# Cyan4973/FiniteStateEntropy

Measured on AMD Instinct MI355X. Metric: MB/s encode+decode per GPU on 32KB probagen blocks; bit-exact vs CPU ref, higher is better.
Workload: dtype u8; 1 GPU; probagen Proba14, 100000 x 32KB blocks per GPU, FSE encode+decode (one-shot calls at the reference's default limits: tableLog 11, decode maxLog 12), bit-exact check; blocks_per_gpu=100000, block_bytes=32768, codec=fse, parity=fse: roundtrip-all-blocks

## Files before the change

### finitestateentropy_amd/csrc/capi_batch.hip

```cpp
#include "internal.h"

extern "C" int FSEHIP_HIST_count_batch(unsigned* d_counts, unsigned* d_maxSymbolValues, size_t* d_results,
                                       const void* d_src, size_t srcStride, const size_t* d_sizes, size_t uniformSize,
                                       size_t nBlocks, void* stream)
{
    HistArgs a;
    a.counts = d_counts; a.maxSVs = d_maxSymbolValues; a.uniformMaxSV = 255; a.useUniformIn = 0;
    a.results = d_results; a.src = mkview(d_src, srcStride, d_sizes, uniformSize); a.nBlocks = nBlocks;
    return (int)launch_hist(a, (hipStream_t)stream);
}

extern "C" int FSEHIP_FSE_compress_usingCTable_batch(void* d_dst, size_t dstStride, size_t dstCapacity, size_t* d_results,
                                                     const void* d_src, size_t srcStride, const size_t* d_sizes, size_t uniformSize,
                                                     const FSEHIP_FSE_CTable* d_ctables, size_t ctableStrideU32, unsigned maxTableLog,
                                                     size_t nBlocks, void* stream)
{
    if (maxTableLog == 0 || maxTableLog > FSEHIP_FSE_MAX_TABLELOG) maxTableLog = FSEHIP_FSE_MAX_TABLELOG;
    FseEncArgs a;
    a.dst = (u8*)d_dst; a.dstStride = dstStride; a.dstCapacity = dstCapacity; a.results = d_results;
    a.src = mkview(d_src, srcStride, d_sizes, uniformSize);
    a.ctables = d_ctables; a.ctStrideU32 = ctableStrideU32; a.meta = nullptr;
    a.maxTableLog = maxTableLog; a.G = 0; a.slotU32 = 0; a.nBlocks = nBlocks; a.list = nullptr; a.count = nullptr;
    return (int)launch_fse_encode_auto(a, (hipStream_t)stream);
}

extern "C" int FSEHIP_FSE_decompress_usingDTable_batch(void* d_dst, size_t dstStride, size_t dstCapacity, size_t* d_results,
                                                       const void* d_cSrc, size_t cStride, const size_t* d_cSizes, size_t uniformCSize,
                                                       const FSEHIP_FSE_DTable* d_dtables, size_t dtableStrideU32, unsigned maxTableLog,
                                                       size_t nBlocks, void* stream)
{
    if (maxTableLog == 0 || maxTableLog > FSEHIP_FSE_MAX_TABLELOG) maxTableLog = FSEHIP_FSE_MAX_TABLELOG;
    FseDecArgs a;
    a.dst = (u8*)d_dst; a.dstStride = dstStride; a.dstCapacity = dstCapacity; a.results = d_results;
    a.csrc = mkview(d_cSrc, cStride, d_cSizes, uniformCSize);
    a.dtables = d_dtables; a.dtStrideU32 = dtableStrideU32; a.atab = nullptr; a.symtab = nullptr; a.meta = nullptr;
    a.maxTableLog = maxTableLog; a.G = 0; a.slotU32 = 0; a.nBlocks = nBlocks; a.tlMin = 0; a.declineNb0 = 0; a.onlyDeclined = 0;
    a.symScratch = nullptr; a.slotBitmap = nullptr; a.nSlots = 0; a.scratchSlotBytes = 0;
    return (int)launch_fse_decode(a, (hipStream_t)stream);
}

#define WS_SLACK 2048
#define WS_MAX_CHUNK 131072
static size_t ws_pass_blocks(size_t nBlocks) { const size_t c = nBlocks < WS_MAX_CHUNK ? nBlocks : WS_MAX_CHUNK; return c ? c : 1; }
static size_t ws_size(size_t nBlocks, size_t perBlock, size_t pad = 0) { return ws_pass_blocks(nBlocks) * perBlock + pad + WS_SLACK; }
static size_t round_chunk(size_t limit, size_t perRound)
{
    if (perRound == 0 || limit < perRound) return limit;
    return limit / perRound * perRound;
}
static size_t ws_chunk(size_t workspaceBytes, size_t nBlocks, size_t perBlock, size_t pad = 0, size_t perRound = 0)
{
    if (workspaceBytes < perBlock + pad + WS_SLACK) return 0;
    const size_t chunk = (workspaceBytes - WS_SLACK - pad) / perBlock;
    return chunk >= nBlocks ? nBlocks : round_chunk(chunk, perRound);
}
static inline size_t pass_blocks(size_t nBlocks, size_t b0, size_t chunk) { return nBlocks - b0 < chunk ? nBlocks - b0 : chunk; }

struct Carver {
    u8* const base; u8* p;
    explicit Carver(void* ws) : base((u8*)ws), p((u8*)ws) {}
    template <class T> T* take(size_t bytes) { T* const r = (T*)p; p += align_up(bytes, 256); return r; }
    template <class T> T* last(size_t bytes) { T* const r = (T*)p; p += bytes; return r; }
    size_t used() const { return (size_t)(p - base); }
};
template <class Meta> struct CounterWs {
    static constexpr size_t bytes_per_block = 1024 + 4 + 8 + sizeof(Meta);
    unsigned* counts; unsigned* maxSVs; size_t* hres; Meta* meta;
    CounterWs(Carver& c, size_t chunk)
        : counts(c.take<unsigned>(chunk * 1024)), maxSVs(c.take<unsigned>(chunk * 4)), hres(c.take<size_t>(chunk * 8)), meta(c.take<Meta>(chunk * sizeof(Meta))) {}
    HistArgs hist_args(unsigned msv, const BlockView& src, size_t nb) const
    {
        HistArgs h;
        h.counts = counts; h.maxSVs = maxSVs; h.uniformMaxSV = msv; h.useUniformIn = 1; h.results = hres; h.src = src; h.nBlocks = nb;
        return h;
    }
};
template <class Meta> struct BuildCTableWs {
    static constexpr size_t bytes_per_block = CounterWs<Meta>::bytes_per_block;
    Carver c; CounterWs<Meta> cb;
    BuildCTableWs(void* ws, size_t chunk) : c(ws), cb(c, chunk) {}
    size_t end() const { return c.used(); }
};

struct FseCWs { size_t perBlock; size_t ctU32; size_t ts; unsigned maxTl; };
static FseCWs fse_cws(unsigned tableLog)
{
    FseCWs w;
    unsigned tl = tableLog ? tableLog : FSEHIP_FSE_DEFAULT_TABLELOG;
    if (tl < 9) tl = 9;
    if (tl > FSEHIP_FSE_MAX_TABLELOG) tl = FSEHIP_FSE_MAX_TABLELOG;
    w.maxTl = tl;
    w.ctU32 = FSEHIP_FSE_CTABLE_SIZE_U32(tl, 255);
    w.ts = (size_t)1 << tl;
    w.perBlock = 1024 + 4 + 8 + sizeof(FseMeta) + 4 * w.ctU32 + FSE_EBINS * sizeof(u32);
    return w;
}
struct FseCompWs {
    Carver c; CounterWs<FseMeta> cb; u32* ctables; u32* encLists; u32* encCounts;
    FseCompWs(void* ws, size_t chunk, const FseCWs& w)
        : c(ws), cb(c, chunk), ctables(c.take<u32>(chunk * 4 * w.ctU32)), encLists(c.take<u32>(chunk * FSE_EBINS * sizeof(u32))),
          encCounts(c.last<u32>(FSE_EBINS * sizeof(u32))) {}
    size_t end() const { return c.used(); }
};

extern "C" size_t FSEHIP_FSE_compress_batch_workspaceSize(size_t nBlocks, unsigned tableLog) { return ws_size(nBlocks, fse_cws(tableLog).perBlock); }

extern "C" int FSEHIP_FSE_compress_batch(void* d_dst, size_t dstStride, size_t dstCapacity, size_t* d_results,
                                         const void* d_src, size_t srcStride, const size_t* d_sizes, size_t uniformSize,
                                         unsigned maxSymbolValue, unsigned tableLog, size_t nBlocks,
                                         void* d_workspace, size_t workspaceBytes, void* stream)
{
    hipStream_t s = (hipStream_t)stream;
    if ((uintptr_t)d_workspace & 255u) return (int)hipErrorInvalidValue;
    if (nBlocks == 0) return 0;
    if (tableLog > FSEHIP_FSE_MAX_TABLELOG)
        return batch_arg_error(d_results, nullptr, 0, dstCapacity, nBlocks, FSEHIP_ERROR(tableLog_tooLarge), 0, s);
    if (maxSymbolValue > 255 && tableLog != 0) {
        const size_t wksp = 4 * (size_t)FSEHIP_FSE_CTABLE_SIZE_U32(FSEHIP_FSE_MAX_TABLELOG, 255) + ((size_t)1 << FSEHIP_FSE_MAX_TABLELOG);
        const size_t ctBytes = 4 * (1 + ((size_t)1 << (tableLog - 1)) + 2 * ((size_t)maxSymbolValue + 1));
        if (ctBytes <= wksp && wksp - ctBytes < 4096)
            return batch_arg_error(d_results, d_sizes, uniformSize, dstCapacity, nBlocks, FSEHIP_ERROR(workSpace_tooSmall), 2, s);
    }
    return fse_compress_view(d_dst, dstStride, dstCapacity, d_results, mkview(d_src, srcStride, d_sizes, uniformSize), maxSymbolValue, tableLog, nBlocks,
                             d_workspace, workspaceBytes, s);
}
int fse_compress_view(void* d_dst, size_t dstStride, size_t dstCapacity, size_t* d_results, const BlockView& srcAll, unsigned maxSymbolValue, unsigned tableLog,
                      size_t nBlocks, void* d_workspace, size_t workspaceBytes, hipStream_t s)
{
    const FseCWs w = fse_cws(tableLog);
    const size_t chunk = ws_chunk(workspaceBytes, nBlocks, w.perBlock, 0, fse_encode_blocks_per_round(w.maxTl));
    if (chunk == 0) return (int)hipErrorInvalidValue;
    const FseCompWs ws(d_workspace, chunk, w);
    if (ws.end() > workspaceBytes) return (int)hipErrorInvalidValue;
    unsigned msv = maxSymbolValue ? maxSymbolValue : 255;
    if (msv > 255) msv = 255;
    for (size_t b0 = 0; b0 < nBlocks; b0 += chunk) {
        const size_t nb = pass_blocks(nBlocks, b0, chunk);
        const BlockView src = subview(srcAll, b0);
        CK(launch_hist(ws.cb.hist_args(msv, src, nb), s));
        FseCPrepArgs c;
        c.counts = ws.cb.counts; c.maxSVs = ws.cb.maxSVs; c.histResults = ws.cb.hres; c.src = src;
        c.dst = (u8*)d_dst + b0 * dstStride; c.dstStride = dstStride; c.dstCapacity = dstCapacity;
        c.maxSVReq = msv; c.tableLogReq = tableLog;
        c.ctables = ws.ctables; c.ctStrideU32 = w.ctU32; c.maxTl = w.maxTl;
        c.meta = ws.cb.meta; c.results = d_results + b0; c.nBlocks = nb;
        CK(launch_fse_cprep(c, s));
        FseEncArgs e;
        e.dst = (u8*)d_dst + b0 * dstStride; e.dstStride = dstStride; e.dstCapacity = dstCapacity; e.results = d_results + b0;
        e.src = src; e.ctables = ws.ctables; e.ctStrideU32 = w.ctU32; e.meta = ws.cb.meta;
        e.maxTableLog = w.maxTl; e.G = 0; e.slotU32 = 0; e.nBlocks = nb; e.list = ws.encLists; e.count = ws.encCounts;
        CK(launch_fse_encode_auto(e, s));
    }
    return 0;
}

struct FseDecWs {
    static size_t bytes_per_block(unsigned maxLog) { return sizeof(FseMeta) + 512 + 3 * ((size_t)1 << maxLog) + FSE_DCLS_COUNT * sizeof(u32); }
    Carver c; FseMeta* meta; s16* norms; u16* atab; u8* symtab; u32* lists; u32* counts;
    FseDecWs(void* ws, size_t chunk, unsigned maxLog)
        : c(ws), meta(c.take<FseMeta>(chunk * sizeof(FseMeta))), norms(c.take<s16>(chunk * 512)), atab(c.take<u16>((chunk * 2) << maxLog)),
          symtab(c.take<u8>(chunk << maxLog)), lists(c.take<u32>(chunk * FSE_DCLS_COUNT * sizeof(u32))), counts(c.last<u32>(FSE_DCLS_COUNT * sizeof(u32))) {}
    size_t end() const { return c.used(); }
    FseDPrepArgs dprep_args(const BlockView& cs, unsigned maxLog, size_t* results, size_t nb) const
    {
        FseDPrepArgs d;
        d.csrc = cs; d.maxLog = maxLog; d.atab = atab; d.symtab = symtab; d.norms = norms; d.meta = meta; d.lists = lists; d.counts = counts;
        d.results = results; d.nBlocks = nb; d.rawRle = 0; d.origSizes = nullptr; d.uniformOrig = 0;
        return d;
    }
};
static_assert(5 * 255 + FSE_DCLS_COUNT * sizeof(u32) <= WS_SLACK && 6 * 255 + FSE_EBINS * sizeof(u32) <= WS_SLACK, "WS_SLACK covers the padding of the FSE workspaces");
static unsigned clamp_maxlog(unsigned maxLog) { return (maxLog == 0 || maxLog > FSEHIP_FSE_MAX_TABLELOG) ? FSEHIP_FSE_MAX_TABLELOG : maxLog; }

extern "C" size_t FSEHIP_FSE_decompress_batch_workspaceSize(size_t nBlocks, unsigned maxLog) { return ws_size(nBlocks, FseDecWs::bytes_per_block(clamp_maxlog(maxLog))); }

static int fse_decompress_impl(void* d_dst, size_t dstStride, size_t dstCapacity, size_t* d_results, const BlockView& csAll, unsigned maxLog, size_t nBlocks,
                               void* d_workspace, size_t workspaceBytes, hipStream_t s, const size_t* d_origSizes, size_t uniformOrig, int rawRle,
                               const u64* d_dstOffsets = nullptr, const size_t* d_dstCaps = nullptr)
{
    if ((uintptr_t)d_workspace & 255u) return (int)hipErrorInvalidValue;
    if (nBlocks == 0) return 0;
    maxLog = clamp_maxlog(maxLog);
    const size_t chunk = ws_chunk(workspaceBytes, nBlocks, FseDecWs::bytes_per_block(maxLog), 0, fse_decode_blocks_per_round(maxLog));
    if (chunk == 0) return (int)hipErrorInvalidValue;
    const FseDecWs ws(d_workspace, chunk, maxLog);
    if (ws.end() > workspaceBytes) return (int)hipErrorInvalidValue;
    for (size_t b0 = 0; b0 < nBlocks; b0 += chunk) {
        const size_t nb = pass_blocks(nBlocks, b0, chunk);
        const BlockView cs = subview(csAll, b0);
        if (rawRle) CK(launch_rawrle_expand((u8*)d_dst + b0 * dstStride, dstStride, dstCapacity, d_results + b0, cs, d_origSizes ? d_origSizes + b0 : nullptr, uniformOrig, nb, s));
        FseDPrepArgs d = ws.dprep_args(cs, maxLog, d_results + b0, nb);
        d.rawRle = rawRle; d.origSizes = d_origSizes ? d_origSizes + b0 : nullptr; d.uniformOrig = uniformOrig;
        CK(launch_fse_dprep(d, s));
        FseDecArgs e;
        e.dst = (u8*)d_dst + b0 * dstStride; e.dstStride = dstStride; e.dstCapacity = dstCapacity; e.results = d_results + b0;
        e.csrc = cs; e.dtables = nullptr; e.dtStrideU32 = 0; e.atab = ws.atab; e.symtab = ws.symtab; e.meta = ws.meta;
        e.maxTableLog = maxLog; e.G = 0; e.slotU32 = 0; e.nBlocks = nb; e.tlMin = 0; e.declineNb0 = 0; e.onlyDeclined = 0;
        e.symScratch = nullptr; e.slotBitmap = nullptr; e.nSlots = 0; e.scratchSlotBytes = 0;
        if (d_dstOffsets) { e.dst = (u8*)d_dst; e.dstOffsets = d_dstOffsets + b0; e.dstCaps = d_dstCaps + b0; }
        CK(launch_fse_decode_classes(e, ws.lists, ws.counts, s));
    }
    return 0;
}
extern "C" int FSEHIP_FSE_decompress_batch(void* d_dst, size_t dstStride, size_t dstCapacity, size_t* d_results,
                                           const void* d_cSrc, size_t cStride, const size_t* d_cSizes, size_t uniformCSize,
                                           unsigned maxLog, size_t nBlocks,
                                           void* d_workspace, size_t workspaceBytes, void* stream)
{
    return fse_decompress_impl(d_dst, dstStride, dstCapacity, d_results, mkview(d_cSrc, cStride, d_cSizes, uniformCSize), maxLog, nBlocks,
                               d_workspace, workspaceBytes, (hipStream_t)stream, nullptr, 0, 0);
}
int fse_decompress_view(void* d_dst, const u64* d_dstOffsets, const size_t* d_dstCaps, size_t* d_results, const BlockView& csrc, unsigned maxLog, size_t nBlocks,
                        void* d_workspace, size_t workspaceBytes, hipStream_t s)
{
    return fse_decompress_impl(d_dst, 0, 0, d_results, csrc, maxLog, nBlocks, d_workspace, workspaceBytes, s, nullptr, 0, 0, d_dstOffsets, d_dstCaps);
}
extern "C" int FSEHIP_FSE_decompress_packed_batch(void* d_dst, size_t dstStride, size_t dstCapacity, size_t* d_results,
                                                  const void* d_packed, const uint64_t* d_offsets, const size_t* d_origSizes, size_t uniformOrigSize,
                                                  unsigned maxLog, size_t nBlocks, void* d_workspace, size_t workspaceBytes, void* stream)
{
    BlockView v = mkview(d_packed, 0, nullptr, 0);
    v.offsets = (const u64*)d_offsets;
    return fse_decompress_impl(d_dst, dstStride, dstCapacity, d_results, v, maxLog, nBlocks, d_workspace, workspaceBytes, (hipStream_t)stream,
                               d_origSizes, uniformOrigSize, 1);
}

extern "C" size_t FSEHIP_FSE_buildCTable_batch_workspaceSize(size_t nBlocks) { return ws_size(nBlocks, BuildCTableWs<FseMeta>::bytes_per_block); }
extern "C" int FSEHIP_FSE_buildCTable_batch(FSEHIP_FSE_CTable* d_ctables, size_t ctableStrideU32, void* d_headers, size_t headerStride, size_t headerCapacity,
                                            size_t* d_results, const void* d_src, size_t srcStride, const size_t* d_sizes, size_t uniformSize,
                                            unsigned maxSymbolValue, unsigned tableLog, size_t nBlocks, void* d_workspace, size_t workspaceBytes, void* stream)
{
    hipStream_t s = (hipStream_t)stream;
    if ((uintptr_t)d_workspace & 255u) return (int)hipErrorInvalidValue;
    if (nBlocks == 0) return 0;
    if (tableLog > FSEHIP_FSE_MAX_TABLELOG) return batch_arg_error(d_results, nullptr, 0, headerCapacity, nBlocks, FSEHIP_ERROR(tableLog_tooLarge), 0, s);
    const FseCWs w = fse_cws(tableLog);
    if (ctableStrideU32 < w.ctU32) return (int)hipErrorInvalidValue;
    const size_t chunk = ws_chunk(workspaceBytes, nBlocks, BuildCTableWs<FseMeta>::bytes_per_block);
    if (chunk == 0) return (int)hipErrorInvalidValue;
    const BuildCTableWs<FseMeta> ws(d_workspace, chunk);
    if (ws.end() > workspaceBytes) return (int)hipErrorInvalidValue;
    unsigned msv = maxSymbolValue ? maxSymbolValue : 255;
    if (msv > 255) msv = 255;
    for (size_t b0 = 0; b0 < nBlocks; b0 += chunk) {
        const size_t nb = pass_blocks(nBlocks, b0, chunk);
        const BlockView src = mkview((const u8*)d_src + b0 * srcStride, srcStride, d_sizes ? d_sizes + b0 : nullptr, uniformSize);
        CK(launch_hist(ws.cb.hist_args(msv, src, nb), s));
        FseCPrepArgs c;
        c.counts = ws.cb.counts; c.maxSVs = ws.cb.maxSVs; c.histResults = ws.cb.hres; c.src = src;
        c.dst = (u8*)d_headers + b0 * headerStride; c.dstStride = headerStride; c.dstCapacity = headerCapacity;
        c.maxSVReq = msv; c.tableLogReq = tableLog;
        c.ctables = d_ctables + b0 * ctableStrideU32; c.ctStrideU32 = ctableStrideU32; c.maxTl = w.maxTl;
        c.meta = ws.cb.meta; c.results = d_results + b0; c.nBlocks = nb;
        CK(launch_fse_cprep(c, s));
        CK(launch_hdr_results(ws.cb.meta, sizeof(FseMeta), d_results + b0, nb, s));
    }
    return 0;
}

extern "C" int FSEHIP_FSE_normalizeCount_batch(short* d_norms, size_t normStride, unsigned tableLog, const unsigned* d_counts, size_t countStride,
                                               const size_t* d_totals, const unsigned* d_maxSymbolValues, size_t nBlocks, size_t* d_results, void* stream)
{
    if (nBlocks == 0) return 0;
    if (!d_norms || !d_counts || !d_totals || !d_maxSymbolValues || !d_results || normStride < 256 || countStride < 256) return (int)hipErrorInvalidValue;
    return (int)launch_fse_glue_normalize((s16*)d_norms, normStride, tableLog, d_counts, countStride, d_totals, d_maxSymbolValues, d_results, nBlocks, (hipStream_t)stream);
}
extern "C" int FSEHIP_FSE_writeNCount_batch(void* d_headers, size_t headerStride, size_t headerCapacity, const short* d_norms, size_t normStride,
                                            const unsigned* d_maxSymbolValues, unsigned tableLog, size_t nBlocks, size_t* d_results, void* stream)
{
    if (nBlocks == 0) return 0;
    if (!d_headers || !d_norms || !d_maxSymbolValues || !d_results || normStride < 256 || headerCapacity > headerStride) return (int)hipErrorInvalidValue;
    return (int)launch_fse_glue_write_ncount((u8*)d_headers, headerStride, headerCapacity, (const s16*)d_norms, normStride, d_maxSymbolValues, tableLog, d_results, nBlocks,
                                             (hipStream_t)stream);
}
extern "C" int FSEHIP_FSE_readNCount_batch(short* d_norms, size_t normStride, unsigned* d_maxSymbolValues, unsigned* d_tableLogs,
                                           const void* d_headers, size_t headerStride, const size_t* d_headerSizes, size_t uniformHeaderSize,
                                           size_t nBlocks, size_t* d_results, void* stream)
{
    if (nBlocks == 0) return 0;
    if (!d_norms || !d_maxSymbolValues || !d_tableLogs || !d_headers || !d_results) return (int)hipErrorInvalidValue;
    return (int)launch_fse_glue_read_ncount((s16*)d_norms, normStride, d_maxSymbolValues, d_tableLogs, mkview(d_headers, headerStride, d_headerSizes, uniformHeaderSize),
                                            d_results, nBlocks, (hipStream_t)stream);
}

extern "C" size_t FSEHIP_FSE_buildDTable_batch_workspaceSize(size_t nBlocks, unsigned maxLog) { return FSEHIP_FSE_decompress_batch_workspaceSize(nBlocks, maxLog); }
extern "C" int FSEHIP_FSE_buildDTable_batch(FSEHIP_FSE_DTable* d_dtables, size_t dtableStrideU32, size_t* d_results,
                                            const void* d_headers, size_t headerStride, const size_t* d_headerSizes, size_t uniformHeaderSize,
                                            unsigned maxLog, size_t nBlocks, void* d_workspace, size_t workspaceBytes, void* stream)
{
    hipStream_t s = (hipStream_t)stream;
    if ((uintptr_t)d_workspace & 255u) return (int)hipErrorInvalidValue;
    if (nBlocks == 0) return 0;
    maxLog = clamp_maxlog(maxLog);
    if (dtableStrideU32 < FSEHIP_FSE_DTABLE_SIZE_U32(maxLog)) return (int)hipErrorInvalidValue;
    const size_t chunk = ws_chunk(workspaceBytes, nBlocks, FseDecWs::bytes_per_block(maxLog));
    if (chunk == 0) return (int)hipErrorInvalidValue;
    const FseDecWs ws(d_workspace, chunk, maxLog);
    if (ws.end() > workspaceBytes) return (int)hipErrorInvalidValue;
    for (size_t b0 = 0; b0 < nBlocks; b0 += chunk) {
        const size_t nb = pass_blocks(nBlocks, b0, chunk);
        const FseDPrepArgs d = ws.dprep_args(mkview((const u8*)d_headers + b0 * headerStride, headerStride, d_headerSizes ? d_headerSizes + b0 : nullptr, uniformHeaderSize),
                                             maxLog, d_results + b0, nb);
        CK(launch_fse_dprep(d, s));
        CK(launch_fse_export_dtables(d, d_dtables + b0 * dtableStrideU32, dtableStrideU32, s));
        CK(launch_hdr_results(ws.meta, sizeof(FseMeta), d_results + b0, nb, s));
    }
    return 0;
}

extern "C" int FSEHIP_FSE_buildCTable_fromNorm_batch(FSEHIP_FSE_CTable* d_ctables, size_t ctableStrideU32, const short* d_norms, size_t normStride,
                                                     const unsigned* d_maxSymbolValues, unsigned tableLog, size_t nBlocks, size_t* d_results, void* stream)
{
    if (nBlocks == 0) return 0;
    if (!d_ctables || !d_norms || !d_maxSymbolValues || !d_results || normStride < 256) return (int)hipErrorInvalidValue;
    if (tableLog >= 1 && tableLog <= FSEHIP_FSE_MAX_TABLELOG && ctableStrideU32 < FSEHIP_FSE_CTABLE_SIZE_U32(tableLog, 255)) return (int)hipErrorInvalidValue;
    return (int)launch_fse_ctable_from_norm((const s16*)d_norms, normStride, d_maxSymbolValues, tableLog, d_ctables, ctableStrideU32, d_results, nBlocks, (hipStream_t)stream);
}
extern "C" size_t FSEHIP_FSE_buildDTable_fromNorm_batch_workspaceSize(size_t nBlocks, unsigned tableLog) { return FSEHIP_FSE_decompress_batch_workspaceSize(nBlocks, tableLog); }
extern "C" int FSEHIP_FSE_buildDTable_fromNorm_batch(FSEHIP_FSE_DTable* d_dtables, size_t dtableStrideU32, const short* d_norms, size_t normStride,
                                                     const unsigned* d_maxSymbolValues, unsigned tableLog, size_t nBlocks, size_t* d_results,
                                                     void* d_workspace, size_t workspaceBytes, void* stream)
{
    hipStream_t s = (hipStream_t)stream;
    if ((uintptr_t)d_workspace & 255u) return (int)hipErrorInvalidValue;
    if (nBlocks == 0) return 0;
    if (!d_dtables || !d_norms || !d_maxSymbolValues || !d_results || normStride < 256) return (int)hipErrorInvalidValue;
    if (tableLog > FSEHIP_FSE_MAX_TABLELOG) return batch_arg_error(d_results, nullptr, 0, 0, nBlocks, FSEHIP_ERROR(tableLog_tooLarge), 0, s);
    const unsigned maxLog = tableLog ? tableLog : 1;
    if (dtableStrideU32 < FSEHIP_FSE_DTABLE_SIZE_U32(maxLog)) return (int)hipErrorInvalidValue;
    const size_t chunk = ws_chunk(workspaceBytes, nBlocks, FseDecWs::bytes_per_block(maxLog));
    if (chunk == 0) return (int)hipErrorInvalidValue;
    const FseDecWs ws(d_workspace, chunk, maxLog);
    if (ws.end() > workspaceBytes) return (int)hipErrorInvalidValue;
    for (size_t b0 = 0; b0 < nBlocks; b0 += chunk) {
        const size_t nb = pass_blocks(nBlocks, b0, chunk);
        const FseDPrepArgs d = ws.dprep_args(mkview(nullptr, 0, nullptr, 0), maxLog, d_results + b0, nb);
        CK(launch_fse_dprep_from_norm(d, (const s16*)d_norms + b0 * normStride, normStride, d_maxSymbolValues + b0, tableLog, s));
        CK(launch_fse_export_dtables(d, d_dtables + b0 * dtableStrideU32, dtableStrideU32, s));
        CK(launch_hdr_results(ws.meta, sizeof(FseMeta), d_results + b0, nb, s));
    }
    return 0;
}

extern "C" size_t FSEHIP_HUF_buildCTable_batch_workspaceSize(size_t nBlocks) { return ws_size(nBlocks, BuildCTableWs<HufMeta>::bytes_per_block); }
extern "C" int FSEHIP_HUF_buildCTable_batch(FSEHIP_HUF_CElt* d_ctables, size_t ctableStrideU32, void* d_headers, size_t headerStride, size_t headerCapacity,
                                            size_t* d_results, const void* d_src, size_t srcStride, const size_t* d_sizes, size_t uniformSize,
                                            unsigned maxSymbolValue, unsigned tableLog, size_t nBlocks, void* d_workspace, size_t workspaceBytes, void* stream)
{
    hipStream_t s = (hipStream_t)stream;
    if ((uintptr_t)d_workspace & 255u) return (int)hipErrorInvalidValue;
    if (nBlocks == 0) return 0;
    if (tableLog > FSEHIP_HUF_TABLELOG_MAX || maxSymbolValue > 255)
        return batch_arg_error(d_results, d_sizes, uniformSize, headerCapacity, nBlocks,
                               tableLog > FSEHIP_HUF_TABLELOG_MAX ? FSEHIP_ERROR(tableLog_tooLarge) : FSEHIP_ERROR(maxSymbolValue_tooLarge), 1, s);
    if (ctableStrideU32 < 256) return (int)hipErrorInvalidValue;
    const size_t chunk = ws_chunk(workspaceBytes, nBlocks, BuildCTableWs<HufMeta>::bytes_per_block);
    if (chunk == 0) return (int)hipErrorInvalidValue;
    const BuildCTableWs<HufMeta> ws(d_workspace, chunk);
    if (ws.end() > workspaceBytes) return (int)hipErrorInvalidValue;
    const unsigned msv = maxSymbolValue ? maxSymbolValue : 255;
    for (size_t b0 = 0; b0 < nBlocks; b0 += chunk) {
        const size_t nb = pass_blocks(nBlocks, b0, chunk);
        const BlockView src = mkview((const u8*)d_src + b0 * srcStride, srcStride, d_sizes ? d_sizes + b0 : nullptr, uniformSize);
        CK(launch_hist(ws.cb.hist_args(msv, src, nb), s));
        HufCPrepArgs c;
        c.counts = ws.cb.counts; c.maxSVs = ws.cb.maxSVs; c.histResults = ws.cb.hres; c.src = src;
        c.dst = (u8*)d_headers + b0 * headerStride; c.dstStride = headerStride; c.dstCapacity = headerCapacity;
        c.maxSVReq = msv; c.huffLogReq = tableLog; c.ctables = d_ctables + b0 * ctableStrideU32; c.ctStrideU32 = ctableStrideU32;
        c.meta = ws.cb.meta; c.results = d_results + b0; c.nBlocks = nb;
        CK(launch_huf_cprep(c, s, nullptr));
        CK(launch_hdr_results(ws.cb.meta, sizeof(HufMeta), d_results + b0, nb, s));
    }
    return 0;
}

extern "C" int FSEHIP_HUF_buildCTable_fromCount_batch(FSEHIP_HUF_CElt* d_ctables, size_t ctableStrideU32, const unsigned* d_counts, size_t countStride,
                                                      const unsigned* d_maxSymbolValues, unsigned maxNbBits, size_t nBlocks, size_t* d_results, void* stream)
{
    if (nBlocks == 0) return 0;
    if (!d_ctables || !d_counts || !d_maxSymbolValues || !d_results || ctableStrideU32 < 256 || (ctableStrideU32 & 3) || countStride != 256) return (int)hipErrorInvalidValue;
    HufCPrepArgs c;
    c.counts = d_counts; c.maxSVs = d_maxSymbolValues; c.histResults = nullptr; c.src = mkview(nullptr, 0, nullptr, 0);
    c.dst = nullptr; c.dstStride = 0; c.dstCapacity = 0; c.maxSVReq = 255; c.huffLogReq = maxNbBits;
    c.ctables = d_ctables; c.ctStrideU32 = ctableStrideU32; c.meta = nullptr; c.results = d_results; c.nBlocks = nBlocks;
    return (int)launch_huf_cprep_glue(c, 1, (hipStream_t)stream);
}
extern "C" int FSEHIP_HUF_writeCTable_batch(void* d_headers, size_t headerStride, size_t headerCapacity, const FSEHIP_HUF_CElt* d_ctables, size_t ctableStrideU32,
                                            const unsigned* d_maxSymbolValues, unsigned huffLog, size_t nBlocks, size_t* d_results, void* stream)
{
    if (nBlocks == 0) return 0;
    if (!d_headers || !d_ctables || !d_maxSymbolValues || !d_results || ctableStrideU32 < 256 || (ctableStrideU32 & 3) || headerCapacity > headerStride) return (int)hipErrorInvalidValue;
    HufCPrepArgs c;
    c.counts = nullptr; c.maxSVs = d_maxSymbolValues; c.histResults = nullptr; c.src = mkview(nullptr, 0, nullptr, 0);
    c.dst = (u8*)d_headers; c.dstStride = headerStride; c.dstCapacity = headerCapacity; c.maxSVReq = 255; c.huffLogReq = huffLog;
    c.ctables = (u32*)d_ctables; c.ctStrideU32 = ctableStrideU32; c.meta = nullptr; c.results = d_results; c.nBlocks = nBlocks;
    return (int)launch_huf_cprep_glue(c, 2, (hipStream_t)stream);
}

struct HufReadDTableWs {
    static constexpr size_t bytes_per_block = sizeof(HufMeta) + HUF_DCLS_COUNT * sizeof(u32);
    Carver c; HufMeta* meta; u32* lists; u32* counts;
    HufReadDTableWs(void* ws, size_t chunk)
        : c(ws), meta(c.take<HufMeta>(chunk * sizeof(HufMeta))), lists(c.take<u32>(chunk * HUF_DCLS_COUNT * sizeof(u32))), counts(c.last<u32>(HUF_DCLS_COUNT * sizeof(u32))) {}
    size_t end() const { return c.used(); }
};
static int huf_read_dtable_batch(hipError_t (*launch)(const HufDPrepArgs&, hipStream_t), FSEHIP_HUF_DTable* d_dtables, size_t dtableStrideU32, unsigned maxTableLog,
                                 size_t* d_results, const void* d_src, size_t srcStride, const size_t* d_srcSizes, size_t uniformSrcSize,
                                 size_t nBlocks, void* d_workspace, size_t workspaceBytes, hipStream_t s)
{
    const size_t chunk = ws_chunk(workspaceBytes, nBlocks, HufReadDTableWs::bytes_per_block);
    if (chunk == 0) return (int)hipErrorInvalidValue;
    const HufReadDTableWs ws(d_workspace, chunk);
    if (ws.end() > workspaceBytes) return (int)hipErrorInvalidValue;
    for (size_t b0 = 0; b0 < nBlocks; b0 += chunk) {
        const size_t nb = pass_blocks(nBlocks, b0, chunk);
        HufDPrepArgs d;
        d.csrc = mkview((const u8*)d_src + b0 * srcStride, srcStride, d_srcSizes ? d_srcSizes + b0 : nullptr, uniformSrcSize);
        d.dstSizes = mkview(nullptr, 0, nullptr, 0); d.dst = nullptr; d.dstStride = 0;
        d.dtables = d_dtables + b0 * dtableStrideU32; d.dtStrideU32 = dtableStrideU32; d.meta = ws.meta; d.lists = ws.lists; d.counts = ws.counts;
        d.results = d_results + b0; d.nBlocks = nb; d.tableOnly = 1; d.dtMaxLog = maxTableLog;
        CK(launch(d, s));
    }
    return 0;
}
extern "C" size_t FSEHIP_HUF_readDTableX1_batch_workspaceSize(size_t nBlocks) { return ws_size(nBlocks, HufReadDTableWs::bytes_per_block); }
extern "C" int FSEHIP_HUF_readDTableX1_batch(FSEHIP_HUF_DTable* d_dtables, size_t dtableStrideU32, unsigned maxTableLog, size_t* d_results,
                                             const void* d_src, size_t srcStride, const size_t* d_srcSizes, size_t uniformSrcSize,
                                             size_t nBlocks, void* d_workspace, size_t workspaceBytes, void* stream)
{
    if ((uintptr_t)d_workspace & 255u) return (int)hipErrorInvalidValue;
    if (nBlocks == 0) return 0;
    if (maxTableLog == 0 || maxTableLog > FSEHIP_HUF_TABLELOG_MAX) maxTableLog = FSEHIP_HUF_TABLELOG_MAX;
    if (dtableStrideU32 < 1 + ((size_t)1 << maxTableLog)) return (int)hipErrorInvalidValue;
    return huf_read_dtable_batch(launch_huf_dprep, d_dtables, dtableStrideU32, maxTableLog, d_results, d_src, srcStride, d_srcSizes, uniformSrcSize,
                                 nBlocks, d_workspace, workspaceBytes, (hipStream_t)stream);
}

extern "C" size_t FSEHIP_HUF_readDTableX2_batch_workspaceSize(size_t nBlocks) { return FSEHIP_HUF_readDTableX1_batch_workspaceSize(nBlocks); }
extern "C" int FSEHIP_HUF_readDTableX2_batch(FSEHIP_HUF_DTable* d_dtables, size_t dtableStrideU32, unsigned maxTableLog, size_t* d_results,
                                             const void* d_src, size_t srcStride, const size_t* d_srcSizes, size_t uniformSrcSize,
                                             size_t nBlocks, void* d_workspace, size_t workspaceBytes, void* stream)
{
    if ((uintptr_t)d_workspace & 255u) return (int)hipErrorInvalidValue;
    if (nBlocks == 0) return 0;
    if (maxTableLog <= FSEHIP_HUF_TABLELOG_MAX && dtableStrideU32 < 1 + ((size_t)1 << maxTableLog)) return (int)hipErrorInvalidValue;
    return huf_read_dtable_batch(launch_huf_dprep_x2, d_dtables, dtableStrideU32, maxTableLog, d_results, d_src, srcStride, d_srcSizes, uniformSrcSize,
                                 nBlocks, d_workspace, workspaceBytes, (hipStream_t)stream);
}

extern "C" int FSEHIP_HUF_compress4X_usingCTable_batch(void* d_dst, size_t dstStride, size_t dstCapacity, size_t* d_results,
                                                       const void* d_src, size_t srcStride, const size_t* d_sizes, size_t uniformSize,
                                                       const FSEHIP_HUF_CElt* d_ctables, size_t ctableStrideU32,
                                                       size_t nBlocks, void* stream)
{
    HufEncArgs a;
    a.dst = (u8*)d_dst; a.dstStride = dstStride; a.dstCapacity = dstCapacity; a.results = d_results;
    a.src = mkview(d_src, srcStride, d_sizes, uniformSize);
    a.ctables = d_ctables; a.ctStrideU32 = ctableStrideU32; a.meta = nullptr; a.streams = 4; a.split1X = 0; a.nBlocks = nBlocks;
    return (int)launch_huf_encode(a, (hipStream_t)stream);
}

extern "C" int FSEHIP_HUF_compress1X_usingCTable_batch(void* d_dst, size_t dstStride, size_t dstCapacity, size_t* d_results,
                                                       const void* d_src, size_t srcStride, const size_t* d_sizes, size_t uniformSize,
                                                       const FSEHIP_HUF_CElt* d_ctables, size_t ctableStrideU32,
                                                       size_t nBlocks, void* stream)
{
    HufEncArgs a;
    a.dst = (u8*)d_dst; a.dstStride = dstStride; a.dstCapacity = dstCapacity; a.results = d_results;
    a.src = mkview(d_src, srcStride, d_sizes, uniformSize);
    a.ctables = d_ctables; a.ctStrideU32 = ctableStrideU32; a.meta = nullptr; a.streams = 1; a.split1X = 1; a.nBlocks = nBlocks;
    return (int)launch_huf_encode(a, (hipStream_t)stream);
}

static int huf_dtable_batch(int streams, int acceptX2, void* d_dst, size_t dstStride, const size_t* d_dstSizes, size_t uniformDstSize,
// ... 262 lines not shown
```

### finitestateentropy_amd/csrc/fse_decode.hip

```cpp
#include "internal.h"
#include <atomic>

#include "bitreader.h"

#ifndef FSE_SYM_L1
#define FSE_SYM_L1 1
#endif
#ifndef FSE_DEC_RING
#define FSE_DEC_RING 64
#endif
#define FSE_IN_RING 256
#define FSE_IN_RING_LOG 8
#define FSE_IN_CHUNK 64
#define FSE_IN_LANES (FSE_IN_CHUNK / 4)
#define FSE_IN_MIRROR 16
#ifndef FSE_CHECK_EVERY
#define FSE_CHECK_EVERY 16
#endif
#ifndef FSE_PHASE_UNROLL
#define FSE_PHASE_UNROLL 16
#endif
#define FSE_FINISH_EVERY 2
#ifndef FSE_DEC_LDS_KB
#define FSE_DEC_LDS_KB 160
#endif
#ifndef FSE_DEC_WAVES
#define FSE_DEC_WAVES 2
#endif
#ifndef FSE_SRV_WAVES
#define FSE_SRV_WAVES 9
#endif
#define FSE_MAXG (4 * FSE_SRV_WAVES)
#define FSE_WGS_PER_CU (160 / FSE_DEC_LDS_KB)

__device__ unsigned long long g_decTiming[16];
static std::atomic<bool> g_decTimingOn{false};
#define TIMING(...) do { if constexpr (TIMED) { __VA_ARGS__ } } while (0)
struct BulkState { u32 s, q, bq; };

typedef const __attribute__((address_space(1))) u8* gbl_u8_ptr;
typedef __attribute__((address_space(1))) u8* gbl_u8_w_ptr;
typedef u32 __attribute__((aligned(1))) u32_unaligned;
DEV u32 gbl_load_u32(gbl_u8_ptr p) { return *(const __attribute__((address_space(1))) u32_unaligned*)p; }
DEV void gbl_store_u32(gbl_u8_w_ptr p, u32 w) { *(__attribute__((address_space(1))) u32_unaligned*)p = w; }
typedef const __attribute__((address_space(3))) u16* lds_u16_ptr;
typedef const __attribute__((address_space(3))) u32* lds_u32_ptr;
DEV u32 lds_cell(u32 addr) { return *(lds_u16_ptr)(uintptr_t)addr; }

DEV bool wave_all(bool p) { return __builtin_amdgcn_ballot_w64(p) == __builtin_amdgcn_ballot_w64(true); }
DEV u32 dpp_swap(u32 v) { return (u32)__builtin_amdgcn_mov_dpp((int)v, 0xB1, 0xF, 0xF, true); }

template <bool NB0>
DEV void fse_bulk_phase(u32& sMine, u32& qRef, u32& bqRef, u32 tabOff, u32 myIn, u32 half, u32 maskB, uint2* ringMine)
{
    u32 s = sMine, q = qRef, bq = bqRef;
    u32 prev = 0;
    (void)half;
    u32 w0, w1, w2;
    {   const lds_u32_ptr wp = (lds_u32_ptr)(uintptr_t)(myIn + (q & (FSE_IN_RING - 4)));
        w0 = wp[0]; w1 = wp[1]; w2 = wp[2]; }
#pragma unroll 8
    for (int it = 0; it < FSE_CHECK_EVERY; ++it) {
        const u32 c = lds_cell(s);
        const lds_u32_ptr np = (lds_u32_ptr)(uintptr_t)(myIn + ((q - 8u) & (FSE_IN_RING - 4)));
        const u32 n0 = np[0], n1 = np[1];
        const u32 thi = __builtin_amdgcn_alignbit(w2, w1, bq), tlo = __builtin_amdgcn_alignbit(w1, w0, bq);
        const u32 cO = dpp_swap(c);
        const u32 nbM = c >> 12, nbO = cO >> 12;
        const u32 sStart = s;
        {   const u32 t = thi << (nbO & maskB);
            const u32 bits = __builtin_amdgcn_ubfe(t, 32u - nbM, nbM);
            s = (((c & 0xFFFu) | bits) << 1) + tabOff; }
        const u32 c2 = lds_cell(s);
        const u32 s12 = nbM + nbO;
        u32 t3 = __builtin_amdgcn_alignbit(thi, tlo, 32u - s12);
        if (NB0) t3 = s12 ? t3 : thi;
        const u32 rec = __builtin_amdgcn_perm(s, sStart, 0x05040100u);
        const u32 cO2 = dpp_swap(c2);
        const u32 nbM2 = c2 >> 12, nbO2 = cO2 >> 12;
        {   const u32 t = t3 << (nbO2 & maskB);
            const u32 bits = __builtin_amdgcn_ubfe(t, 32u - nbM2, nbM2);
            s = (((c2 & 0xFFFu) | bits) << 1) + tabOff; }
        const int left = (int)bq - (int)(s12 + nbM2 + nbO2);
        const bool k1 = left < 0, k2 = left < -32;
        w2 = k2 ? w0 : (k1 ? w1 : w2);
        w1 = k2 ? n1 : (k1 ? w0 : w1);
        w0 = k2 ? n0 : (k1 ? n1 : w0);
        q += (u32)((left >> 5) << 2);
        bq = (u32)left & 31u;
        if (it & 1) ringMine[it & ~1] = make_uint2(prev, rec); else prev = rec;
    }
    sMine = s; qRef = q; bqRef = bq;
}

DEV u32 dpp_swap_and(u32 v, u32 m) { return dpp_swap(v) & m; }
DEV u32 dpp_swap_add(u32 v, u32 w) { return dpp_swap(v) + w; }
DEV u32 lshl_or(u32 v, u32 sh, u32 o) { u32 r; __asm__("v_lshl_or_b32 %0, %1, %2, %3" : "=v"(r) : "v"(v), "v"(sh), "v"(o)); return r; }
DEV u32 ring_dword(u32 P) { u32 r; __asm__("v_bfe_u32 %0, %1, 5, %2" : "=v"(r) : "v"(P), "n"(FSE_IN_RING_LOG - 2)); return r; }
#define SB __builtin_amdgcn_sched_barrier(0)
template <int NITER>
DEV void fse_bulk_phase_rev(u32& sMine, u32& Pref, u32& PheadRef, u32 K, u32 cellShift, u32 tabOff, u32 myIn, u32 maskB, uint2* ringMine)
{
    u32 s = sMine, P = Pref;
    u32 prev = 0;
    __asm__ volatile("" : "+v"(myIn));
    u32 c = lds_cell(s);
    u32 Pw = P;
    lds_u32_ptr wp = (lds_u32_ptr)(uintptr_t)(myIn + (ring_dword(P) << 2));
    u32 w0 = wp[0], w1 = wp[1], w2 = wp[2], w3 = wp[3];
#pragma unroll FSE_PHASE_UNROLL
    for (int it = 0; it < NITER; ++it) {
        if (it == NITER - 1) PheadRef = P;
        const bool k = ((P ^ Pw) & 32u) != 0;
        const u32 e0 = k ? w1 : w0, e1 = k ? w2 : w1, e2 = k ? w3 : w2;
        u32 lo = __builtin_amdgcn_alignbit(e1, e0, P);
        u32 hi = __builtin_amdgcn_alignbit(e2, e1, P);
        __asm__ volatile("" : "+v"(lo), "+v"(hi));
        SB;
        const u32 sStart = s;
        s = lshl_or(__builtin_amdgcn_ubfe(lo, dpp_swap_and(c, maskB), c), K - c, (c >> cellShift) | tabOff);
        const u32 c2 = lds_cell(s);
        SB;
        const u32 n1 = dpp_swap_add(c, c);
        const u32 P1 = P + (n1 & 31u);
        if (it + 1 < NITER) {
            Pw = P1;
            wp = (lds_u32_ptr)(uintptr_t)(myIn + (ring_dword(P1) << 2));
            w0 = wp[0]; w1 = wp[1]; w2 = wp[2]; w3 = wp[3];
        }
        u32 lo2 = __builtin_amdgcn_alignbit(hi, lo, n1);
        u32 rec = __builtin_amdgcn_perm(s, sStart, 0x05040100u);
        __asm__ volatile("" : "+v"(lo2), "+v"(rec));
        if (it & 1) ringMine[it & ~1] = make_uint2(prev, rec); else prev = rec;
        SB;
        s = lshl_or(__builtin_amdgcn_ubfe(lo2, dpp_swap_and(c2, maskB), c2), K - c2, (c2 >> cellShift) | tabOff);
        if (it + 1 < NITER) c = lds_cell(s);
        SB;
        const u32 n2 = dpp_swap_add(c2, c2);
        P = P1 + (n2 & 31u);
    }
    sMine = s; Pref = P;
}
#undef SB

struct DecCtl {
    u32 pubIters;
    u32 pubPofs;
    u32 srvFlushed;
    int srvValidLo;
    int initValidLo;
    int S32;
    u32 inLo, inHi, outLo, outHi, symLo, symHi;
};
#define FSE_DEC_THREADS (64 * (FSE_DEC_WAVES + FSE_SRV_WAVES))

DEV u32 ctl_load(const u32* p) { return __hip_atomic_load(p, __ATOMIC_ACQUIRE, __HIP_MEMORY_SCOPE_WORKGROUP); }
DEV int ctl_load(const int* p) { return __hip_atomic_load(p, __ATOMIC_ACQUIRE, __HIP_MEMORY_SCOPE_WORKGROUP); }
DEV u32 ctl_peek(const u32* p) { const u32 v = __hip_atomic_load(p, __ATOMIC_RELAXED, __HIP_MEMORY_SCOPE_WORKGROUP); __asm__ volatile("" ::: "memory"); return v; }
DEV int ctl_peek(const int* p) { const int v = __hip_atomic_load(p, __ATOMIC_RELAXED, __HIP_MEMORY_SCOPE_WORKGROUP); __asm__ volatile("" ::: "memory"); return v; }
DEV void ctl_store(u32* p, u32 v) { __hip_atomic_store(p, v, __ATOMIC_RELEASE, __HIP_MEMORY_SCOPE_WORKGROUP); }
DEV u64 ctl_load2(const u32* p) { return __hip_atomic_load((const u64*)p, __ATOMIC_ACQUIRE, __HIP_MEMORY_SCOPE_WORKGROUP); }
DEV u64 ctl_peek2(const u32* p) { const u64 v = __hip_atomic_load((const u64*)p, __ATOMIC_RELAXED, __HIP_MEMORY_SCOPE_WORKGROUP); __asm__ volatile("" ::: "memory"); return v; }
DEV void ctl_store2(u32* p, u32 lo, u32 hi) { __hip_atomic_store((u64*)p, (u64)lo | ((u64)hi << 32), __ATOMIC_RELEASE, __HIP_MEMORY_SCOPE_WORKGROUP); }
DEV void ctl_store(int* p, int v) { __hip_atomic_store(p, v, __ATOMIC_RELEASE, __HIP_MEMORY_SCOPE_WORKGROUP); }

#define FSE_SRV_G 4
#ifndef FSE_FLUSH_MIN
#define FSE_FLUSH_MIN 32u
#endif
static_assert(FSE_SRV_WAVES * FSE_SRV_G == FSE_MAXG, "every block of a workgroup has a service wave");
static_assert((FSE_DEC_RING & (FSE_DEC_RING - 1)) == 0 && FSE_DEC_RING % FSE_CHECK_EVERY == 0, "ring positions wrap by masking; a phase never wraps");
DEV void fse_ring_put(u32* rg, int off, u32 w)
{
    const u32 j = (u32)off & (FSE_IN_RING - 1);
    rg[j >> 2] = w;
    if (j < FSE_IN_MIRROR) rg[(FSE_IN_RING + j) >> 2] = w;
}
DEV void fse_ring_put_rev(u32* rg, int Sg, int off, u32 w) { fse_ring_put(rg, ((Sg + 3) & ~3) - 4 - off, __brev(w)); }
DEV u32 fse_scratch_slot_claim(const FseDecArgs& a, u32* flagsSh)
{
    u32 slot = (u32)blockIdx.x % a.nSlots;
    for (;;) {
        const u32 bit = 1u << (slot & 31u);
        const u32 old = __hip_atomic_fetch_or(a.slotBitmap + (slot >> 5), bit, __ATOMIC_ACQUIRE, __HIP_MEMORY_SCOPE_AGENT);
        if (!(old & bit)) break;
        slot = slot + 1 == a.nSlots ? 0 : slot + 1;
    }
    flagsSh[6] = slot;
#if FSE_SYM_L1
    __builtin_amdgcn_fence(__ATOMIC_ACQUIRE, "agent");
#endif
    return slot;
}
DEV void fse_scratch_slot_done(const FseDecArgs& a, u32* flagsSh, int lane)
{
    if (lane == 0 && atomicAdd(&flagsSh[7], 1u) == FSE_SRV_WAVES + FSE_DEC_WAVES - 1) {
        const u32 slot = flagsSh[6];
        __hip_atomic_fetch_and(a.slotBitmap + (slot >> 5), ~(1u << (slot & 31u)), __ATOMIC_RELEASE, __HIP_MEMORY_SCOPE_AGENT);
    }
}
DEV u32 srv_rl(u32 v, int l) { return (u32)__builtin_amdgcn_readlane((int)v, l); }
DEV unsigned long long srv_rl64(unsigned long long v, int l) { return (unsigned long long)srv_rl((u32)v, l) | ((unsigned long long)srv_rl((u32)(v >> 32), l) << 32); }
template <bool TIMED, bool CALLER>
DEV void fse_decode_service(const FseDecArgs& a, u8* ldsb, DecCtl* ctlAll, u32 slotBytes, u32 ringOff, u32 inOff, int lane, int g0, bool rev, u32* flagsSh)
{
    const int myG = g0 + (lane < FSE_SRV_G ? lane : 0);
    DecCtl* const ctl = ctlAll + (myG < a.G ? myG : 0);
    const unsigned long long inBits = ((unsigned long long)ctl->inHi << 32) | ctl->inLo;
    const unsigned long long outBits = ((unsigned long long)ctl->outHi << 32) | ctl->outLo;
    const unsigned long long tabBits = ((unsigned long long)ctl->symHi << 32) | ctl->symLo;
    const int S32 = ctl->S32;
    int validLo = ctl->initValidLo;
    u32 flushed = 0, fpos = 0;
    bool live = lane < FSE_SRV_G && myG < a.G && !(ctl->pubPofs >> 31);

    static_assert(64 / FSE_IN_LANES == FSE_SRV_G, "one 16-lane group per block of a service wave");
    const int grp = lane / FSE_IN_LANES, sub = lane % FSE_IN_LANES;
    const int SgK = __shfl(S32, grp, WAVE);
    const gbl_u8_ptr igK = (gbl_u8_ptr)(uintptr_t)__shfl(inBits, grp, WAVE);
    u32* const rgK = (u32*)(ldsb + (size_t)(g0 + grp) * slotBytes + inOff);
    {   const bool liveK = (__ballot(live) >> grp) & 1ull;
        const int vlo = __shfl(validLo, grp, WAVE);
#pragma unroll
        for (int c = 0; c < FSE_IN_RING / FSE_IN_CHUNK; ++c) {
            const int off = liveK ? vlo + FSE_IN_CHUNK * c + 4 * sub : -1;
            if (off >= 0 && off + 4 <= SgK) { const u32 w = gbl_load_u32(igK + off); if (rev) fse_ring_put_rev(rgK, SgK, off, w); else fse_ring_put(rgK, off, w); }
            else if (off >= 0 && off < SgK) {
                u32 w = 0;
                for (int i = 0; i < 3; ++i) if (off + i < SgK) w |= (u32)igK[off + i] << (8 * i);
                if (rev) fse_ring_put_rev(rgK, SgK, off, w); else fse_ring_put(rgK, off, w);
            }
        }
        if (live) ctl_store(&ctl->srvValidLo, validLo);
    }

    int nextOff = __shfl(validLo, grp, WAVE) - FSE_IN_CHUNK + 4 * sub;
    u32 pend = 0;
    if (((__ballot(live) >> grp) & 1ull) && nextOff >= 0 && nextOff + 4 <= SgK) pend = gbl_load_u32(igK + nextOff);
    u32 yq[FSE_SRV_G][4];
#pragma unroll
    for (int l = 0; l < FSE_SRV_G; ++l) { yq[l][0] = yq[l][1] = yq[l][2] = yq[l][3] = 0; }
    unsigned long long sBusy = 0, sIdle = 0, nBusy = 0, sA = 0;
    (void)sBusy; (void)sIdle; (void)nBusy; (void)sA;
    TIMING(sA = __builtin_readcyclecounter(););
    for (;;) {
        u32 pp = 0x80000000u, it = flushed;
        if (live) { const u64 pub = ctl_load2(&ctl->pubIters); it = (u32)pub; pp = (u32)(pub >> 32); }
        const bool fin = (pp >> 31) != 0;
        const int P = (int)(pp & 0x7FFFFFFFu);
        const u32 avail = it - flushed;
        const bool wantFlush = live && (avail >= FSE_FLUSH_MIN || (fin && avail > 0));
        const bool wantFill = live && !fin && validLo > 0 && P + 4 <= validLo + (FSE_IN_RING - FSE_IN_CHUNK);
        const unsigned long long fm = __ballot(wantFlush), rm = __ballot(wantFill);
        if (live && fin && avail == 0) live = false;
        if (!(fm | rm)) {
            if (!__any(live)) break;
            __builtin_amdgcn_s_sleep(4);
            TIMING(const unsigned long long sB = __builtin_readcyclecounter(); sIdle += sB - sA; sA = sB;);
            continue;
        }
        const bool fillK = (rm >> grp) & 1ull;
        if (rm) {
            if (fillK) { if (rev) fse_ring_put_rev(rgK, SgK, nextOff, pend); else fse_ring_put(rgK, nextOff, pend); }
            if (wantFill) { validLo -= FSE_IN_CHUNK; ctl_store(&ctl->srvValidLo, validLo); }
            if (fillK) {
                nextOff -= FSE_IN_CHUNK;
                pend = 0;
                if (nextOff >= 0 && nextOff + 4 <= SgK) pend = gbl_load_u32(igK + nextOff);
            }
        }
#pragma unroll
        for (int l = 0; l < FSE_SRV_G; ++l) {
            if (!((fm >> l) & 1ull)) continue;
            const u32 cnt = srv_rl(avail, l), fp_g = srv_rl(fpos, l);
            const gbl_u8_ptr tg = (gbl_u8_ptr)(uintptr_t)srv_rl64(tabBits, l);
            if ((u32)lane < cnt) {
                u32 ri = fp_g + (u32)lane;
                ri = ri >= FSE_DEC_RING ? ri - FSE_DEC_RING : ri;
                const u32* const rw = (const u32*)(ldsb + (size_t)(g0 + l) * slotBytes + ringOff) + 4u * (ri >> 1) + (ri & 1u);
                uint2 rec; rec.x = rw[0]; rec.y = rw[2];
                const u32 x0 = __builtin_amdgcn_ubfe(rec.x, 1u, a.ldsLog), x1 = __builtin_amdgcn_ubfe(rec.x, 17u, a.ldsLog);
                const u32 x2 = __builtin_amdgcn_ubfe(rec.y, 1u, a.ldsLog), x3 = __builtin_amdgcn_ubfe(rec.y, 17u, a.ldsLog);
#if FSE_SYM_L1
                yq[l][0] = tg[x0]; yq[l][2] = tg[x1]; yq[l][1] = tg[x2]; yq[l][3] = tg[x3];
#else
                if (CALLER) {
                    yq[l][0] = __hip_atomic_load(tg + x0, __ATOMIC_RELAXED, __HIP_MEMORY_SCOPE_AGENT); yq[l][2] = __hip_atomic_load(tg + x1, __ATOMIC_RELAXED, __HIP_MEMORY_SCOPE_AGENT);
                    yq[l][1] = __hip_atomic_load(tg + x2, __ATOMIC_RELAXED, __HIP_MEMORY_SCOPE_AGENT); yq[l][3] = __hip_atomic_load(tg + x3, __ATOMIC_RELAXED, __HIP_MEMORY_SCOPE_AGENT);
                } else { yq[l][0] = tg[x0]; yq[l][2] = tg[x1]; yq[l][1] = tg[x2]; yq[l][3] = tg[x3]; }
#endif
            }
        }
        if (wantFlush) { ctl_store(&ctl->srvFlushed, it); }
#pragma unroll
        for (int l = 0; l < FSE_SRV_G; ++l) {
            if (!((fm >> l) & 1ull)) continue;
            const u32 cnt = srv_rl(avail, l), fl_g = srv_rl(flushed, l);
            gbl_u8_w_ptr const og = (gbl_u8_w_ptr)(uintptr_t)(srv_rl64(outBits, l) + 4ull * fl_g);
            if ((u32)lane < cnt) {
                const u32 w = yq[l][0] | (yq[l][1] << 8) | (yq[l][2] << 16) | (yq[l][3] << 24);
                gbl_store_u32(og + 4u * lane, w);
            }
        }
        if (wantFlush) { fpos += it - flushed; fpos = fpos >= FSE_DEC_RING ? fpos - FSE_DEC_RING : fpos; flushed = it; }
        TIMING(const unsigned long long sB = __builtin_readcyclecounter(); sBusy += sB - sA; sA = sB; ++nBusy;);
    }
    TIMING(if (lane == 0 && g0 == 0) { atomicAdd(&g_decTiming[5], sBusy); atomicAdd(&g_decTiming[6], sIdle); });
    if (CALLER) fse_scratch_slot_done(a, flagsSh, lane);
}

struct FseCellsRef { const u32* cells;
    DEV void get(u32 st, u32& ns, u32& nb, u32& sym) const { const u32 c = cells[st]; ns = c & 0xFFFFu; sym = (c >> 16) & 0xFFu; nb = c >> 24; } };
struct FseCellsCompact { const u16* A; const u8* syms;
    DEV void get(u32 st, u32& ns, u32& nb, u32& sym) const { const u32 c = A[st]; ns = c & 0xFFFu; nb = c >> 12; sym = syms[st]; } };
struct FseCellsRev { const u16* A; const u8* syms; u32 tl, cellShift;
    DEV void get(u32 st, u32& ns, u32& nb, u32& sym) const { const u32 i = __brev(st) >> (32u - tl); const u32 c = A[i]; nb = c & 31u; ns = __brev(c >> cellShift) >> (32u - tl); sym = syms[i]; } };
template <class Cells>
DEV u32 fse_tail_step(const Cells& t, u32& state, BitReader& r, bool fast)
{
    u32 ns, nb, sym;
    t.get(state, ns, nb, sym);
    const u32 low = fast ? r.read_fast(nb) : r.read(nb);
    state = ns + low;
    return sym;
}
template <class Cells>
DEV size_t fse_tail(const Cells& t, u32 s1, u32 s2, BitReader& r, u8* out, long op, long omax, bool fast)
{
    for (;;) {
        const int st = r.reload();
        if (!((st == BR_UNFINISHED) & (op < omax - 3))) break;
        u32 w = fse_tail_step(t, s1, r, fast);
        w |= fse_tail_step(t, s2, r, fast) << 8;
        w |= fse_tail_step(t, s1, r, fast) << 16;
        w |= fse_tail_step(t, s2, r, fast) << 24;
        __builtin_memcpy(out + op, &w, 4);
        op += 4;
    }
    for (;;) {
        if (op > omax - 2) return FERR(dstSize_tooSmall);
        out[op++] = (u8)fse_tail_step(t, s1, r, fast);
        if (r.reload() == BR_OVERFLOW) { out[op++] = (u8)fse_tail_step(t, s2, r, fast); return (size_t)op; }
        if (op > omax - 2) return FERR(dstSize_tooSmall);
        out[op++] = (u8)fse_tail_step(t, s2, r, fast);
        if (r.reload() == BR_OVERFLOW) { out[op++] = (u8)fse_tail_step(t, s1, r, fast); return (size_t)op; }
    }
}

template <bool FAST, bool TIMED, bool CALLER, bool VIEW = false>
__global__ __launch_bounds__(FSE_DEC_THREADS) void k_fse_decode(FseDecArgs a)
{
    extern __shared__ __attribute__((aligned(16))) u32 lds[];
    const int tid = threadIdx.x, lane = tid & 63, wave = tid >> 6;
    unsigned long long tBorn = 0, wBorn = 0;
    (void)tBorn; (void)wBorn;
    TIMING(tBorn = __builtin_readcyclecounter(); wBorn = wall_clock64(););
    const size_t first = (size_t)blockIdx.x * a.G;
    static_assert(FSE_DBINS % 4 == 0, "the bin lengths are read as 16-byte vectors");
    size_t nTot = a.nBlocks, q0 = first;
    u32 bin0 = 0, cnt0 = 0xFFFFFFFFu;
    if (a.count) {
        uint4 cv[FSE_DBINS / 4];
#pragma unroll
        for (u32 i = 0; i < FSE_DBINS / 4; ++i) cv[i] = ((const uint4*)a.count)[i];
        u64 before = 0;
        bool found = false;
#pragma unroll
        for (u32 i = 0; i < FSE_DBINS; ++i) {
            const uint4 v = cv[i >> 2];
            const u32 c = (i & 3u) == 0 ? v.x : (i & 3u) == 1 ? v.y : (i & 3u) == 2 ? v.z : v.w;
            const bool here = !found & (((u64)first < before + c) | (i == FSE_DBINS - 1));
            bin0 = here ? i : bin0; q0 = here ? (size_t)((u64)first - before) : q0; cnt0 = here ? c : cnt0;
            found |= here;
            before += c;
        }
        nTot = (size_t)before;
    }
    if (first >= nTot) return;
    auto slotBlock = [&](size_t g) -> size_t {
        if (!a.list) return first + g;
        size_t q = q0 + g; u32 i = bin0;
        if (q >= cnt0) {
            while (i < FSE_DBINS - 1) { const u32 c = a.count[i]; if (q < c) break; q -= c; ++i; }
        }
        return a.list[(size_t)i * a.nBlocks + q];
    };
    u8* const lds8 = (u8*)lds;
    const u32 tabStride = 2u << a.ldsLog;
    DecCtl* const ctlAll = (DecCtl*)(lds8 + (size_t)a.G * tabStride);
    u8* const ldsb = (u8*)ctlAll + (size_t)a.G * sizeof(DecCtl);
    const u32 slotBytes = a.slotU32 * 4u;
    const u32 ringOff = 0;
    const u32 inOff = FSE_DEC_RING * 8;

    u32* const flagsSh = (u32*)(ldsb + (size_t)a.G * slotBytes);
    if (tid < 6 || tid == 7) flagsSh[tid] = 0;
    const bool decWave = wave < FSE_DEC_WAVES;
    u8* const tlSh = (u8*)(flagsSh + 8);
    if (CALLER) {
        __syncthreads();
        bool mine = false;
        if (tid >= 64 && tid < 64 + a.G) {
            const size_t g = (size_t)tid - 64;
            u32 tl = 0xFFu;
            if (first + g < nTot) {
                const size_t bi = slotBlock(g);
                if (!(a.onlyDeclined && a.results[bi] != FSE_DECLINED)) {
                    const u32 t0 = a.dtables[bi * a.dtStrideU32] & 0xFFFFu;
                    if (t0 <= a.ldsLog && t0 >= a.tlMin) tl = t0;
                    else if (t0 > a.maxTableLog && a.tlMin == 0 && !a.onlyDeclined) a.results[bi] = FERR(tableLog_tooLarge);
                }
            }
            tlSh[g] = (u8)tl;
            mine = tl != 0xFFu;
        }
        if (mine) flagsSh[1] = 1u;
        u32 slot = 0;
        if (tid == 0) slot = fse_scratch_slot_claim(a, flagsSh);
        __syncthreads();
        if (!flagsSh[1]) {
            if (tid == 0) __hip_atomic_fetch_and(a.slotBitmap + (slot >> 5), ~(1u << (slot & 31u)), __ATOMIC_RELEASE, __HIP_MEMORY_SCOPE_AGENT);
            return;
        }
    }
    else __syncthreads();
    u8* const symSlot = CALLER ? a.symScratch + (size_t)flagsSh[6] * a.scratchSlotBytes : nullptr;
    {   u64 badBits = 0, declBits = 0; bool anyNb0 = false;
        if (!CALLER) {
            const size_t nTab = nTot - first < (size_t)a.G ? nTot - first : (size_t)a.G;
            if (tabStride >= 1024u) {
                const u32 ppt = tabStride >> 10;
                const u32 nPieces = (u32)nTab * ppt;
                for (u32 p = (u32)wave; p < nPieces; p += FSE_DEC_THREADS / 64) {
                    const u32 g = p / ppt, k = p - g * ppt;
                    const size_t bi = slotBlock(g);
                    const u8* const src = (const u8*)(a.atab + (bi << a.maxTableLog)) + 1024u * k + 16u * (u32)lane;
                    __builtin_amdgcn_global_load_lds((const __attribute__((address_space(1))) void*)src,
                                                     (__attribute__((address_space(3))) void*)(lds8 + 1024u * p), 16, 0, 0);
                }
            }
            else {
            uint4* const dstv = (uint4*)lds8;
            const u32 vptLog = a.ldsLog - 3u;
            const u32 nvec = (u32)nTab << vptLog;
            constexpr u32 MAXV = (FSE_MAXG * 512u / 16u + FSE_DEC_THREADS - 1) / FSE_DEC_THREADS;
            uint4 buf[MAXV];
#pragma unroll
            for (u32 k = 0; k < MAXV; ++k) {
                const u32 idx = tid + k * FSE_DEC_THREADS;
                if (idx < nvec) {
                    const size_t sl = first + (idx >> vptLog);
                    const size_t bi = slotBlock(sl - first);
                    buf[k] = ((const uint4*)(a.atab + (bi << a.maxTableLog)))[idx & ((1u << vptLog) - 1u)];
                }
            }
#pragma unroll
            for (u32 k = 0; k < MAXV; ++k) { const u32 idx = tid + k * FSE_DEC_THREADS; if (idx < nvec) dstv[idx] = buf[k]; }
            }
            if (!FAST) for (size_t g = 0; g < nTab; ++g) {
                const u32 st = a.meta[slotBlock(g)].state; anyNb0 |= st != 0 && !(st & 2u); }
        }
        else {
            const size_t nTab = nTot - first < (size_t)a.G ? nTot - first : (size_t)a.G;
            constexpr u32 QL = 2048u / 4u / 64u;
            if (!decWave) for (u32 g = (u32)wave - FSE_DEC_WAVES; g < (u32)nTab; g += FSE_SRV_WAVES) {
                const u32 tl = tlSh[g];
                if (tl == 0xFFu) continue;
                const u32 ts = 1u << tl;
                const u32* const t = a.dtables + slotBlock(g) * a.dtStrideU32;
                u8* const slotB = lds8 + (size_t)g * tabStride;
                u16* const A = (u16*)slotB;
                u8* const symOut = symSlot + ((size_t)g << a.ldsLog);
                bool bad = false, nbz = false;
                if (FAST && tl >= 4u) {
                    const u32 sR = 32u - tl;
                    const u32 qo[4] = { 0u, 1u << (tl - 1u), 1u << (tl - 2u), 3u << (tl - 2u) };
                    const u32 passes = ts > 2048u ? ts / 2048u : 1u;
                    u32 acc = 0, minNb = 15u;
                    uint4 cv[QL];
                    for (u32 h = 0; h < passes; ++h) {
#pragma unroll
                        for (u32 j = 0; j < QL; ++j) {
                            const u32 i0 = 2048u * h + 4u * ((u32)lane + 64u * j);
                            cv[j] = make_uint4(0, 0, 0, 0);
                            if (i0 < ts) __builtin_memcpy(&cv[j], t + 1 + i0, 16);
                        }
#pragma unroll
                        for (u32 j = 0; j < QL; ++j) {
                            const u32 i0 = 2048u * h + 4u * ((u32)lane + 64u * j);
                            if (i0 >= ts) continue;
                            const u32 r0 = __brev(i0) >> sR;
                            const u32 cw[4] = { cv[j].x, cv[j].y, cv[j].z, cv[j].w };
#pragma unroll
                            for (u32 q = 0; q < 4; ++q) {
                                const u32 c = cw[q], ns = c & 0xFFFFu, nb = c >> 24;
                                acc |= (ns >> tl) | ((tl - nb) >> 5) | (ns & ((1u << (nb & 31u)) - 1u));
                                minNb = nb < minNb ? nb : minNb;
                                slotB[r0 | qo[q]] = (u8)(c >> 16);
                            }
                        }
                    }
                    { for (u32 off = 16u * (u32)lane; off < ts; off += 1024u) { const uint4 v = *(const uint4*)(slotB + off); *(uint4*)(symOut + off) = v; } }
                    for (u32 h = 0; h < passes; ++h) {
                        if (passes > 1u) {
#pragma unroll
                            for (u32 j = 0; j < QL; ++j) { const u32 i0 = 2048u * h + 4u * ((u32)lane + 64u * j); __builtin_memcpy(&cv[j], t + 1 + i0, 16); }
                        }
#pragma unroll
                        for (u32 j = 0; j < QL; ++j) {
                            const u32 i0 = 2048u * h + 4u * ((u32)lane + 64u * j);
                            if (i0 >= ts) continue;
                            const u32 r0 = __brev(i0) >> sR;
                            const u32 cw[4] = { cv[j].x, cv[j].y, cv[j].z, cv[j].w };
#pragma unroll
                            for (u32 q = 0; q < 4; ++q) {
                                const u32 c = cw[q];
                                A[r0 | qo[q]] = (u16)(((__brev(c << 16) >> (16u - tl)) << 5) | ((c >> 24) & 31u));
                            }
                        }
                    }
                    bad = acc != 0; nbz = minNb == 0;
                } else {
#pragma unroll 2
                    for (u32 i = (u32)lane; i < ts; i += 64u) {
                        const u32 c = t[1 + i];
                        const u32 ns = c & 0xFFFFu, nb = c >> 24;
                        bad |= (ns >> tl) != 0 || nb > tl || nb > 15u || (ns & ((1u << (nb & 15u)) - 1u)) != 0;
                        nbz |= nb == 0;
                        const u32 pos = FAST ? __brev(i) >> (32u - tl) : i;
                        symOut[pos] = (u8)(c >> 16);
                        if (FAST) A[pos] = (u16)((nb & 31u) | ((__brev(ns & ((1u << tl) - 1u)) >> (32u - tl)) << 5));
                        else A[pos] = (u16)((ns & 0xFFFu) | (nb << 12));
                    }
                }
                if (__any(bad)) badBits |= 1ull << g;
                if (FAST && tl == 12u && __any(nbz)) declBits |= 1ull << g;
                anyNb0 |= __any(nbz) != 0;
            }
        }
        if (badBits) { atomicOr(&flagsSh[2], (u32)badBits); atomicOr(&flagsSh[3], (u32)(badBits >> 32)); }
        if (declBits) { atomicOr(&flagsSh[4], (u32)declBits); atomicOr(&flagsSh[5], (u32)(declBits >> 32)); }
        if (anyNb0) atomicOr(&flagsSh[0], 1u);
    }
    const int ppw = (a.G + FSE_DEC_WAVES - 1) / FSE_DEC_WAVES;
    const int gsl = (decWave ? wave * ppw : 0) + (lane >> 1);
    const u32 half = (u32)lane & 1u, maskB = half ? ~0u : 0u;
    const bool inRange = (lane >> 1) < ppw && gsl < a.G && first + (size_t)gsl < nTot;
    const size_t b = inRange ? slotBlock((size_t)gsl) : 0;
    bool owner = decWave && inRange;
    u32 hdr = 0;
    if (owner && a.meta) { if (a.meta[b].state == 0) owner = false; else hdr = a.meta[b].hdrSize; }
    u32 tl = 0; bool fast = false;
    constexpr bool compact = !CALLER;
    const u32* const gtab = compact ? nullptr : a.dtables + (owner ? b : 0) * a.dtStrideU32;
    if (owner) {
        if (compact) { tl = a.meta[b].tableLog; fast = (a.meta[b].state & 2u) != 0; if (tl > a.ldsLog) { a.results[b] = FERR(tableLog_tooLarge); owner = false; } }
        else {
            const u32 h0 = gtab[0]; tl = h0 & 0xFFFFu; fast = (h0 >> 16) != 0;
            if (tlSh[gsl] == 0xFFu) owner = false;
        }
    }
    const u32* const cells = compact ? nullptr : gtab + 1;
    const u8* const syms = compact ? a.symtab + ((owner ? b : 0) << a.maxTableLog) : symSlot + ((size_t)(gsl < a.G ? gsl : 0) << a.ldsLog);
    const u32 ldsBase = (u32)(uintptr_t)(__attribute__((address_space(3))) u8*)lds8;
    if (ldsBase & (tabStride - 1)) __builtin_trap();
    const u32 tabOff = ldsBase + (u32)(gsl < a.G ? gsl : 0) * tabStride;
    const u16* const A = (const u16*)(lds8 + (tabOff - ldsBase));
    const u8* in = nullptr; size_t S = 0; u8* out = nullptr;
    const long omax = VIEW ? (long)a.dstCaps[owner ? b : 0] : (long)a.dstCapacity;
    long op = 0;
    BitReader r; r.base = nullptr; r.size = 0; r.at = 0; r.win = 0; r.used = 0;
    u32 s1 = 0, s2 = 0;
    if (owner) {
        in = view_ptr(a.csrc, b) + hdr;
        S = view_size(a.csrc, b) - hdr;
        out = VIEW ? a.dst + a.dstOffsets[b] : a.dst + b * a.dstStride;
        const size_t e = r.init(in, S);
        if (is_err(e)) { a.results[b] = e; owner = false; }
        else {
            s1 = r.read(tl); r.reload();
            s2 = r.read(tl); r.reload();
        }
    }

    __builtin_amdgcn_s_waitcnt(0x0f70);
    __syncthreads();
    const u64 badMask = (u64)flagsSh[2] | ((u64)flagsSh[3] << 32);
    const u64 declMask = (u64)flagsSh[4] | ((u64)flagsSh[5] << 32);
    const bool nb0 = flagsSh[0] != 0;
    if (CALLER && owner && a.declineNb0 && ((declMask >> gsl) & 1ull)) { if (half == 0) a.results[b] = FSE_DECLINED; owner = false; }

    const bool bulkOk = owner && S < (1ull << 28) && !((badMask >> gsl) & 1ull) && !(FAST && !compact && ((declMask >> gsl) & 1ull));
    const int Bstart = bulkOk ? (int)(8u * ((u32)r.at + 8u)) - (int)r.used : 0;
    const long groups0 = (omax - 3 - op + 3) / 4;
    bool can = bulkOk && (FAST ? Bstart >= 65 + 48 * (FSE_CHECK_EVERY - 1) : r.at >= 24 + 6 * FSE_CHECK_EVERY + 8) && groups0 >= FSE_CHECK_EVERY;
    bool can2 = FAST && bulkOk && Bstart >= 65 + 48 * (FSE_FINISH_EVERY - 1) && groups0 >= FSE_FINISH_EVERY;
    const bool everBulk = can || can2;
    BulkState bs; bs.q = 0; bs.bq = 0;
    {   const u32 st = half ? s2 : s1;
        bs.s = tabOff + 2u * (FAST ? __brev(st) >> (32u - (tl ? tl : 1u)) : st); }
    const u32 inA = (u32)((uintptr_t)in & 3u);
    const u32 R8 = 8u * (((u32)S + inA + 3u) & ~3u);
    u32 P = 0;
    long groups = 0;
    u32 iters = 0;
    int validLo = 0;
    if (everBulk) {
        const u32 B = 8u * ((u32)r.at + 8u + inA) - r.used;
        bs.q = 4u * (B >> 5) - 8u; bs.bq = B & 31u; P = R8 - B;
        groups = (omax - 3 - op + 3) >> 2;
        const int c0 = (int)((0 - ((uintptr_t)in - inA)) & (FSE_IN_CHUNK - 1));
        validLo = (((int)bs.q + 8 - 112 - c0) & ~(FSE_IN_CHUNK - 1)) + c0;
    }
    DecCtl* const ctl = ctlAll + (gsl < a.G ? gsl : 0);
    if (decWave && (lane >> 1) < ppw && gsl < a.G && half == 0) {
        ctl->pubIters = 0; ctl->pubPofs = everBulk ? bs.q + 8u : 0x80000000u;
        ctl->srvFlushed = 0; ctl->srvValidLo = 0x7FFFFFFF;
        ctl->initValidLo = validLo; ctl->S32 = (int)(S < (1ull << 31) ? S + inA : 0);
        const unsigned long long ib = (unsigned long long)(uintptr_t)(in - inA), ob = (unsigned long long)(uintptr_t)out, tb = (unsigned long long)(uintptr_t)syms;
        ctl->inLo = (u32)ib; ctl->inHi = (u32)(ib >> 32); ctl->outLo = (u32)ob; ctl->outHi = (u32)(ob >> 32); ctl->symLo = (u32)tb; ctl->symHi = (u32)(tb >> 32);
    }
    __syncthreads();
    if (!decWave) { fse_decode_service<TIMED, CALLER>(a, ldsb, ctlAll, slotBytes, ringOff, inOff, lane, (wave - FSE_DEC_WAVES) * FSE_SRV_G, FAST, flagsSh); return; }

    __builtin_amdgcn_s_setprio(3);
    uint2* const myRing = (uint2*)(ldsb + (size_t)(gsl < a.G ? gsl : 0) * slotBytes + ringOff) + half;
    const u32 myIn = (u32)(uintptr_t)(__attribute__((address_space(3))) u8*)(ldsb + (size_t)(gsl < a.G ? gsl : 0) * slotBytes + inOff);
    unsigned long long tRun = 0, tWait = 0, nRun = 0, nWait = 0, tA = 0, tFin = 0, nFin = 0, tInner = 0;
    (void)tRun; (void)tWait; (void)nRun; (void)nWait; (void)tA; (void)tFin; (void)nFin; (void)tInner;
    TIMING(tA = __builtin_readcyclecounter(););
    const unsigned long long tBulk0 = tA;
    (void)tBulk0;
    u32 rpos = 0;
    u64 srvNext = ctl_peek2(&ctl->srvFlushed);
    const u32 inA8 = 8u * inA;
    u32 Phead = P;
    int grp = groups > (1 << 30) ? (1 << 30) : (int)groups;
    if constexpr (FAST) {
        uint2* const dummyRing = (uint2*)(flagsSh + 32) + half;
        if ((lane >> 1) < ppw && everBulk) {
        for (;;) {
            const int lowest = (int)bs.q - 4 * ((48 * (FSE_CHECK_EVERY - 1) + 31) / 32);
            const int need = lowest > 0 ? lowest : 0;
            bool rdy;
            do {
                const u32 fl = (u32)srvNext;
                const int vlo = (int)(u32)(srvNext >> 32);
                srvNext = ctl_peek2(&ctl->srvFlushed);
                rdy = !can | ((iters + FSE_CHECK_EVERY - fl <= FSE_DEC_RING) & (need >= vlo));
                TIMING(if (!__all(rdy)) { const unsigned long long tB = __builtin_readcyclecounter(); tWait += tB - tA; ++nWait; tA = tB; });
            } while (!__all(rdy));
            if (!__any(can)) break;
            if (__all(can)) {
                u32 qp;
                for (;;) {
                    unsigned long long tI = 0; (void)tI;
                    TIMING(tI = __builtin_readcyclecounter(););
                    fse_bulk_phase_rev<FSE_CHECK_EVERY>(bs.s, P, Phead, tl + 1u, 4u, tabOff, myIn, maskB & 31u, myRing + (iters & (FSE_DEC_RING - 1)));
                    TIMING(tInner += __builtin_readcyclecounter() - tI;);
                    iters += FSE_CHECK_EVERY; grp -= FSE_CHECK_EVERY;
                    const u32 B = R8 - P;
                    qp = 4u * (B >> 5);
                    const u32 Bp = B - inA8;
                    const u32 shortBy = max(Bp - (65u + 48u * (FSE_CHECK_EVERY - 1)), (u32)grp - (u32)FSE_CHECK_EVERY);
                    can = shortBy < 0xC0000000u;
                    const bool more = can | ((Bp >= 65u + 48u * (FSE_FINISH_EVERY - 1)) & (grp >= FSE_FINISH_EVERY));
                    ctl_store2(&ctl->pubIters, iters, more ? qp : (qp | 0x80000000u));
                    TIMING(const unsigned long long tB = __builtin_readcyclecounter(); tRun += tB - tA; ++nRun; tA = tB;);
                    if (!wave_all(can)) break;
                    const int needF = max((int)qp - 8 - 4 * ((48 * (FSE_CHECK_EVERY - 1) + 31) / 32), 0);
                    const int roomF = FSE_DEC_RING - FSE_CHECK_EVERY - (int)iters;
                    bool rdyF;
                    do {
                        const int fl = (int)(u32)srvNext;
                        const int vlo = (int)(u32)(srvNext >> 32);
                        srvNext = ctl_peek2(&ctl->srvFlushed);
                        rdyF = min(roomF + fl, needF - vlo) >= 0;
                        TIMING(if (!wave_all(rdyF)) { const unsigned long long tB = __builtin_readcyclecounter(); tWait += tB - tA; ++nWait; tA = tB; });
                    } while (!wave_all(rdyF));
                }
                bs.q = qp - 8u; rpos = iters & (FSE_DEC_RING - 1);
                continue;
            }
            uint2* const ring = can ? myRing + rpos : dummyRing;
            u32 sN = bs.s, Pn = P, PhN = Phead;
            unsigned long long tI = 0; (void)tI;
            TIMING(tI = __builtin_readcyclecounter(););
            fse_bulk_phase_rev<FSE_CHECK_EVERY>(sN, Pn, PhN, tl + 1u, 4u, tabOff, myIn, maskB & 31u, ring);
            TIMING(tInner += __builtin_readcyclecounter() - tI;);
            bs.s = can ? sN : bs.s; P = can ? Pn : P; Phead = can ? PhN : Phead;
            const u32 adv = can ? (u32)FSE_CHECK_EVERY : 0u;
            rpos = (rpos + adv) & (FSE_DEC_RING - 1);
            iters += adv; grp -= (int)adv;
            const u32 B = R8 - P;
            bs.q = 4u * (B >> 5) - 8u;
            const u32 Bp = B - inA8;
            const bool canN = can & (Bp >= 65u + 48u * (FSE_CHECK_EVERY - 1)) & (grp >= FSE_CHECK_EVERY);
            const bool more = canN | ((Bp >= 65u + 48u * (FSE_FINISH_EVERY - 1)) & (grp >= FSE_FINISH_EVERY));
            if (can & (half == 0)) ctl_store2(&ctl->pubIters, iters, more ? bs.q + 8u : ((bs.q + 8u) | 0x80000000u));
            can = canN;
            TIMING(const unsigned long long tB = __builtin_readcyclecounter(); tRun += tB - tA; ++nRun; tA = tB;);
        }
        {   const u32 B = R8 - P; bs.bq = B & 31u;
            can2 = bulkOk & (B - inA8 >= 65u + 48u * (FSE_FINISH_EVERY - 1)) & (grp >= FSE_FINISH_EVERY); }
        can2 = can2 & bulkOk;
        for (;;) {
            const u32 fl = (u32)srvNext;
            const int vlo = (int)(u32)(srvNext >> 32);
            srvNext = ctl_peek2(&ctl->srvFlushed);
            const int lowest = (int)bs.q - 8;
            const bool rdy = !can2 | ((iters + FSE_FINISH_EVERY - fl <= FSE_DEC_RING) & ((lowest > 0 ? lowest : 0) >= vlo));
            if (!__all(rdy)) {
                TIMING(const unsigned long long tB = __builtin_readcyclecounter(); tWait += tB - tA; ++nWait; tA = tB;);
                continue;
            }
            if (!__any(can2)) break;
            uint2* const ring = can2 ? myRing + rpos : dummyRing;
            u32 sN = bs.s, Pn = P, PhN = Phead;
            fse_bulk_phase_rev<FSE_FINISH_EVERY>(sN, Pn, PhN, tl + 1u, 4u, tabOff, myIn, maskB & 31u, ring);
            bs.s = can2 ? sN : bs.s; P = can2 ? Pn : P; Phead = can2 ? PhN : Phead;
            rpos = can2 ? (rpos + FSE_FINISH_EVERY) & (FSE_DEC_RING - 1) : rpos;
            iters += can2 ? FSE_FINISH_EVERY : 0u; grp -= can2 ? FSE_FINISH_EVERY : 0;
            const u32 B = R8 - P;
            bs.q = 4u * (B >> 5) - 8u; bs.bq = B & 31u;
            const bool can2N = can2 & (B - inA8 >= 65u + 48u * (FSE_FINISH_EVERY - 1)) & (grp >= FSE_FINISH_EVERY);
            if (can2 & (half == 0)) ctl_store2(&ctl->pubIters, iters, can2N ? bs.q + 8u : ((bs.q + 8u) | 0x80000000u));
            can2 = can2N;
            TIMING(const unsigned long long tB = __builtin_readcyclecounter(); tFin += tB - tA; ++nFin; tA = tB;);
        }
        }
    } else {
    while (__any(can)) {
        const u32 fl = (u32)srvNext;
        const int vlo = (int)(u32)(srvNext >> 32);
        srvNext = ctl_peek2(&ctl->srvFlushed);
        const int lowest = (int)bs.q - (6 * FSE_CHECK_EVERY + 8);
        const bool ready = can & (iters + FSE_CHECK_EVERY - fl <= FSE_DEC_RING) & ((lowest > 0 ? lowest : 0) >= vlo);
        if (ready) {
            uint2* const ring = myRing + rpos;
            rpos = (rpos + FSE_CHECK_EVERY) & (FSE_DEC_RING - 1);
            if (nb0) fse_bulk_phase<true>(bs.s, bs.q, bs.bq, tabOff, myIn, half, maskB, ring);
            else     fse_bulk_phase<false>(bs.s, bs.q, bs.bq, tabOff, myIn, half, maskB, ring);
            iters += FSE_CHECK_EVERY; grp -= FSE_CHECK_EVERY;
            can = (bs.q >= 24u + 6u * FSE_CHECK_EVERY + 4u) & (grp >= FSE_CHECK_EVERY);
            if (half == 0) ctl_store2(&ctl->pubIters, iters, can ? bs.q + 8u : ((bs.q + 8u) | 0x80000000u));
        }
        TIMING(const unsigned long long tB = __builtin_readcyclecounter(); if (__any(ready)) { tRun += tB - tA; ++nRun; } else { tWait += tB - tA; ++nWait; } tA = tB;);
    }
    }
    TIMING(if (lane == 0) { atomicAdd(&g_decTiming[0], tRun); atomicAdd(&g_decTiming[1], tWait); atomicAdd(&g_decTiming[2], nRun); atomicAdd(&g_decTiming[3], nWait); atomicAdd(&g_decTiming[4], 1ull);
                            atomicAdd(&g_decTiming[13], tBulk0 - tBorn); atomicAdd(&g_decTiming[15], tFin); atomicAdd(&g_decTiming[10], nFin); atomicAdd(&g_decTiming[7], tInner); });
    const u32 sOther = dpp_swap(bs.s);
    const unsigned long long tBulk1 = tA;
    (void)tBulk1;
    if (owner && !half) {
    op = 4 * (long)iters;
    if (iters) {
        const u32 B = 8u * (bs.q + 8u) + bs.bq - 8u * inA;
        const u32 Bh = FAST ? R8 - Phead - 8u * inA : B;
        r.at = (size_t)((Bh + 7u) >> 3) - 8; r.used = 8u * ((u32)r.at + 8u) - B; r.win = ldg64u(in + r.at); s1 = (bs.s - tabOff) >> 1; s2 = (sOther - tabOff) >> 1;
        if (FAST) { s1 = __brev(s1) >> (32u - tl); s2 = __brev(s2) >> (32u - tl); }
    }

    size_t result;
    if (!compact) {
        if ((badMask >> gsl) & 1ull) result = fse_tail(FseCellsRef{cells}, s1, s2, r, out, op, omax, fast);
        else if (FAST)               result = fse_tail(FseCellsRev{A, syms, tl, 5u}, s1, s2, r, out, op, omax, fast);
        else                         result = fse_tail(FseCellsCompact{A, syms}, s1, s2, r, out, op, omax, fast);
    }
    else if (FAST)    result = fse_tail(FseCellsRev{A, syms, tl, 5u}, s1, s2, r, out, op, omax, fast);
    else              result = fse_tail(FseCellsCompact{A, syms}, s1, s2, r, out, op, omax, fast);
    a.results[b] = result;
    TIMING(if (lane == 0) { const unsigned long long tE = __builtin_readcyclecounter(); atomicAdd(&g_decTiming[11], tE - tBorn); atomicAdd(&g_decTiming[12], wall_clock64() - wBorn);
                            atomicAdd(&g_decTiming[14], tE - tBulk1); });
    }
    if (CALLER) fse_scratch_slot_done(a, flagsSh, lane);
}

static void fse_decode_geometry(unsigned ldsLog, size_t ldsBytes, unsigned* slotU32, int* G)
{
    *slotU32 = (FSE_DEC_RING * 8 + FSE_IN_RING + FSE_IN_MIRROR + 16) / 4;
    int g = (int)((ldsBytes - 256) / ((2u << ldsLog) + *slotU32 * 4 + sizeof(DecCtl)));
    if (g > FSE_MAXG) g = FSE_MAXG;
    *G = g;
}
#define FSE_DEC_LDS (FSE_DEC_LDS_KB * 1024)
size_t fse_decode_blocks_per_round(unsigned maxTableLog)
{
    unsigned slot; int G;
    fse_decode_geometry(maxTableLog < FSE_DEC_FAST_MAXLOG ? maxTableLog : FSE_DEC_FAST_MAXLOG, FSE_DEC_LDS, &slot, &G);
    const int cus = dev_props().ok ? dev_props().cus : 256;
    return (size_t)G * FSE_WGS_PER_CU * cus;
}

#define FSE_SYM_SLOT_BYTES (FSE_MAXG * 2048u)
#include <mutex>
namespace {
std::mutex g_symMutex;
struct SymScratch { u8* base = nullptr; u32* bitmap = nullptr; u32 nSlots = 0; };
SymScratch g_symScratch[64];
}
static hipError_t fse_sym_scratch(FseDecArgs& a, hipStream_t s)
{
    int dev = 0;
    hipError_t e = hipGetDevice(&dev);
    if (e != hipSuccess) return e;
    if (dev < 0 || dev >= 64) return hipErrorInvalidDevice;
    std::lock_guard<std::mutex> lock(g_symMutex);
    SymScratch& sc = g_symScratch[dev];
    if (!sc.base && s) {
        hipStreamCaptureStatus st = hipStreamCaptureStatusNone;
        if (hipStreamIsCapturing(s, &st) == hipSuccess && st != hipStreamCaptureStatusNone) return hipErrorStreamCaptureUnsupported;
        (void)hipGetLastError();
    }
    if (!sc.base) {
        const u32 nSlots = 2u * (u32)(dev_props().ok ? dev_props().cus : 256);
        const size_t bitmapBytes = ((nSlots + 31u) / 32u * 4u + 255u) & ~(size_t)255;
        u8* p = nullptr;
        e = hipMalloc((void**)&p, bitmapBytes + (size_t)nSlots * FSE_SYM_SLOT_BYTES);
        if (e != hipSuccess) return e;
        e = hipMemset(p, 0, bitmapBytes);
        if (e != hipSuccess) { (void)hipFree(p); return e; }
        sc.bitmap = (u32*)p; sc.base = p + bitmapBytes; sc.nSlots = nSlots;
    }
    a.symScratch = sc.base; a.slotBitmap = sc.bitmap; a.nSlots = sc.nSlots; a.scratchSlotBytes = FSE_SYM_SLOT_BYTES;
    return hipSuccess;
}

static hipError_t fse_decode_launch(FseDecArgs a, bool rev, hipStream_t s)
{
    const size_t ldsBytes = FSE_DEC_LDS;
    const bool caller = a.atab == nullptr;
    {   hipError_t e = ensure_dyn_lds((const void*)k_fse_decode<true, false, false>, FSE_DEC_LDS);
        if (e == hipSuccess) e = ensure_dyn_lds((const void*)k_fse_decode<false, false, false>, FSE_DEC_LDS);
        if (e == hipSuccess) e = ensure_dyn_lds((const void*)k_fse_decode<true, true, false>, FSE_DEC_LDS);
        if (e == hipSuccess && caller) e = ensure_dyn_lds((const void*)k_fse_decode<true, false, true>, FSE_DEC_LDS);
        if (e == hipSuccess && caller) e = ensure_dyn_lds((const void*)k_fse_decode<false, false, true>, FSE_DEC_LDS);
        if (e == hipSuccess && caller) e = fse_sym_scratch(a, s);
        if (e != hipSuccess) return e;
    }
    fse_decode_geometry(a.ldsLog, ldsBytes, &a.slotU32, &a.G);
    if (a.G < 1) return hipErrorInvalidValue;
    if (caller && ((size_t)a.G << a.ldsLog) > FSE_SYM_SLOT_BYTES) return hipErrorInvalidValue;
    const size_t groups = (a.nBlocks + a.G - 1) / a.G;
    if (a.dstOffsets) {
        if (caller || !a.dstCaps) return hipErrorInvalidValue;
        hipError_t e = ensure_dyn_lds((const void*)k_fse_decode<true, false, false, true>, FSE_DEC_LDS);
        if (e == hipSuccess) e = ensure_dyn_lds((const void*)k_fse_decode<false, false, false, true>, FSE_DEC_LDS);
        if (e != hipSuccess) return e;
        if (rev) hipLaunchKernelGGL((k_fse_decode<true, false, false, true>), dim3((unsigned)groups), dim3(FSE_DEC_THREADS), ldsBytes, s, a);
        else     hipLaunchKernelGGL((k_fse_decode<false, false, false, true>), dim3((unsigned)groups), dim3(FSE_DEC_THREADS), ldsBytes, s, a);
        return hipGetLastError();
    }
    if (caller) {
        if (rev && g_decTimingOn.load(std::memory_order_relaxed)) {
            hipError_t e = ensure_dyn_lds((const void*)k_fse_decode<true, true, true>, FSE_DEC_LDS);
            if (e != hipSuccess) return e;
            hipLaunchKernelGGL((k_fse_decode<true, true, true>), dim3((unsigned)groups), dim3(FSE_DEC_THREADS), ldsBytes, s, a);
        }
        else if (rev) hipLaunchKernelGGL((k_fse_decode<true, false, true>), dim3((unsigned)groups), dim3(FSE_DEC_THREADS), ldsBytes, s, a);
        else     hipLaunchKernelGGL((k_fse_decode<false, false, true>), dim3((unsigned)groups), dim3(FSE_DEC_THREADS), ldsBytes, s, a);
    }
    else if (rev && g_decTimingOn.load(std::memory_order_relaxed)) hipLaunchKernelGGL((k_fse_decode<true, true, false>), dim3((unsigned)groups), dim3(FSE_DEC_THREADS), ldsBytes, s, a);
    else if (rev) hipLaunchKernelGGL((k_fse_decode<true, false, false>), dim3((unsigned)groups), dim3(FSE_DEC_THREADS), ldsBytes, s, a);
    else          hipLaunchKernelGGL((k_fse_decode<false, false, false>), dim3((unsigned)groups), dim3(FSE_DEC_THREADS), ldsBytes, s, a);
    return hipGetLastError();
}

extern "C" __attribute__((visibility("default"))) int FSEHIP_prepareDevice(void)
{
    FseDecArgs a = FseDecArgs();
    return (int)fse_sym_scratch(a, nullptr);
}

extern "C" __attribute__((visibility("default"))) int FSEHIP_debug_decodeTiming(int enable, unsigned long long* out16)
{
    hipError_t e = hipDeviceSynchronize();
    if (e != hipSuccess) return (int)e;
    if (enable) {
        unsigned long long zero[16] = { 0 };
        e = hipMemcpyToSymbol(HIP_SYMBOL(g_decTiming), zero, sizeof(zero));
        g_decTimingOn.store(e == hipSuccess);
        return (int)e;
    }
    g_decTimingOn.store(false);
    if (!out16) return 0;
    e = hipMemcpyFromSymbol(out16, HIP_SYMBOL(g_decTiming), sizeof(g_decTiming));
    if (e != hipSuccess) return (int)e;
    int dev = 0, khz = 0;
    (void)hipGetDevice(&dev);
    (void)hipDeviceGetAttribute(&khz, hipDeviceAttributeClockRate, dev);
    unsigned slot; int G;
    fse_decode_geometry(FSE_DEC_FAST_MAXLOG, FSE_DEC_LDS, &slot, &G);
    out16[8] = (unsigned long long)khz; out16[9] = (unsigned long long)G | ((unsigned long long)FSE_WGS_PER_CU << 32) | ((unsigned long long)FSE_DEC_WAVES << 40) | ((unsigned long long)FSE_CHECK_EVERY << 48);
    return 0;
}

hipError_t launch_fse_decode(FseDecArgs a, hipStream_t s)
{
    if (a.nBlocks == 0) return hipSuccess;
    a.list = nullptr; a.count = nullptr;
    probe_before(PK_FSE_DECODE, s);
    a.ldsLog = a.maxTableLog < FSE_DEC_FAST_MAXLOG ? a.maxTableLog : FSE_DEC_FAST_MAXLOG;
    a.tlMin = 0; a.declineNb0 = 0; a.onlyDeclined = 0;
    hipError_t e = fse_decode_launch(a, true, s);
    if (e == hipSuccess && a.maxTableLog > FSE_DEC_FAST_MAXLOG) {
        a.ldsLog = a.maxTableLog; a.tlMin = FSE_DEC_FAST_MAXLOG + 1; a.declineNb0 = 1;
        e = fse_decode_launch(a, true, s);
        if (e == hipSuccess) { a.tlMin = 0; a.declineNb0 = 0; a.onlyDeclined = 1; e = fse_decode_launch(a, false, s); }
    }
    probe_after(PK_FSE_DECODE, s);
    return e;
}

hipError_t launch_fse_decode_classes(FseDecArgs a, const u32* lists, const u32* counts, hipStream_t s)
{
    if (a.nBlocks == 0) return hipSuccess;
    probe_before(PK_FSE_DECODE, s);
    hipError_t e = hipSuccess;
    for (int c = 0; c < FSE_DCLS_KINDS && e == hipSuccess; ++c) {
        if (c != FSE_DCLS_REV11 && a.maxTableLog <= FSE_DEC_FAST_MAXLOG) break;
        a.list = lists + (size_t)c * FSE_DBINS * a.nBlocks; a.count = counts + c * FSE_DBINS;
        a.ldsLog = c == FSE_DCLS_REV11 ? (a.maxTableLog < FSE_DEC_FAST_MAXLOG ? a.maxTableLog : FSE_DEC_FAST_MAXLOG) : a.maxTableLog;
        e = fse_decode_launch(a, c != FSE_DCLS_PLAIN, s);
    }
    probe_after(PK_FSE_DECODE, s);
    return e;
}
```

### finitestateentropy_amd/csrc/fse_encode.hip

```cpp
#include "internal.h"

#define FSE_ENC_STEP(x, sym, bits, nb)                                                              \
    {   const u32 f2 = tt[2 * (sym)], dn = tt[2 * (sym) + 1];                                        \
        nb = ((x) + dn) >> 16;                                                                       \
        bits = __builtin_amdgcn_ubfe((x), 0u, nb);                                                   \
        (x) = *(const u16*)(ldsb + ((((x) >> nb) << 1) + f2));                                       \
    }

__global__ __launch_bounds__(64) void k_fse_encode(FseEncArgs a)
{
    extern __shared__ __attribute__((aligned(16))) u32 lds[];
    const u8* const ldsb = (const u8*)lds;
    const u32 lane = threadIdx.x;
    const size_t first = (size_t)blockIdx.x * a.G;

    if (a.meta) {
        const size_t bb = first + lane;
        const bool mine = lane < (u32)a.G && bb < a.nBlocks && !fse_enc_skip(a.meta[bb].state, a.onlyState);
        if (!__any(mine)) return;
    }

    for (int g = 0; g < a.G; ++g) {
        const size_t b = first + g;
        if (b >= a.nBlocks) break;
        if (a.meta && fse_enc_skip(a.meta[b].state, a.onlyState)) continue;
        if (a.sizeSplit && view_size(a.src, b) >= FSE_ENC_WAVE_MIN) continue;
        const u32* t = a.ctables + b * a.ctStrideU32;
        const u32 h = t[0];
        const u32 tl = h & 0xFFFFu, msv = (h >> 16) > 255u ? 255u : (h >> 16);
        if (tl > a.maxTableLog) continue;
        const u32 ttStart = 1 + (tl ? (1u << (tl - 1)) : 1u);
        const u32 words = ttStart + 2 * (msv + 1);
        u32* s = lds + (size_t)g * a.slotU32;
        const u32 stOff = (u32)(g * a.slotU32 + 1) * 4u;
        for (u32 i = lane; i < words; i += 64) {
            u32 v = t[i];
            if (i >= ttStart && (((i - ttStart) & 1u) == 0)) v = 2u * v + stOff;
            s[i] = v;
        }
    }
    __syncthreads();
    if (lane >= (u32)a.G) return;
    const size_t b = first + lane;
    if (b >= a.nBlocks) return;
    u32 hdr = 0;
    if (a.meta) { if (fse_enc_skip(a.meta[b].state, a.onlyState)) return; hdr = a.meta[b].hdrSize; }
    if (a.sizeSplit && view_size(a.src, b) >= FSE_ENC_WAVE_MIN) return;

    const u32 h0 = a.ctables[b * a.ctStrideU32];
    const u32 tl = h0 & 0xFFFFu;
    if (tl > a.maxTableLog) {
        a.results[b] = FERR(tableLog_tooLarge);
        return;
    }
    const u32* const tt = lds + (size_t)lane * a.slotU32 + 1 + (tl ? (1u << (tl - 1)) : 1u);

    const u8* const sbase = a.src.offsets ? a.src.base + a.src.offsets[b] : a.src.base + first * a.src.stride;
    const u32 soff = a.src.offsets ? 0u : lane * (u32)a.src.stride;
    u8* const dbase = a.dst + first * a.dstStride;
    const u32 doff = lane * (u32)a.dstStride + hdr;
    const size_t n64 = view_size(a.src, b);
    const size_t cap64 = a.dstCapacity - hdr;

    size_t csize = 0;
    if (n64 >= ((size_t)1 << 31)) { a.results[b] = FERR(srcSize_wrong); return; }
    const u32 n = (u32)n64;
    if (n > 2 && cap64 > 8) {
        const u32 lim = (u32)(cap64 - 8);
        u64 acc = 0; u32 nacc = 0, pos = 0;
#define FSE_FLUSH()                                                                                  \
        {   __builtin_memcpy(dbase + (doff + pos), &acc, 8);                                          \
            const u32 nby = nacc >> 3;                                                                \
            pos += nby; pos = pos > lim ? lim : pos;                                                  \
            acc >>= (nby << 3); nacc &= 7u; }
        u32 xa, xb;
        {   const u32 s0 = sbase[soff + n - 1], s1 = sbase[soff + n - 2];
            const u32 f0 = tt[2 * s0], d0 = tt[2 * s0 + 1], f1 = tt[2 * s1], d1 = tt[2 * s1 + 1];
            const u32 n0 = (d0 + (1u << 15)) >> 16, n1 = (d1 + (1u << 15)) >> 16;
            xa = *(const u16*)(ldsb + (((((n0 << 16) - d0) >> n0) << 1) + f0));
            xb = *(const u16*)(ldsb + (((((n1 << 16) - d1) >> n1) << 1) + f1));
        }
        u32 idx = n - 2;
        bool swapped = false;
        while (idx > 0 && (((uintptr_t)(sbase + soff) + idx) & 15u)) {
            const u32 sym = sbase[soff + idx - 1];
            u32 bits, nb;
            FSE_ENC_STEP(xa, sym, bits, nb)
            acc |= (u64)bits << nacc; nacc += nb;
            FSE_FLUSH()
            const u32 tsw = xa; xa = xb; xb = tsw; swapped = !swapped;
            --idx;
        }
        if (idx >= 16) {
            uint4 cur = *(const uint4*)(sbase + (soff + idx - 16));
            while (idx >= 16) {
                const u32 nidx = idx - 16;
                const uint4 nxt = *(const uint4*)(sbase + (soff + (nidx >= 16 ? nidx - 16 : nidx)));
                u32 ba, na, bb, nbb;
#define FSE_PAIR(w, hiA, hiB)                                                                        \
                {   const u32 sa = __builtin_amdgcn_ubfe(w, hiA, 8u), sb = __builtin_amdgcn_ubfe(w, hiB, 8u); \
                    FSE_ENC_STEP(xa, sa, ba, na)                                                      \
                    FSE_ENC_STEP(xb, sb, bb, nbb)                                                     \
                    acc |= (u64)(ba | (bb << na)) << nacc; nacc += na + nbb; }
                FSE_PAIR(cur.w, 24u, 16u) FSE_PAIR(cur.w, 8u, 0u) FSE_FLUSH()
                FSE_PAIR(cur.z, 24u, 16u) FSE_PAIR(cur.z, 8u, 0u) FSE_FLUSH()
                FSE_PAIR(cur.y, 24u, 16u) FSE_PAIR(cur.y, 8u, 0u) FSE_FLUSH()
                FSE_PAIR(cur.x, 24u, 16u) FSE_PAIR(cur.x, 8u, 0u) FSE_FLUSH()
                cur = nxt;
                idx = nidx;
            }
        }
        while (idx > 0) {
            const u32 sym = sbase[soff + idx - 1];
            u32 bits, nb;
            FSE_ENC_STEP(xa, sym, bits, nb)
            acc |= (u64)bits << nacc; nacc += nb;
            FSE_FLUSH()
            const u32 tsw = xa; xa = xb; xb = tsw; swapped = !swapped;
            --idx;
        }
        if (swapped) { const u32 tsw = xa; xa = xb; xb = tsw; }
        const u32 c2 = (n & 1) ? xb : xa, c1 = (n & 1) ? xa : xb;
        acc |= (u64)(c2 & ((1u << tl) - 1u)) << nacc; nacc += tl; FSE_FLUSH()
        acc |= (u64)(c1 & ((1u << tl) - 1u)) << nacc; nacc += tl; FSE_FLUSH()
        acc |= (u64)1 << nacc; nacc += 1; FSE_FLUSH()
        csize = (pos >= lim) ? 0 : (size_t)pos + (nacc > 0);
#undef FSE_FLUSH
#undef FSE_PAIR
    }
    if (a.meta) {
        size_t r = 0;
        if (csize != 0 && (size_t)hdr + csize < n64 - 1) r = (size_t)hdr + csize;
        a.results[b] = r;
    } else a.results[b] = csize;
}

#define FSE_ENC_LDS (80 * 1024)
static void fse_encode_geometry(unsigned maxTableLog, unsigned* slotU32, int* G)
{
    *slotU32 = (1 + (1u << (maxTableLog - 1)) + 512) | 1u;
    int g = (int)(FSE_ENC_LDS / (*slotU32 * 4));
    if (g > 64) g = 64;
    *G = g;
}
size_t fse_encode_blocks_per_round(unsigned maxTableLog)
{
    unsigned slot; int G;
    fse_encode_geometry(maxTableLog, &slot, &G);
    const int cus = dev_props().ok ? dev_props().cus : 256;
    return (size_t)G * 2 * cus;
}

hipError_t launch_fse_encode(FseEncArgs a, hipStream_t s)
{
    if (a.nBlocks == 0) return hipSuccess;
    const size_t ldsBytes = FSE_ENC_LDS;
    {   const hipError_t e = ensure_dyn_lds((const void*)k_fse_encode, (int)ldsBytes); if (e != hipSuccess) return e; }
    fse_encode_geometry(a.maxTableLog, &a.slotU32, &a.G);
    if (a.nBlocks > 1 && ((a.src.stride > 0x3FFFFFFu) || (a.dstStride > 0x3FFFFFFu))) a.G = 1;
    if (a.dstCapacity > 0x7FFFFFF0u) a.dstCapacity = 0x7FFFFFF0u;
    const size_t groups = (a.nBlocks + a.G - 1) / a.G;
    probe_before(PK_FSE_ENCODE, s);
    hipLaunchKernelGGL(k_fse_encode, dim3((unsigned)groups), dim3(64), ldsBytes, s, a);
    probe_after(PK_FSE_ENCODE, s);
    return hipGetLastError();
}
```

### finitestateentropy_amd/csrc/fse_encode_wave.hip

```cpp
#include "internal.h"

#ifndef FSE_WV_WARM_FACTOR
#define FSE_WV_WARM_FACTOR 2u
#endif
#define FSE_WV_WARM_MIN 64u
#define FSE_WV_WARM_MAX 4096u

typedef const __attribute__((address_space(3))) u16* wv_lds_u16;
typedef const __attribute__((address_space(3))) u32* wv_lds_u32;
typedef u32 wv_u32x2 __attribute__((ext_vector_type(2)));
typedef const __attribute__((address_space(3))) wv_u32x2* wv_lds_u64;
DEV u32 wv_lds_addr(const void* p) { return (u32)(uintptr_t)(const __attribute__((address_space(3))) u8*)p; }
template <bool TT4>
DEV void wv_step(u32& st, u32 ttb, u32 sym, u32& nb)
{
    if (TT4) {
        const u32 e = *(wv_lds_u32)(uintptr_t)(ttb + 4u * sym);
        nb = (st + (e & 0xFFFFu)) >> 12;
        st = *(wv_lds_u16)(uintptr_t)(((st >> nb) + (u32)((int)e >> 16)) << 1);
    } else {
        const wv_u32x2 e = *(wv_lds_u64)(uintptr_t)(ttb + 8u * sym);
        nb = (st + e.y) >> 16;
        st = *(wv_lds_u16)(uintptr_t)(((st >> nb) << 1) + e.x);
    }
// ... 75 lines not shown
        while (j + 64 <= jb) {
            const u32 nj = j + 64;
            const u8* const q = src + (n - 64 - (nj + 64 <= jb ? nj : j));
            const uint4 n0 = wv_load16(q), n1 = wv_load16(q + 16), n2 = wv_load16(q + 32), n3 = wv_load16(q + 48);
            __asm__ volatile("" ::: "memory");
            WV_QUAD(c3) WV_QUAD(c2) WV_QUAD(c1) WV_QUAD(c0)
            c0 = n0; c1 = n1; c2 = n2; c3 = n3; j = nj;
        }
    }
    while (j + 16 <= jb) {
        const uint4 c = wv_load16(src + (n - 16 - j));
        WV_QUAD(c)
        j += 16;
    }
#undef WV_QUAD
#undef WV_PAIR
    for (; j < jb; ++j) {
        const u32 sym = src[n - 1 - j];
        u32 nb, b1;
        if (j & 1u) { WV_STEP_BITS(xb, sym, nb, b1) } else { WV_STEP_BITS(xa, sym, nb, b1) }
        k.push(b1, nb);
    }
}

enum { WV_CK_NONE = 0, WV_CK_RECORD = 1, WV_CK_MERGE = 2 };
#define WV_CK_MAX 8u
struct WvCk { uint2* slot; u32 every, left, idx, total; u32 d; bool merged; };
template <bool TT4, int CK>
DEV void wv_chain(u32 ttb, const u8* src, u32 n, u32 ja, u32 jb, u32 c, u32& x, u32& bits, WvCk* ck = nullptr)
{
    u32 j = ja;
    const u32 shHi = 24u - 8u * c, shLo = 8u - 8u * c;
#define WV_CSTEP(w, sh) { const u32 sy = __builtin_amdgcn_ubfe(w, sh, 8u); u32 nb; WV_STEP(x, sy, nb) bits += nb; }
#define WV_CQUAD(v) WV_CSTEP(v.w, shHi) WV_CSTEP(v.w, shLo) WV_CSTEP(v.z, shHi) WV_CSTEP(v.z, shLo) WV_CSTEP(v.y, shHi) WV_CSTEP(v.y, shLo) WV_CSTEP(v.x, shHi) WV_CSTEP(v.x, shLo)
    if (j + 64 <= jb) {
        const u8* p = src + (n - 64 - j);
        uint4 c0 = wv_load16(p), c1 = wv_load16(p + 16), c2 = wv_load16(p + 32), c3 = wv_load16(p + 48);
        while (j + 64 <= jb) {
            const u32 nj = j + 64;
            const u8* const q = src + (n - 64 - (nj + 64 <= jb ? nj : j));
            const uint4 n0 = wv_load16(q), n1 = wv_load16(q + 16), n2 = wv_load16(q + 32), n3 = wv_load16(q + 48);
            __asm__ volatile("" ::: "memory");
            WV_CQUAD(c3) WV_CQUAD(c2) WV_CQUAD(c1) WV_CQUAD(c0)
            c0 = n0; c1 = n1; c2 = n2; c3 = n3; j = nj;
            if (CK != WV_CK_NONE && --ck->left == 0) {
                ck->left = ck->every;
                if (CK == WV_CK_MERGE && ck->idx < WV_CK_MAX) {
                    const uint2 o = ck->slot[ck->idx];
                    if (o.x == x) {
                        const u32 d = bits - o.y;
                        for (u32 i = ck->idx; i < ck->total && i < WV_CK_MAX; ++i) ck->slot[i].y += d;
                        ck->d = d; ck->merged = true;
                        return;
                    }
                }
                if (ck->idx < WV_CK_MAX) ck->slot[ck->idx] = make_uint2(x, bits);
                ++ck->idx;
            }
        }
    }
    while (j + 16 <= jb) {
        const uint4 v = wv_load16(src + (n - 16 - j));
        WV_CQUAD(v)
        j += 16;
    }
#undef WV_CQUAD
#undef WV_CSTEP
    for (j += c; j < jb; j += 2) { u32 nb; WV_STEP(x, (u32)src[n - 1 - j], nb) bits += nb; }
}

template <bool TT4>
DEV u32 wv_init_state(u32 ttb, u32 sym)
{
    if (TT4) {
        const u32 e = *(wv_lds_u32)(uintptr_t)(ttb + 4u * sym);
        const u32 d = e & 0xFFFFu, nb = (d >> 12) + 1u, msp = (nb << 12) - d;
        return *(wv_lds_u16)(uintptr_t)(((msp >> nb) + (u32)((int)e >> 16)) << 1);
    }
    const wv_u32x2 e = *(wv_lds_u64)(uintptr_t)(ttb + 8u * sym);
    const u32 nb = (e.y + (1u << 15)) >> 16;
    return *(wv_lds_u16)(uintptr_t)(((((nb << 16) - e.y) >> nb) << 1) + e.x);
}

template <bool TT4>
DEV size_t wv_serial(u32 ttb, const u8* src, u32 n, u8* dst, size_t cap, u32 tl)
{
    const u32 lim = (u32)(cap - 8);
    u64 acc = 0; u32 nacc = 0, pos = 0;
    u32 xa = wv_init_state<TT4>(ttb, src[n - 1]), xb = wv_init_state<TT4>(ttb, src[n - 2]);
    for (u32 j = 2; j < n; ++j) {
        const u32 sym = src[n - 1 - j];
        u32 nb, bits;
        if (j & 1u) { WV_STEP_BITS(xb, sym, nb, bits) } else { WV_STEP_BITS(xa, sym, nb, bits) }
        acc |= (u64)bits << nacc; nacc += nb;
        if (nacc >= 32u || j + 1 == n) {
            __builtin_memcpy(dst + pos, &acc, 8);
            const u32 nby = nacc >> 3; pos += nby; pos = pos > lim ? lim : pos; acc >>= (nby << 3); nacc &= 7u;
        }
    }
    const u32 c2 = (n & 1u) ? xb : xa, c1 = (n & 1u) ? xa : xb, mask = (1u << tl) - 1u;
#define WV_FLUSH() { __builtin_memcpy(dst + pos, &acc, 8); const u32 nby = nacc >> 3; pos += nby; pos = pos > lim ? lim : pos; acc >>= (nby << 3); nacc &= 7u; }
    acc |= (u64)(c2 & mask) << nacc; nacc += tl; WV_FLUSH()
    acc |= (u64)(c1 & mask) << nacc; nacc += tl; WV_FLUSH()
    acc |= (u64)1 << nacc; nacc += 1; WV_FLUSH()
#undef WV_FLUSH
    return (pos >= lim) ? 0 : (size_t)pos + (nacc > 0);
}

#ifdef FSE_ENC_TIMING
__device__ unsigned long long g_encTiming[4096 * 8];
extern "C" __attribute__((visibility("default"))) int FSEHIP_debug_encTiming(unsigned long long* host) { return (int)hipMemcpyFromSymbol(host, HIP_SYMBOL(g_encTiming), sizeof(g_encTiming)); }
#define ETIMING(x) x
#else
#define ETIMING(x)
#endif

#define FSE_WV_WAVES 1
#ifndef WV_LANES
#define WV_LANES 32u
#endif
#define WV_BPW (64u / WV_LANES)
template <bool TT4>
__global__ __launch_bounds__(64 * FSE_WV_WAVES) void k_fse_encode_wave(FseEncArgs a, u32 slotWords, u32 tableWords)
{
    ETIMING(unsigned long long T0 = __builtin_readcyclecounter(); unsigned long long T1 = 0; unsigned long long T2 = 0; unsigned long long T3 = 0; unsigned long long T4 = 0; u32 rounds = 0; u32 nBad0 = 0; u32 firstBad = 99;)
    extern __shared__ __attribute__((aligned(16))) u32 ldsAll[];
    const u32 lane = threadIdx.x & 63u, wv = threadIdx.x >> 6;
    const u32 part = lane / WV_LANES, hl = lane % WV_LANES;
    const u32 partBase = lane - hl;
    const u32 slot = wv * WV_BPW + part;
    u32* const lds = ldsAll + slot * slotWords;
    const u32 ldsOff = wv_lds_addr(ldsAll) + slot * slotWords * 4u;
    const size_t pos = ((size_t)blockIdx.x * FSE_WV_WAVES + wv) * WV_BPW + part;

    size_t b = pos;
    bool on = pos < a.nBlocks;
    if (a.list) {
        size_t q = pos; int i = 0;
        for (; i < FSE_EBINS; ++i) { const u32 c = a.count[i]; if (q < c) break; q -= c; }
        on = i < FSE_EBINS;
        b = on ? (size_t)a.list[(size_t)i * a.nBlocks + q] : 0;
    }
    u32 hdr = 0;
    if (on && a.meta) { if (fse_enc_skip(a.meta[b].state, a.onlyState)) on = false; else hdr = a.meta[b].hdrSize; }
    const u32* const gct = a.ctables + (on ? b : 0) * a.ctStrideU32;
    u32 tl = 0, msv = 0;
    if (on) {
        const u32 h0 = gct[0];
        tl = h0 & 0xFFFFu; msv = (h0 >> 16) > 255u ? 255u : (h0 >> 16);
        if (tl > a.maxTableLog) { if (hl == 0) a.results[b] = FERR(tableLog_tooLarge); on = false; }
    }
    const u8* const src = on ? view_ptr(a.src, b) : nullptr;
    const size_t n64 = on ? view_size(a.src, b) : 0;
    u8* const dst = a.dst + (on ? b : 0) * a.dstStride + hdr;
    const size_t cap = a.dstCapacity - hdr;
    if (on && a.sizeSplit && n64 < FSE_ENC_WAVE_MIN) on = false;
    if (on && n64 >= ((size_t)1 << 31)) { if (hl == 0) a.results[b] = FERR(srcSize_wrong); on = false; }
    const u32 n = (u32)n64;
    if (on && (n <= 2 || cap <= 8)) { if (hl == 0) a.results[b] = 0; on = false; }
    if (on && tl == 0) {
        if (hl == 0) { dst[0] = 1; a.results[b] = a.meta ? (((size_t)hdr + 1 < n64 - 1) ? (size_t)hdr + 1 : 0) : 1; }
        on = false;
    }

    const u32 ttStart = 1 + (tl ? (1u << (tl - 1)) : 1u);
    const u32 ttAl = (ttStart + 1u) & ~1u;
    u32 presentLane = 0;
    if (on) {
        for (u32 i = hl; i < ttStart; i += WV_LANES) lds[i] = gct[i];
        for (u32 sy = hl; sy <= msv; sy += WV_LANES) {
            const u32 dfs = gct[ttStart + 2 * sy], dnb = gct[ttStart + 2 * sy + 1];
            presentLane += dnb != ((tl + 1) << 16) - (1u << tl);
            if (TT4) {
                const u32 mbo = (dnb >> 16) + 1u, msp = (mbo << 16) - dnb;
                lds[ttAl + sy] = (((mbo << 12) - msp) & 0xFFFFu) | ((dfs + 2u + (ldsOff >> 1)) << 16);
            } else {
                lds[ttAl + 2 * sy] = 2u * dfs + 4u + ldsOff;
                lds[ttAl + 2 * sy + 1] = dnb;
            }
        }
    }
    u32 present = presentLane;
#pragma unroll
    for (int off = (int)WV_LANES / 2; off > 0; off >>= 1) present += (u32)__shfl_xor((int)present, off, WAVE);
    u32 warm = (FSE_WV_WARM_FACTOR << tl) / (present ? present : 1u);
    warm = (warm + 63u) & ~63u;
    warm = warm < FSE_WV_WARM_MIN ? FSE_WV_WARM_MIN : (warm > FSE_WV_WARM_MAX ? FSE_WV_WARM_MAX : warm);
    __builtin_amdgcn_fence(__ATOMIC_ACQ_REL, "wavefront");
    u32 ttb = ldsOff + 4u * ttAl;
    __asm__("" : "+v"(ttb));
    u32* const ringBase = lds + tableWords;
    ETIMING(T1 = __builtin_readcyclecounter();)

    const u32 m = on ? n - 2 : 0u;
    u32 C = (m + WV_LANES - 1u) / WV_LANES;
    C = m >= 4096u ? (C + 63u) & ~63u : (C + 1u) & ~1u;
    C = C ? C : 2u;
    const u32 delta = m >= 4096u ? (u32)((0 - ((uintptr_t)src + n - 2u)) & 62u) : 0u;
    const u32 lo0 = hl ? 2 + hl * C - delta : 2u, hi0 = 2 + (hl + 1) * C - delta;
    const u32 j0 = lo0 < n ? lo0 : n;
    const u32 j1 = (hl == WV_LANES - 1u || hi0 > n) ? n : hi0;
    const bool mine = on && j0 < n;
    const u32 lastLane = m ? ((m + delta - 1) / C < WV_LANES - 1u ? (m + delta - 1) / C : WV_LANES - 1u) : 0u;

    const u32 cc = hl & 1u, kk = hl >> 1;
    const u32 sLo0 = kk ? 2 + 2u * kk * C - delta : 2u, sMid0 = 2 + (2u * kk + 1u) * C - delta, sHi0 = 2 + (2u * kk + 2u) * C - delta;
    const u32 sLo = sLo0 < n ? sLo0 : n, sMid = sMid0 < n ? sMid0 : n;
    const u32 sHi = (2u * kk + 2u >= WV_LANES || sHi0 > n) ? n : sHi0;
    const bool mineC = on && sLo < n;
    WvCk ck; ck.slot = (uint2*)(ringBase + hl * (WV_RING / 4)); ck.merged = false; ck.d = 0; ck.idx = 0;
    ck.every = (2u * C / 64u + WV_CK_MAX - 1u) / WV_CK_MAX; ck.every = ck.every ? ck.every : 1u;
    if (C & 63u) ck.every = 0x7FFFFFFFu;
    ck.left = ck.every; ck.total = (2u * C / 64u) / ck.every;
    u32 cstart = 0, cmid = 0, cend = 0, bitsLo = 0, bitsTot = 0;
    if (mineC) {
        u32 x, scratch = 0;
        if (sLo <= 2 + warm) {
            x = wv_init_state<TT4>(ttb, src[n - 1 - cc]);
            wv_chain<TT4, WV_CK_NONE>(ttb, src, n, 2, sLo, cc, x, scratch);
        } else {
            x = 1u << tl;
            wv_chain<TT4, WV_CK_NONE>(ttb, src, n, sLo - warm, sLo, cc, x, scratch);
        }
        cstart = x;
        u32 lo = sLo, hi = sMid, nbits = 0;
#pragma nounroll
        for (int piece = 0; piece < 2; ++piece) {
            wv_chain<TT4, WV_CK_RECORD>(ttb, src, n, lo, hi, cc, x, nbits, &ck);
            if (piece == 0) { cmid = x; bitsLo = nbits; }
            lo = sMid; hi = sHi;
        }
        cend = x; bitsTot = nbits;
    }
    ETIMING(T2 = __builtin_readcyclecounter();)
#ifndef WV_SAMPLE_CACHE
#define WV_SAMPLE_CACHE 1
#endif
    u32 oStart = 0xFFFFFFFFu, oEnd = 0, oMid = 0, oLo = 0, oTot = 0;
    u32 rEnd = cend, rMid = cmid, rLo = bitsLo, rTot = bitsTot;
    for (;;) {
        u32 prevEnd; bool bad;
        for (;;) {
            prevEnd = (u32)__shfl_up((int)cend, 2, WAVE);
            bad = mineC && kk > 0 && cstart != prevEnd;
            const bool hit = WV_SAMPLE_CACHE && bad && oStart == prevEnd;
            if (!__any(hit)) break;
            if (hit) {
                u32 t;
                t = cstart; cstart = oStart; oStart = t;  t = cend; cend = oEnd; oEnd = t;  t = cmid; cmid = oMid; oMid = t;
                t = bitsLo; bitsLo = oLo; oLo = t;  t = bitsTot; bitsTot = oTot; oTot = t;
            }
        }
        if (!__any(bad)) break;
        ETIMING(if (rounds == 0) { const unsigned long long bm = __ballot(bad); nBad0 = (u32)__builtin_popcountll(bm); firstBad = (u32)__builtin_ctzll(bm); })
        if (bad) {
            oStart = cstart; oEnd = cend; oMid = cmid; oLo = bitsLo; oTot = bitsTot;
            cstart = prevEnd; cend = rEnd; cmid = rMid; bitsLo = rLo; bitsTot = rTot;
            u32 x = cstart, lo = sLo, hi = sMid, nbits = 0;
            ck.merged = false; ck.idx = 0; ck.left = ck.every;
            bool midDone = false;
#pragma nounroll
            for (int piece = 0; piece < 2 && !ck.merged; ++piece) {
                wv_chain<TT4, WV_CK_MERGE>(ttb, src, n, lo, hi, cc, x, nbits, &ck);
                if (piece == 0 && !ck.merged) { cmid = x; bitsLo = nbits; midDone = true; }
                lo = sMid; hi = sHi;
            }
            if (ck.merged) {
                if (!midDone) bitsLo += ck.d;
                bitsTot += ck.d;
            } else { cend = x; bitsTot = nbits; }
            rEnd = cend; rMid = cmid; rLo = bitsLo; rTot = bitsTot;
        }
        ETIMING(++rounds;)
    }
    ETIMING(T3 = __builtin_readcyclecounter();)
    u32 start, bits;
    {   const int la = (int)(partBase + (hl & ~1u)), lb = la + 1;
        const u32 sA = (u32)__shfl((int)cstart, la, WAVE), sB = (u32)__shfl((int)cstart, lb, WAVE);
        const u32 mA = (u32)__shfl((int)cmid, la, WAVE), mB = (u32)__shfl((int)cmid, lb, WAVE);
        const u32 lA = (u32)__shfl((int)bitsLo, la, WAVE), lB = (u32)__shfl((int)bitsLo, lb, WAVE);
        const u32 tA = (u32)__shfl((int)bitsTot, la, WAVE), tB = (u32)__shfl((int)bitsTot, lb, WAVE);
        start = cc ? (mA | (mB << 16)) : (sA | (sB << 16));
        bits = cc ? (tA - lA) + (tB - lB) : lA + lB;
    }
    u32 xa = 0, xb = 0;

    u32 incl = bits;
#pragma unroll
    for (int off = 1; off < (int)WV_LANES; off <<= 1) { const u32 o = (u32)__shfl_up((int)incl, off, WAVE); if ((int)hl >= off) incl += o; }
    const u32 excl = incl - bits;
    const u64 bodyBits = (u32)__shfl((int)incl, (int)(partBase + WV_LANES - 1u), WAVE);

    const u64 totalBits = bodyBits + 2u * tl + 1u;
    const size_t whole = (size_t)(totalBits >> 3);
    size_t csize = (whole >= cap - 8) ? 0 : (size_t)((totalBits + 7) >> 3);
    size_t result = csize;
    if (a.meta) result = (csize != 0 && (size_t)hdr + csize < n64 - 1) ? (size_t)hdr + csize : 0;
    if (on && result == 0) { if (hl == 0) a.results[b] = 0; on = false; }

    {   const unsigned long long thin = __ballot(on && mine && hl < lastLane && bits < 8u);
        const unsigned long long partMask = (WV_LANES == 64u ? ~0ull : ((1ull << (WV_LANES & 63u)) - 1ull)) << partBase;
        if (on && (thin & partMask)) {
            if (a.meta && a.onlyState == FSE_ENC_PAR) {
                if (hl == 0) const_cast<FseMeta*>(a.meta)[b].state = FSE_ENC_LANE;
            } else if (hl == 0) {
                const size_t cs = wv_serial<TT4>(ttb, src, n, dst, cap, tl);
                a.results[b] = a.meta ? ((cs != 0 && (size_t)hdr + cs < n64 - 1) ? (size_t)hdr + cs : 0) : cs;
            }
            on = false;
        }
    }
    u32 tail = 0;
    if (on && mine) {
        WvSink k;
        const u32 lead = (u32)((uintptr_t)dst & (WV_RING - 1));
        const u32 off0 = lead + (excl >> 3);
        k.dstAl = dst - lead; k.ring = ringBase + hl * (WV_RING / 4); k.ringA = wv_lds_addr(k.ring);
        k.woff = off0 & ~3u; k.done = off0; k.acc = 0; k.nacc = 8u * (off0 & 3u) + (excl & 7u);
        xa = start & 0xFFFFu; xb = start >> 16;
        wv_emit<TT4>(ttb, src, n, j0, j1, xa, xb, k);
        if (hl == lastLane) {
            const u32 c2 = (n & 1u) ? xb : xa, c1 = (n & 1u) ? xa : xb;
            const u32 mask = (1u << tl) - 1u;
            k.push(c2 & mask, tl);
            k.push(c1 & mask, tl);
            k.push(1u, 1u);
            k.nacc = (k.nacc + 7u) & ~7u;
        }
        k.ring[(k.woff & (WV_RING - 1)) >> 2] = k.acc;
        k.copy_out(k.woff + (k.nacc >> 3));
        tail = k.acc >> (k.nacc & ~7u);
    }
    const u32 prevTail = (u32)__shfl_up((int)tail, 1, WAVE);
    if (on && mine && hl > 0 && (excl & 7u)) {
        u8* const p = dst + (excl >> 3);
        const uintptr_t ad = (uintptr_t)p;
        atomicOr((u32*)(ad & ~(uintptr_t)3), prevTail << (8u * (u32)(ad & 3u)));
    }
    ETIMING(T4 = __builtin_readcyclecounter(); if (hl == 0 && b < 4096) { unsigned long long* t = g_encTiming + 8 * b; t[0] = T1 - T0; t[1] = T2 - T1; t[2] = T3 - T2; t[3] = T4 - T3; t[4] = rounds; t[5] = nBad0; t[6] = firstBad; })
    if (on && hl == 0) a.results[b] = result;
}

__global__ __launch_bounds__(64) void k_fse_enc_lists(FseEncArgs a)
{
    const size_t b = (size_t)blockIdx.x * 64 + threadIdx.x;
    const u32 lane = threadIdx.x;
    int bin = -1;
    if (b < a.nBlocks && a.meta[b].state == FSE_ENC_PAR) { const u32 p = a.meta[b].pace; bin = (int)(p < FSE_EBINS ? p : FSE_EBINS - 1); }
    const unsigned long long below = (1ull << lane) - 1ull;
    for (int c = 0; c < FSE_EBINS; ++c) {
        const unsigned long long mask = __ballot(bin == c);
        if (!mask) continue;
        const int leader = __builtin_ctzll(mask);
        u32 base = 0;
        if ((int)lane == leader) base = atomicAdd(&a.count[c], (u32)__builtin_popcountll(mask));
        base = (u32)__shfl((int)base, leader, WAVE);
        if (bin == c) a.list[(size_t)c * a.nBlocks + base + (u32)__builtin_popcountll(mask & below)] = (u32)b;
    }
}
hipError_t launch_fse_enc_lists(const FseEncArgs& a, hipStream_t s)
{
    if (a.nBlocks == 0) return hipSuccess;
    const hipError_t e = launch_zero_u32(a.count, FSE_EBINS, s);
    if (e != hipSuccess) return e;
    hipLaunchKernelGGL(k_fse_enc_lists, dim3((unsigned)((a.nBlocks + 63) / 64)), dim3(64), 0, s, a);
    return hipGetLastError();
}

hipError_t launch_fse_encode_wave(FseEncArgs a, hipStream_t s)
{
    if (a.nBlocks == 0) return hipSuccess;
    const bool tt4 = a.maxTableLog <= 11;
    const u32 tableWords = (2 + (1u << (a.maxTableLog - 1)) + (tt4 ? 256 : 512) + 2 + 31) & ~31u;
#ifndef WV_EXTRA_LDS_WORDS
#define WV_EXTRA_LDS_WORDS 0u
#endif
    const u32 slotWords = tableWords + WV_LANES * (WV_RING / 4) + WV_EXTRA_LDS_WORDS;
    const size_t ldsBytes = 4 * (size_t)slotWords * WV_BPW * FSE_WV_WAVES;
    const size_t perGroup = (size_t)WV_BPW * FSE_WV_WAVES;
    probe_before(PK_FSE_ENCODE_WAVE, s);
    const dim3 grid((unsigned)((a.nBlocks + perGroup - 1) / perGroup));
    if (tt4) hipLaunchKernelGGL(k_fse_encode_wave<true>, grid, dim3(64 * FSE_WV_WAVES), ldsBytes, s, a, slotWords, tableWords);
    else     hipLaunchKernelGGL(k_fse_encode_wave<false>, grid, dim3(64 * FSE_WV_WAVES), ldsBytes, s, a, slotWords, tableWords);
    probe_after(PK_FSE_ENCODE_WAVE, s);
    return hipGetLastError();
}
```

### finitestateentropy_amd/csrc/fse_tables.hip

```cpp
#include "internal.h"

#include "wave_glue.h"
#include "ncount_reader.h"
#include "fse_wave_build.h"

template <u32 MAXC>
DEV void fse_wave_build_ctable(const WaveBuildLds& w, const int nn[4], u32 maxSV, u32 tl, u32* img, u32 lane)
{
    u16* const cumAll = w.cumP;
    *(uint2*)(w.nrm + 4 * lane) = make_uint2(((u32)nn[0] & 0xFFFFu) | ((u32)nn[1] << 16), ((u32)nn[2] & 0xFFFFu) | ((u32)nn[3] << 16));
    __syncthreads();
    const u32 ts = 1u << tl;
    u16* const stateTable = (u16*)(img + 1);
    u32* const tt = img + 1 + (ts >> 1);
    {
        u32 eff[4], laneSum = 0;
#pragma unroll
        for (int i = 0; i < 4; ++i) { eff[i] = nn[i] == -1 ? 1u : (u32)nn[i]; laneSum += eff[i]; }
        u32 total;
        u32 run = wb_scan_excl(laneSum, lane, &total);
#pragma unroll
        for (int i = 0; i < 4; ++i) {
            const u32 s = 4 * lane + i;
            cumAll[s] = (u16)run;
            if (s <= maxSV) {
                if (nn[i] == 0) { tt[2 * s] = 0; tt[2 * s + 1] = ((tl + 1) << 16) - ts; }
                else if (nn[i] == -1 || nn[i] == 1) { tt[2 * s] = run - 1u; tt[2 * s + 1] = (tl << 16) - ts; }
                else {
                    const u32 maxBitsOut = tl - hibit32((u32)nn[i] - 1);
                    tt[2 * s] = run - (u32)nn[i];
                    tt[2 * s + 1] = (maxBitsOut << 16) - ((u32)nn[i] << maxBitsOut);
                }
            }
            run += eff[i];
        }
        if (lane == 0) img[0] = tl | (maxSV << 16);
    }
    __syncthreads();
    wave_spread_rank<MAXC>(w, maxSV, tl, lane, [&](u32 s) { return (u32)cumAll[s]; },
                     [&](u32 u, u32 s, u32 r, u32 first) { (void)s; stateTable[first + r] = (u16)(ts + u); });
}

template <u32 MAXC>
__global__ __launch_bounds__(64) void k_fse_cprep(FseCPrepArgs a, u32 capTs)
{
    extern __shared__ __attribute__((aligned(16))) u8 wbLds[];
    const size_t b = blockIdx.x;
    const u32 lane = threadIdx.x;
    const size_t n = view_size(a.src, b);
    FseMeta m; m.state = 0; m.hdrSize = 0; m.tableLog = 0; m.maxSV = 0; m.pace = 0;
    const size_t top = a.histResults[b];
    size_t result = 0; bool go = false;
    if (n <= 1) result = 0;
    else if (is_err(top)) result = top;
    else if (top == n) result = 1;
    else if (top == 1 || top < (n >> 7)) result = 0;
    else go = true;
    const WaveBuildLds w = wave_build_carve(wbLds, capTs, true);
    u32* const hdrImg = w.cnt;
    u32 maxSV = 0, tl = 0;
    int nn[4] = { 0, 0, 0, 0 };
    if (go) {
        maxSV = a.maxSVs[b];
        tl = wg_optimal_tablelog(a.tableLogReq, n, maxSV, 2);
        if ((1u << tl) > 64u * MAXC || (1u << tl) > capTs) { result = FERR(tableLog_tooLarge); go = false; }
    }
    if (go) {
        const uint4 cv = ((const uint4*)(a.counts + b * 256))[lane];
        const u32 c[4] = { cv.x, cv.y, cv.z, cv.w };
        for (u32 i = lane; i < 136; i += 64) hdrImg[i] = 0;
        const size_t e = wg_normalize<64>(nn, c, (u64)n, maxSV, tl, lane);
        if (is_err(e)) { result = e; go = false; }
    }
    __syncthreads();
    if (go) {
        const size_t h = wg_write_ncount<64>(hdrImg, a.dstCapacity, nn, maxSV, tl, lane);
        if (is_err(h)) { result = h; go = false; }
        else m.hdrSize = (u32)h;
    }
    __syncthreads();
    if (!go) { if (lane == 0) { a.meta[b] = m; a.results[b] = result; } return; }
    {   u8* const dst = a.dst + b * a.dstStride;
        const u8* const hb = (const u8*)hdrImg;
        for (u32 i = lane; i < m.hdrSize; i += 64) dst[i] = hb[i];
    }
    int top1 = nn[0] > nn[1] ? nn[0] : nn[1]; top1 = nn[2] > top1 ? nn[2] : top1; top1 = nn[3] > top1 ? nn[3] : top1;
    top1 = wave_max_i32(top1);
    m.state = ((u32)top1 * 64u > (63u << tl) || n < FSE_ENC_WAVE_MIN) ? FSE_ENC_LANE : FSE_ENC_PAR;
    {
        u32 present = (nn[0] != 0) + (nn[1] != 0) + (nn[2] != 0) + (nn[3] != 0);
        present = wg_sum<64>(present);
        const u32 mix = (1u << tl) / (present ? present : 1u);
        m.pace = mix < 64u ? 0u : mix < 128u ? 1u : mix < 256u ? 2u : 3u;
    }
    m.tableLog = tl; m.maxSV = maxSV;
    if (lane == 0) a.meta[b] = m;
    fse_wave_build_ctable<MAXC>(w, nn, maxSV, tl, a.ctables + b * a.ctStrideU32, lane);
}

__global__ __launch_bounds__(64) void k_fse_dparse(FseDPrepArgs a)
{
    __shared__ __attribute__((aligned(16))) u32 stage[NCS_WORDS];
    const size_t b0 = (size_t)blockIdx.x * 64, b = b0 + threadIdx.x;
    const u32 lane = threadIdx.x;
    const bool have = b < a.nBlocks;
    const u8* const in = have ? view_ptr(a.csrc, b) : nullptr;
    const size_t cSize = have ? view_size(a.csrc, b) : 0;
    bool done = false;
    if (have && a.rawRle) { const size_t orig = a.origSizes ? a.origSizes[b] : a.uniformOrig; done = cSize == orig || cSize == 1; }
    const u32 staged = ncount_stage(stage, in, cSize, lane, have && !done);
    {   uint4* const rows = (uint4*)(a.norms + b0 * 256);
        const u32 nRows = a.nBlocks - b0 < 64 ? (u32)(a.nBlocks - b0) : 64u;
        for (u32 i = lane; i < nRows * 32u; i += 64) rows[i] = make_uint4(0, 0, 0, 0);
    }
    __syncthreads();
    int cls = -1;
    if (have) {
        FseMeta m; m.state = 0; m.hdrSize = 0; m.tableLog = 0; m.maxSV = 0; m.pace = 0; m.pace = 0;
        size_t result = 0;
        if (!done) do {
            u32 tl = 0, maxSV = 255;
            s16* const norm = a.norms + b * 256;
            const size_t h = ncount_read_staged(norm, &maxSV, &tl, stage + lane, staged, in, cSize);
            if (is_err(h)) { result = h; break; }
            if (tl > a.maxLog) { result = FERR(tableLog_tooLarge); break; }
            cls = FSE_DCLS_REV11;
            if (tl > FSE_DEC_FAST_MAXLOG) {
                int top = 0;
                for (u32 i = 0; i <= maxSV >> 3; ++i) {
                    const uint4 v = ((const uint4*)norm)[i];
                    const u32 q[4] = { v.x, v.y, v.z, v.w };
#pragma unroll
                    for (int k = 0; k < 4; ++k) { const int lo = (s16)(q[k] & 0xFFFFu), hi = (s16)(q[k] >> 16); top = lo > top ? lo : top; top = hi > top ? hi : top; }
                }
                cls = 2 * top > (1 << tl) ? FSE_DCLS_PLAIN : FSE_DCLS_REV12;
            }
            m.state = 1u | ((u32)cls << 2); m.hdrSize = (u32)h; m.tableLog = tl; m.maxSV = maxSV;
        } while (0);
        a.meta[b] = m;
        if (m.state == 0 && !done) a.results[b] = result;
    }
    if (cls >= 0) { const size_t bin = view_size(a.csrc, b) >> FSE_DBIN_LOG; cls = cls * FSE_DBINS + (int)(bin < FSE_DBINS - 1 ? bin : FSE_DBINS - 1); }
    const unsigned long long below = (1ull << lane) - 1ull;
    unsigned long long todo = __ballot(cls >= 0);
    while (todo) {
        const int leader = __builtin_ctzll(todo);
        const int c = __shfl(cls, leader, WAVE);
        const unsigned long long mask = __ballot(cls == c);
        u32 base = 0;
        if ((int)lane == leader) {
            base = atomicAdd(&a.counts[c], (u32)__builtin_popcountll(mask));
            atomicAdd(&a.counts[FSE_DCLS_COUNT + c / FSE_DBINS], (u32)__builtin_popcountll(mask));
        }
        base = (u32)__shfl((int)base, leader, WAVE);
        if (cls == c) a.lists[(size_t)c * a.nBlocks + base + (u32)__builtin_popcountll(mask & below)] = (u32)b;
        todo &= ~mask;
    }
}

template <u32 MAXC>
__global__ __launch_bounds__(64) void k_fse_dbuild(FseDPrepArgs a, u32 capTs, int firstList, int nLists, u32 ldsCapTs)
{
    extern __shared__ __attribute__((aligned(16))) u8 wbLds[];
    {   u32 total = 0;
        for (int k = firstList / (int)FSE_DBINS; k < (firstList + nLists) / (int)FSE_DBINS; ++k) total += a.counts[FSE_DCLS_COUNT + k];
        if (blockIdx.x >= total) return;
    }
    constexpr int MAXL = 2 * FSE_DBINS;
    static_assert(FSE_DBINS % 4 == 0, "the list lengths are read as 16-byte vectors");
    uint4 cv[MAXL / 4];
#pragma unroll
    for (int i = 0; i < MAXL / 4; ++i) cv[i] = 4 * i < nLists ? ((const uint4*)(a.counts + firstList))[i] : make_uint4(0, 0, 0, 0);
    u32 idx = blockIdx.x;
    int c = firstList + nLists;
    {   u32 before = 0; bool found = false;
#pragma unroll
        for (int i = 0; i < MAXL; ++i) {
            const uint4 v = cv[i >> 2];
            const u32 n = (i & 3) == 0 ? v.x : (i & 3) == 1 ? v.y : (i & 3) == 2 ? v.z : v.w;
            const bool here = !found & (i < nLists) & (idx < before + n);
            c = here ? firstList + i : c; idx = here ? idx - before : idx;
            found |= here;
            before += n;
        }
    }
    if (c == firstList + nLists) return;
    const size_t b = a.lists[(size_t)c * a.nBlocks + idx];
    const u32 lane = threadIdx.x;
    const FseMeta m = a.meta[b];
    if (m.state == 0) return;
    const u32 tl = m.tableLog, ts = 1u << tl;
    if (ts > ldsCapTs || ts > 64u * MAXC) {
        if (lane == 0) { a.meta[b].state = 0; a.results[b] = FERR(tableLog_tooLarge); }
        return;
    }
    const WaveBuildLds w = wave_build_carve(wbLds, ldsCapTs, false);
    *(uint2*)(w.nrm + 4 * lane) = *(const uint2*)(a.norms + b * 256 + 4 * lane);
    __syncthreads();
    const bool rev = ((m.state >> 2) & 3u) != FSE_DCLS_PLAIN;
    u16* const A = a.atab + b * capTs;
    u8* const S = a.symtab + b * capTs;
    const bool fast = wave_spread_rank<MAXC>(w, m.maxSV, tl, lane, [&](u32 s) { return (u32)(int)w.nrm[s]; }, [&](u32 u, u32 s, u32 r, u32 nrm) {
        const int n = (int)nrm;
        const u32 next = (n > 0 ? (u32)n : 1u) + r;
        const u32 nb = tl - hibit32(next);
        const u32 ns = (next << nb) - ts;
        const u32 x = rev ? __brev(u) >> (32u - tl) : u;
        A[x] = rev ? (u16)(nb | ((__brev(ns) >> (32u - tl)) << 5)) : (u16)((ns & 0xFFFu) | (nb << 12));
        S[x] = (u8)s;
    });
    if (lane == 0) a.meta[b].state = m.state | (fast ? 2u : 0u);
}

__global__ __launch_bounds__(256) void k_fse_export_dtable(FseDPrepArgs a, u32 capTs, u32* dtables, size_t dtStrideU32)
{
    const size_t b = blockIdx.x;
    const FseMeta m = a.meta[b];
    if (m.state == 0) return;
    const u32 tl = m.tableLog, ts = 1u << tl;
    const bool rev = ((m.state >> 2) & 3u) != FSE_DCLS_PLAIN;
    const u16* const A = a.atab + b * capTs;
    const u8* const S = a.symtab + b * capTs;
    u32* const dt = dtables + b * dtStrideU32;
    if (threadIdx.x == 0) dt[0] = tl | ((m.state & 2u) ? 1u << 16 : 0u);
    for (u32 x = threadIdx.x; x < ts; x += blockDim.x) {
        const u32 i = rev ? __brev(x) >> (32u - tl) : x;
        const u32 c = A[i];
        const u32 nb = rev ? (c & 31u) : (c >> 12);
        const u32 ns = rev ? __brev(c >> 5) >> (32u - tl) : (c & 0xFFFu);
        dt[1 + x] = ns | ((u32)S[i] << 16) | (nb << 24);
    }
}
hipError_t launch_fse_export_dtables(const FseDPrepArgs& a, u32* dtables, size_t dtStrideU32, hipStream_t s)
{
    if (a.nBlocks == 0) return hipSuccess;
    hipLaunchKernelGGL(k_fse_export_dtable, dim3((unsigned)a.nBlocks), dim3(256), 0, s, a, 1u << a.maxLog, dtables, dtStrideU32);
    return hipGetLastError();
}

DEV size_t fse_norm_load_checked(int nn[4], const s16* nb, u32 maxSV, u32 tl, u32 maxTl, u32 lane)
{
    if (maxSV > 255u) return FERR(maxSymbolValue_tooLarge);
    if (tl > maxTl) return FERR(tableLog_tooLarge);
    if (tl == 0 || tl == 1 || tl == 3) return FERR(GENERIC);
    u32 cells = 0; bool bad = false;
#pragma unroll
    for (int i = 0; i < 4; ++i) {
        nn[i] = 4 * lane + i <= maxSV ? (int)nb[4 * lane + i] : 0;
        bad |= nn[i] < -1;
        cells += nn[i] == -1 ? 1u : nn[i] > 0 ? (u32)nn[i] : 0u;
    }
    cells = wg_sum<64>(cells);
    return (wg_any<64>(bad, lane) || cells != (1u << tl)) ? FERR(GENERIC) : 0;
}
template <u32 MAXC>
__global__ __launch_bounds__(64) void k_fse_ctable_from_norm(const s16* norms, size_t normStride, const u32* maxSVs, u32 tl, u32* ctables, size_t ctStrideU32,
                                                            size_t* results, u32 capTs)
{
    extern __shared__ __attribute__((aligned(16))) u8 wbLds[];
    const size_t b = blockIdx.x;
    const u32 lane = threadIdx.x;
    const u32 maxSV = maxSVs[b];
    int nn[4] = { 0, 0, 0, 0 };
    static_assert(MAXC == 32 || MAXC == 64, "64 * MAXC cells = a table of tableLog 11 or 12");
    const size_t r = fse_norm_load_checked(nn, norms + b * normStride, maxSV, tl, MAXC == 32 ? 11u : FSE_MAX_TL, lane);
    if (lane == 0) results[b] = r;
    if (is_err(r)) return;
    fse_wave_build_ctable<MAXC>(wave_build_carve(wbLds, capTs, true), nn, maxSV, tl, ctables + b * ctStrideU32, lane);
}
hipError_t launch_fse_ctable_from_norm(const s16* norms, size_t normStride, const u32* maxSVs, u32 tl, u32* ctables, size_t ctStrideU32, size_t* results,
                                       size_t nBlocks, hipStream_t s)
{
    if (nBlocks == 0) return hipSuccess;
    const u32 capTs = 1u << (tl >= 1 && tl <= FSE_MAX_TL ? tl : FSE_MAX_TL);
    if (wb_small(capTs))
        hipLaunchKernelGGL(k_fse_ctable_from_norm<32>, dim3((unsigned)nBlocks), dim3(64), wave_build_lds_bytes(capTs, true), s, norms, normStride, maxSVs, tl, ctables,
                           ctStrideU32, results, capTs);
    else
        hipLaunchKernelGGL(k_fse_ctable_from_norm<64>, dim3((unsigned)nBlocks), dim3(64), wave_build_lds_bytes(capTs, true), s, norms, normStride, maxSVs, tl, ctables,
                           ctStrideU32, results, capTs);
    return hipGetLastError();
}

static void launch_fse_dbuild_lists(const FseDPrepArgs& a, u32 capTs, int firstList, int nLists, u32 ldsCapTs, hipStream_t s)
{
    if (wb_small(ldsCapTs))
        hipLaunchKernelGGL(k_fse_dbuild<32>, dim3((unsigned)a.nBlocks), dim3(64), wave_build_lds_bytes(ldsCapTs, false), s, a, capTs, firstList, nLists, ldsCapTs);
    else
        hipLaunchKernelGGL(k_fse_dbuild<64>, dim3((unsigned)a.nBlocks), dim3(64), wave_build_lds_bytes(ldsCapTs, false), s, a, capTs, firstList, nLists, ldsCapTs);
}
static void launch_fse_dbuilds(const FseDPrepArgs& a, hipStream_t s)
{
    const u32 capTs = 1u << a.maxLog;
    const u32 capA = a.maxLog < FSE_DEC_FAST_MAXLOG ? capTs : (1u << FSE_DEC_FAST_MAXLOG);
    launch_fse_dbuild_lists(a, capTs, (int)FSE_DCLS_REV11 * FSE_DBINS, (int)FSE_DBINS, capA, s);
    if (a.maxLog > FSE_DEC_FAST_MAXLOG) launch_fse_dbuild_lists(a, capTs, (int)FSE_DCLS_REV12 * FSE_DBINS, 2 * (int)FSE_DBINS, capTs, s);
}

__global__ __launch_bounds__(64) void k_fse_dmeta_from_norm(FseDPrepArgs a, const s16* norms, size_t normStride, const u32* maxSVs, u32 tl)
{
    const size_t b = blockIdx.x;
    const u32 lane = threadIdx.x;
    const u32 maxSV = maxSVs[b];
    int nn[4] = { 0, 0, 0, 0 };
    const size_t r = fse_norm_load_checked(nn, norms + b * normStride, maxSV, tl, a.maxLog, lane);
    FseMeta m; m.state = 0; m.hdrSize = 0; m.tableLog = tl; m.maxSV = maxSV; m.pace = 0;
    if (!is_err(r)) {
        *(uint2*)(a.norms + b * 256 + 4 * lane) = make_uint2(((u32)nn[0] & 0xFFFFu) | ((u32)nn[1] << 16), ((u32)nn[2] & 0xFFFFu) | ((u32)nn[3] << 16));
        int top = nn[0] > nn[1] ? nn[0] : nn[1]; top = nn[2] > top ? nn[2] : top; top = nn[3] > top ? nn[3] : top;
        top = wave_max_i32(top);
        const u32 cls = tl <= FSE_DEC_FAST_MAXLOG ? (u32)FSE_DCLS_REV11 : 2 * top > (1 << tl) ? (u32)FSE_DCLS_PLAIN : (u32)FSE_DCLS_REV12;
        m.state = 1u | (cls << 2);
        if (lane == 0) {
            const u32 at = atomicAdd(&a.counts[cls * FSE_DBINS], 1u);
            atomicAdd(&a.counts[FSE_DCLS_COUNT + cls], 1u);
            a.lists[(size_t)cls * FSE_DBINS * a.nBlocks + at] = (u32)b;
        }
    }
    if (lane == 0) { a.meta[b] = m; if (is_err(r)) a.results[b] = r; }
}
hipError_t launch_fse_dprep_from_norm(const FseDPrepArgs& a, const s16* norms, size_t normStride, const u32* maxSVs, u32 tl, hipStream_t s)
{
    if (a.nBlocks == 0) return hipSuccess;
    hipError_t e = launch_zero_u32(a.counts, FSE_DCLS_COUNT + FSE_DCLS_KINDS, s);
    if (e != hipSuccess) return e;
    hipLaunchKernelGGL(k_fse_dmeta_from_norm, dim3((unsigned)a.nBlocks), dim3(64), 0, s, a, norms, normStride, maxSVs, tl);
    launch_fse_dbuilds(a, s);
    return hipGetLastError();
}

#ifdef FSE_WB_TIMING
extern "C" __attribute__((visibility("default"))) int FSEHIP_debug_wbTiming(unsigned long long* host) { return (int)hipMemcpyFromSymbol(host, HIP_SYMBOL(g_wbTiming), sizeof(g_wbTiming)); }
#endif
__global__ __launch_bounds__(64) void k_fse_glue_normalize(s16* norms, size_t normStride, u32 tlReq, const u32* counts, size_t countStride,
                                                          const size_t* totals, const u32* maxSVs, size_t* results)
{
    const size_t b = blockIdx.x;
    const u32 lane = threadIdx.x;
    const u32 maxSV = maxSVs[b] > 255u ? 255u : maxSVs[b];
    const u32* const cb = counts + b * countStride;
    u32 c[4];
#pragma unroll
    for (int i = 0; i < 4; ++i) c[i] = 4 * lane + i <= maxSV ? cb[4 * lane + i] : 0u;
    int nn[4] = { 0, 0, 0, 0 };
    const u32 tl = tlReq ? tlReq : FSE_DEF_TL;
    const u64 total = (u64)totals[b];
    size_t r = total ? wg_normalize<64>(nn, c, total, maxSV, tl, lane) : FERR(GENERIC);
    if (!is_err(r)) r = tl;
    s16* const nb = norms + b * normStride;
#pragma unroll
    for (int i = 0; i < 4; ++i) if (4 * lane + i <= maxSV && !is_err(r)) nb[4 * lane + i] = (s16)nn[i];
    if (lane == 0) results[b] = r;
}

__global__ __launch_bounds__(64) void k_fse_glue_write_ncount(u8* headers, size_t headerStride, size_t headerCapacity, const s16* norms, size_t normStride,
                                                             const u32* maxSVs, u32 tl, size_t* results)
{
    __shared__ u32 img[136];
    const size_t b = blockIdx.x;
    const u32 lane = threadIdx.x;
    const u32 maxSV = maxSVs[b];
    size_t r;
    if (tl > FSE_MAX_TL) r = FERR(tableLog_tooLarge);
    else if (tl < FSE_MIN_TL || maxSV > 255u) r = FERR(GENERIC);
    else {
        const s16* const nb = norms + b * normStride;
        int nn[4];
#pragma unroll
        for (int i = 0; i < 4; ++i) nn[i] = 4 * lane + i <= maxSV ? (int)nb[4 * lane + i] : 0;
        for (u32 i = lane; i < 136; i += 64) img[i] = 0;
        __syncthreads();
        r = wg_write_ncount<64>(img, headerCapacity, nn, maxSV, tl, lane);
        __syncthreads();
        if (!is_err(r)) {
            u8* const dst = headers + b * headerStride;
            const u8* const hb = (const u8*)img;
            for (u32 i = lane; i < (u32)r; i += 64) dst[i] = hb[i];
        }
    }
    if (lane == 0) results[b] = r;
}

__global__ __launch_bounds__(64) void k_fse_glue_read_ncount(s16* norms, size_t normStride, u32* maxSVs, u32* tableLogs, BlockView headers, size_t nBlocks, size_t* results)
{
    const size_t b = (size_t)blockIdx.x * 64 + threadIdx.x;
    if (b >= nBlocks) return;
    u32 maxSV = maxSVs[b], tl = 0;
    size_t r;
    if ((size_t)maxSV >= normStride) r = FERR(maxSymbolValue_tooLarge);
    else r = ncount_read<1>(norms + b * normStride, &maxSV, &tl, view_ptr(headers, b), view_size(headers, b));
    if (!is_err(r)) { maxSVs[b] = maxSV; tableLogs[b] = tl; }
    results[b] = r;
}

hipError_t launch_fse_glue_normalize(s16* norms, size_t normStride, u32 tl, const u32* counts, size_t countStride, const size_t* totals, const u32* maxSVs,
                                     size_t* results, size_t nBlocks, hipStream_t s)
{
    if (nBlocks == 0) return hipSuccess;
    hipLaunchKernelGGL(k_fse_glue_normalize, dim3((unsigned)nBlocks), dim3(64), 0, s, norms, normStride, tl, counts, countStride, totals, maxSVs, results);
    return hipGetLastError();
}
hipError_t launch_fse_glue_write_ncount(u8* headers, size_t headerStride, size_t headerCapacity, const s16* norms, size_t normStride, const u32* maxSVs, u32 tl,
                                        size_t* results, size_t nBlocks, hipStream_t s)
{
    if (nBlocks == 0) return hipSuccess;
    hipLaunchKernelGGL(k_fse_glue_write_ncount, dim3((unsigned)nBlocks), dim3(64), 0, s, headers, headerStride, headerCapacity, norms, normStride, maxSVs, tl, results);
    return hipGetLastError();
}
hipError_t launch_fse_glue_read_ncount(s16* norms, size_t normStride, u32* maxSVs, u32* tableLogs, const BlockView& headers, size_t* results, size_t nBlocks, hipStream_t s)
{
    if (nBlocks == 0) return hipSuccess;
    hipLaunchKernelGGL(k_fse_glue_read_ncount, dim3((unsigned)((nBlocks + 63) / 64)), dim3(64), 0, s, norms, normStride, maxSVs, tableLogs, headers, nBlocks, results);
    return hipGetLastError();
}

hipError_t launch_fse_cprep(const FseCPrepArgs& a, hipStream_t s)
{
    if (a.nBlocks == 0) return hipSuccess;
    const u32 capTs = 1u << a.maxTl;
    const size_t ldsBytes = wave_build_lds_bytes(capTs, true);
    probe_before(PK_FSE_CPREP, s);
    if (wb_small(capTs)) hipLaunchKernelGGL(k_fse_cprep<32>, dim3((unsigned)a.nBlocks), dim3(64), ldsBytes, s, a, capTs);
    else hipLaunchKernelGGL(k_fse_cprep<64>, dim3((unsigned)a.nBlocks), dim3(64), ldsBytes, s, a, capTs);
    probe_after(PK_FSE_CPREP, s);
    return hipGetLastError();
}
hipError_t launch_fse_dprep(const FseDPrepArgs& a, hipStream_t s)
{
    if (a.nBlocks == 0) return hipSuccess;
    hipError_t e = launch_zero_u32(a.counts, FSE_DCLS_COUNT + FSE_DCLS_KINDS, s);
    if (e != hipSuccess) return e;
    probe_before(PK_FSE_DPREP, s);
    hipLaunchKernelGGL(k_fse_dparse, dim3((unsigned)((a.nBlocks + 63) / 64)), dim3(64), 0, s, a);
    launch_fse_dbuilds(a, s);
    probe_after(PK_FSE_DPREP, s);
    return hipGetLastError();
}
```

### finitestateentropy_amd/csrc/hist.hip

```cpp
#include "internal.h"

#define HIST_SEG (1u << 28)

#ifndef HIST_COLS_LOG
#define HIST_COLS_LOG 4
#endif
#define HIST_COLS (1u << HIST_COLS_LOG)
#ifndef HIST_GROUP
#define HIST_GROUP 4
#endif
DEV void hist_add(u32* cnt, u32 col, u32 byte)
{
    atomicAdd(&cnt[(byte << HIST_COLS_LOG) | col], 1u);
}
DEV void hist_add4(u32* cnt, u32 col, u32 w)
{
    hist_add(cnt, col, w & 0xFFu);
    hist_add(cnt, col, (w >> 8) & 0xFFu);
    hist_add(cnt, col, (w >> 16) & 0xFFu);
    hist_add(cnt, col, w >> 24);
}
DEV void hist_add16(u32* cnt, u32 col, const uint4& v)
{
    hist_add4(cnt, col, v.x); hist_add4(cnt, col, v.y); hist_add4(cnt, col, v.z); hist_add4(cnt, col, v.w);
}

__global__ __launch_bounds__(64) void k_hist(HistArgs a)
{
    __shared__ __attribute__((aligned(16))) u32 cnt[256 * HIST_COLS];
    const u32 lane = threadIdx.x;
    const u32 col = lane & (HIST_COLS - 1u);
    const size_t b = blockIdx.x;
    const u8* const p = view_ptr(a.src, b);
    const size_t n = view_size(a.src, b);
    const unsigned limitIn = (a.maxSVs && !a.useUniformIn) ? a.maxSVs[b] : a.uniformMaxSV;
    const bool checked = limitIn < 255u && !a.trustInput;
    const unsigned nOut = limitIn < 255u ? limitIn + 1u : 256u;

    u32 t0 = 0, t1 = 0, t2 = 0, t3 = 0;

    for (size_t seg = 0; seg < n; seg += HIST_SEG) {
        for (u32 i = lane; i < sizeof(cnt) / 16u; i += 64u) ((uint4*)cnt)[i] = make_uint4(0, 0, 0, 0);
        __syncthreads();
        const u8* q = p + seg;
        const size_t len = (n - seg) < (size_t)HIST_SEG ? (n - seg) : (size_t)HIST_SEG;
        size_t head = (size_t)((0 - (uintptr_t)q) & 15u);
        if (head > len) head = len;
        if (lane < head) hist_add(cnt, col, q[lane]);
        const uint4* v = (const uint4*)(q + head);
        const size_t nvec = (len - head) >> 4;
        size_t i = lane;
        constexpr size_t HG = HIST_GROUP;
        if (i + 64 * (HG - 1) < nvec) {
            uint4 x[HG];
#pragma unroll
            for (size_t g = 0; g < HG; ++g) x[g] = v[i + 64 * g];
            for (;;) {
                const size_t j = i + 64 * HG;
                const bool more = j + 64 * (HG - 1) < nvec;
                uint4 y[HG];
#pragma unroll
                for (size_t g = 0; g < HG; ++g) y[g] = x[g];
                if (more) {
#pragma unroll
                    for (size_t g = 0; g < HG; ++g) y[g] = v[j + 64 * g];
                }
                __asm__ volatile("" ::: "memory");
#pragma unroll
                for (size_t g = 0; g < HG; ++g) hist_add16(cnt, col, x[g]);
                i = j;
                if (!more) break;
#pragma unroll
                for (size_t g = 0; g < HG; ++g) x[g] = y[g];
            }
        }
        for (; i < nvec; i += 64) { const uint4 x = v[i]; hist_add16(cnt, col, x); }
        const size_t done = head + (nvec << 4);
        if (lane < len - done) hist_add(cnt, col, q[done + lane]);
        __syncthreads();
        u32 s0 = 0, s1 = 0, s2 = 0, s3 = 0;
#pragma unroll 8
        for (u32 c = 0; c < HIST_COLS; ++c) {
            const u32 cc = (c + lane) & (HIST_COLS - 1u);
            s0 += cnt[(lane << HIST_COLS_LOG) | cc]; s1 += cnt[((lane + 64u) << HIST_COLS_LOG) | cc];
            s2 += cnt[((lane + 128u) << HIST_COLS_LOG) | cc]; s3 += cnt[((lane + 192u) << HIST_COLS_LOG) | cc];
        }
        t0 += s0; t1 += s1; t2 += s2; t3 += s3;
        __syncthreads();
    }

    u32 best = t0 > t1 ? t0 : t1; best = t2 > best ? t2 : best; best = t3 > best ? t3 : best;
    int top = -1;
    if (t0) top = (int)lane;
    if (t1) top = (int)lane + 64;
    if (t2) top = (int)lane + 128;
    if (t3) top = (int)lane + 192;
    best = wave_max_u32(best);
    top = wave_max_i32(top);

    if (n == 0) {
        for (u32 s = lane; s < nOut; s += 64) a.counts[b * 256 + s] = 0;
        if (lane == 0) { if (a.maxSVs) a.maxSVs[b] = 0; a.results[b] = 0; }
        return;
    }
    if (checked && (unsigned)top > limitIn) {
        if (lane == 0) a.results[b] = FERR(maxSymbolValue_tooSmall);
        return;
    }
    unsigned* out = a.counts + b * 256;
    if (lane < nOut) out[lane] = t0;
    if (lane + 64 < nOut) out[lane + 64] = t1;
    if (lane + 128 < nOut) out[lane + 128] = t2;
    if (lane + 192 < nOut) out[lane + 192] = t3;
    if (lane == 0) { if (a.maxSVs) a.maxSVs[b] = (unsigned)top; a.results[b] = (size_t)best; }
}

__global__ __launch_bounds__(1024) void k_hist_fold(const unsigned* __restrict__ part, size_t nPart, unsigned limitIn, int checked, size_t n,
                                                   unsigned* count, unsigned* maxSV, size_t* result)
{
    __shared__ u32 sums[4][256];
    __shared__ u32 wbest[4];
    __shared__ int wtop[4];
    const u32 t = threadIdx.x, sym = t & 255u, q = t >> 8;
    u32 acc = 0;
    for (size_t p = q; p < nPart; p += 4) acc += part[p * 256 + sym];
    sums[q][sym] = acc;
    __syncthreads();
    if (t >= 256) return;
    const u32 c = sums[0][t] + sums[1][t] + sums[2][t] + sums[3][t];
    const u32 best = wave_max_u32(c);
    const int top = wave_max_i32(c ? (int)t : -1);
    if ((t & 63u) == 0) { wbest[t >> 6] = best; wtop[t >> 6] = top; }
    __syncthreads();
    u32 b = wbest[0]; int tp = wtop[0];
    for (int w = 1; w < 4; ++w) { b = wbest[w] > b ? wbest[w] : b; tp = wtop[w] > tp ? wtop[w] : tp; }
    const unsigned nOut = limitIn < 255u ? limitIn + 1u : 256u;
    if (checked && (unsigned)tp > limitIn) { if (t == 0) *result = FERR(maxSymbolValue_tooSmall); return; }
    (void)n;
    if (t < nOut) count[t] = c;
    if (t == 0) { *maxSV = (unsigned)tp; *result = (size_t)b; }
}

hipError_t launch_hist_large(const u8* d_src, size_t n, unsigned limitIn, int trustInput, unsigned* d_part, unsigned* d_count, unsigned* d_maxSV,
                             size_t* d_result, size_t* d_scratchResults, hipStream_t s)
{
    const size_t nFull = n / HIST_PIECE, tail = n % HIST_PIECE, nPart = nFull + (tail ? 1 : 0);
    HistArgs a;
    a.counts = d_part; a.maxSVs = nullptr; a.uniformMaxSV = 255; a.useUniformIn = 1; a.trustInput = 1; a.results = d_scratchResults;
    a.src = BlockView{d_src, HIST_PIECE, nullptr, HIST_PIECE, nullptr}; a.nBlocks = nFull;
    hipError_t e = launch_hist(a, s);
    if (e != hipSuccess) return e;
    if (tail) {
        a.counts = d_part + nFull * 256; a.results = d_scratchResults + nFull;
        a.src = BlockView{d_src + nFull * HIST_PIECE, tail, nullptr, tail, nullptr}; a.nBlocks = 1;
        e = launch_hist(a, s);
        if (e != hipSuccess) return e;
    }
    hipLaunchKernelGGL(k_hist_fold, dim3(1), dim3(1024), 0, s, (const unsigned*)d_part, nPart, limitIn, (int)(limitIn < 255u && !trustInput), n,
                       d_count, d_maxSV, d_result);
    return hipGetLastError();
}

__global__ __launch_bounds__(64) void k_zero_u32(u32* p, u32 n)
{
    for (u32 i = blockIdx.x * 64u + threadIdx.x; i < n; i += gridDim.x * 64u) p[i] = 0;
}
hipError_t launch_zero_u32(u32* p, u32 n, hipStream_t s)
{
    if (n == 0) return hipSuccess;
    const u32 groups = (n + 63u) / 64u;
    hipLaunchKernelGGL(k_zero_u32, dim3(groups < 1024u ? groups : 1024u), dim3(64), 0, s, p, n);
    return hipGetLastError();
}

hipError_t launch_hist(const HistArgs& a, hipStream_t s)
{
    if (a.nBlocks == 0) return hipSuccess;
    probe_before(PK_HIST, s);
    hipLaunchKernelGGL(k_hist, dim3((unsigned)a.nBlocks), dim3(64), 0, s, a);
    probe_after(PK_HIST, s);
    return hipGetLastError();
}
```

### finitestateentropy_amd/csrc/internal.h

```cpp
#pragma once
#include "dev_common.h"

#define CK(x) do { hipError_t e__ = (x); if (e__ != hipSuccess) return (int)e__; } while (0)
static inline size_t align_up(size_t v, size_t a) { return (v + a - 1) / a * a; }

static inline BlockView mkview(const void* base, size_t stride, const size_t* sizes, size_t uniform)
{
    BlockView v; v.base = (const u8*)base; v.stride = stride; v.sizes = sizes; v.uniform = uniform; v.offsets = nullptr; return v;
}
static inline BlockView subview(const BlockView& v, size_t b0)
{
    BlockView r = v;
    if (v.offsets) r.offsets = v.offsets + b0; else r.base = v.base + b0 * v.stride;
    r.sizes = v.sizes ? v.sizes + b0 : nullptr;
    return r;
}

struct HistArgs {
    unsigned* counts;
    unsigned* maxSVs;
    unsigned uniformMaxSV;
    int useUniformIn;
    int trustInput = 0;
    size_t* results;
    BlockView src;
    size_t nBlocks;
};
hipError_t launch_hist(const HistArgs& a, hipStream_t s);
#define HIST_PIECE ((size_t)65536)
#define HIST_LARGE_MIN ((size_t)262144)
hipError_t launch_hist_large(const u8* d_src, size_t n, unsigned limitIn, int trustInput, unsigned* d_part, unsigned* d_count, unsigned* d_maxSV,
                             size_t* d_result, size_t* d_scratchResults, hipStream_t s);
hipError_t launch_zero_u32(u32* p, u32 n, hipStream_t s);

struct FseMeta {
    u32 state;
    u32 hdrSize;
    u32 tableLog;
    u32 maxSV;
    u32 pace;
};

struct FseCPrepArgs {
    const unsigned* counts;
    const unsigned* maxSVs;
    const size_t* histResults;
    BlockView src;
    u8* dst; size_t dstStride; size_t dstCapacity;
    unsigned maxSVReq, tableLogReq;
    u32* ctables; size_t ctStrideU32;
    unsigned maxTl;
    FseMeta* meta;
    size_t* results;
    size_t nBlocks;
};
hipError_t launch_fse_cprep(const FseCPrepArgs& a, hipStream_t s);
hipError_t launch_fse_glue_normalize(s16* norms, size_t normStride, u32 tl, const u32* counts, size_t countStride, const size_t* totals, const u32* maxSVs,
                                     size_t* results, size_t nBlocks, hipStream_t s);
hipError_t launch_fse_glue_write_ncount(u8* headers, size_t headerStride, size_t headerCapacity, const s16* norms, size_t normStride, const u32* maxSVs, u32 tl,
                                        size_t* results, size_t nBlocks, hipStream_t s);
hipError_t launch_fse_glue_read_ncount(s16* norms, size_t normStride, u32* maxSVs, u32* tableLogs, const BlockView& headers, size_t* results, size_t nBlocks, hipStream_t s);
hipError_t launch_fse_ctable_from_norm(const s16* norms, size_t normStride, const u32* maxSVs, u32 tl, u32* ctables, size_t ctStrideU32, size_t* results,
                                       size_t nBlocks, hipStream_t s);

struct FseEncArgs {
    u8* dst; size_t dstStride; size_t dstCapacity;
    size_t* results;
    BlockView src;
    const u32* ctables; size_t ctStrideU32;
    const FseMeta* meta;
    unsigned maxTableLog;
    int G;
    unsigned slotU32;
    size_t nBlocks;
    unsigned onlyState;
    unsigned sizeSplit;
    u32* list; u32* count;
};
enum { FSE_EBINS = 4 };
enum { FSE_ENC_PAR = 1, FSE_ENC_LANE = 2 };
#define FSE_ENC_WAVE_MIN 2048u
__host__ __device__ inline bool fse_enc_skip(unsigned state, unsigned onlyState) { return state == 0 || (onlyState != 0 && state != onlyState); }
hipError_t launch_fse_encode(FseEncArgs a, hipStream_t s);
size_t fse_encode_blocks_per_round(unsigned maxTableLog);
hipError_t launch_fse_encode_wave(FseEncArgs a, hipStream_t s);
hipError_t launch_fse_enc_lists(const FseEncArgs& a, hipStream_t s);
inline hipError_t launch_fse_encode_auto(FseEncArgs a, hipStream_t s)
{
    a.onlyState = 0; a.sizeSplit = 0;
    const bool ragged = a.src.sizes || a.src.offsets;
    if (a.dstCapacity > 0x7FFFFFF0u || (!ragged && a.src.uniform < FSE_ENC_WAVE_MIN)) return launch_fse_encode(a, s);
    if (!a.meta) {
        a.list = nullptr; a.count = nullptr;
        if (!ragged) return launch_fse_encode_wave(a, s);
        a.sizeSplit = 1;
        const hipError_t e = launch_fse_encode_wave(a, s);
        return e != hipSuccess ? e : launch_fse_encode(a, s);
    }
    a.onlyState = FSE_ENC_PAR;
    hipError_t e = a.list ? launch_fse_enc_lists(a, s) : hipSuccess;
    if (e == hipSuccess) e = launch_fse_encode_wave(a, s);
    if (e != hipSuccess) return e;
    a.onlyState = FSE_ENC_LANE;
    return launch_fse_encode(a, s);
}

#ifndef FSE_DBINS_N
#define FSE_DBINS_N 16
#define FSE_DBIN_LOG 11
#endif
enum { FSE_DCLS_REV11 = 0, FSE_DCLS_REV12 = 1, FSE_DCLS_PLAIN = 2, FSE_DCLS_KINDS = 3, FSE_DBINS = FSE_DBINS_N, FSE_DCLS_COUNT = FSE_DCLS_KINDS * FSE_DBINS };
struct FseDPrepArgs {
    BlockView csrc;
    unsigned maxLog;
    u16* atab;
    u8* symtab;
    s16* norms;
    FseMeta* meta;
    u32* lists;
    u32* counts;
    size_t* results;
    size_t nBlocks;
    int rawRle; const size_t* origSizes; size_t uniformOrig;
};
hipError_t launch_fse_dprep(const FseDPrepArgs& a, hipStream_t s);
hipError_t launch_fse_dprep_from_norm(const FseDPrepArgs& a, const s16* norms, size_t normStride, const u32* maxSVs, u32 tl, hipStream_t s);

struct FseDecArgs {
    u8* dst; size_t dstStride; size_t dstCapacity;
    size_t* results;
    BlockView csrc;
    const u32* dtables; size_t dtStrideU32;
    const u16* atab; const u8* symtab;
    const FseMeta* meta;
    unsigned maxTableLog;
    unsigned ldsLog;
    const u32* list;
    const u32* count;
    int G;
    unsigned slotU32;
    size_t nBlocks;
    unsigned tlMin; int declineNb0; int onlyDeclined;
    u8* symScratch; u32* slotBitmap; u32 nSlots; u32 scratchSlotBytes;
    const u64* dstOffsets = nullptr; const size_t* dstCaps = nullptr;
};
#define FSE_DECLINED ((size_t)0 - (size_t)0x7001)
#define FSE_DEC_FAST_MAXLOG 11u
hipError_t launch_fse_decode(FseDecArgs a, hipStream_t s);
hipError_t launch_fse_decode_classes(FseDecArgs a, const u32* lists, const u32* counts, hipStream_t s);
size_t fse_decode_blocks_per_round(unsigned maxTableLog);

struct HufMeta {
    u32 state;
    u32 hdrSize;
    u32 tableLog;
    u32 maxSV;
};

struct HufCPrepArgs {
    const unsigned* counts; const unsigned* maxSVs; const size_t* histResults;
    BlockView src;
    u8* dst; size_t dstStride; size_t dstCapacity;
    unsigned maxSVReq, huffLogReq;
    u32* ctables; size_t ctStrideU32;
    HufMeta* meta;
    size_t* results;
    size_t nBlocks;
};
hipError_t launch_huf_cprep(const HufCPrepArgs& a, hipStream_t s, void* nodeScratch );
hipError_t launch_huf_cprep_glue(const HufCPrepArgs& a, int mode , hipStream_t s);

struct HufEncArgs {
    u8* dst; size_t dstStride; size_t dstCapacity;
    size_t* results;
    BlockView src;
    const u32* ctables; size_t ctStrideU32;
    const HufMeta* meta;
    int streams;
    int split1X;
    size_t nBlocks;
};
hipError_t launch_huf_encode(const HufEncArgs& a, hipStream_t s);

enum { HUF_DKIND_PAR_TINY = 0, HUF_DKIND_PAR_SMALL = 1, HUF_DKIND_PAR_LARGE = 2, HUF_DKIND_SERIAL = 3, HUF_DCLS_COUNT = 8 };
#ifndef HPAR_ALL_SMALL
#define HPAR_ALL_SMALL 1
#endif
#ifndef HPAR_USE_TINY
#define HPAR_USE_TINY 0
#endif
#define HPAR_DATA_TINY  2304u
#ifndef HPAR_DATA_SMALL
#define HPAR_DATA_SMALL 4608u
#endif
#define HPAR_DATA_LARGE (8192u + 384u)
#define HPAR_MIN_BITS 4096u
struct HufDPrepArgs {
    BlockView csrc;
    BlockView dstSizes;
    u8* dst; size_t dstStride;
    u32* dtables; size_t dtStrideU32;
    HufMeta* meta;
    u32* lists;
    u32* counts;
    size_t* results;
    size_t nBlocks;
    const u64* dstOffsets = nullptr;
    int tableOnly;
    unsigned dtMaxLog;
};
hipError_t launch_huf_dprep(const HufDPrepArgs& a, hipStream_t s);
hipError_t launch_huf_dprep_x2(const HufDPrepArgs& a, hipStream_t s);
hipError_t launch_hdr_results(const void* meta, size_t metaStride, size_t* results, size_t nBlocks, hipStream_t s);
hipError_t launch_fse_export_dtables(const FseDPrepArgs& a, u32* dtables, size_t dtStrideU32, hipStream_t s);

struct HufDecArgs {
    u8* dst; size_t dstStride;
    BlockView dstSizes;
    size_t* results;
    BlockView csrc;
    const u32* dtables; size_t dtStrideU32;
    const HufMeta* meta;
    unsigned maxTableLog;
    unsigned ldsLog;
    const u32* list;
    const u32* count;
    int G; unsigned slotU32;
    int streams;
    int acceptX2;
    int onlyDeclined;
    unsigned classLo;
    size_t nBlocks;
    const u64* dstOffsets = nullptr;
};
#define HUF_DECLINED ((size_t)0 - (size_t)0x7000)
hipError_t launch_huf_decode(HufDecArgs a, hipStream_t s);
hipError_t launch_huf_decode_classes(HufDecArgs a, u32* lists, u32* counts, hipStream_t s);
hipError_t launch_huf_decode_par(HufDecArgs a, unsigned dataBytes, u32* serialList, u32* serialCount, hipStream_t s);
hipError_t launch_huf_decode_par_x2(HufDecArgs a, hipStream_t s);

struct U16Meta { u32 state, hdrSize, tableLog, maxSV; };
struct U16CArgs {
    const u16* src; size_t srcStrideBytes; const size_t* srcSizes; size_t uniformSrcSize;
    u8* dst; size_t dstStride; size_t dstCapacity;
    u32 maxSVReq, tableLogReq;
    u16* stateTables; u32* symTT; U16Meta* meta;
    unsigned* countsOut; unsigned* maxSVOut;
    size_t* results; size_t nBlocks;
};
struct U16DArgs {
    u16* dst; size_t dstStrideBytes; size_t dstCapacity;
    const u8* csrc; size_t cStride; const size_t* cSizes; size_t uniformCSize;
    u32* cells; U16Meta* meta;
    size_t* results; size_t nBlocks;
};
hipError_t launch_u16_compress(const U16CArgs& a, hipStream_t s);
hipError_t launch_u16_decompress(const U16DArgs& a, hipStream_t s);
hipError_t launch_u16_decode_lds(const U16DArgs& a, hipStream_t s);

hipError_t launch_probagen(u8* dst, size_t dstStride, size_t blockSize, size_t nBlocks, const u8* d_table, u32 firstSeed, u32 seedStep, hipStream_t s);

hipError_t launch_compact(u8* packed, size_t packedCapacity, u64* offsets, const u8* slots, size_t slotStride, const size_t* results, const BlockView& src,
                          size_t nBlocks, u64* partials, hipStream_t s);
hipError_t launch_rawrle_expand(u8* dst, size_t dstStride, size_t dstCapacity, size_t* results, const BlockView& csrc, const size_t* origSizes, size_t uniformOrig,
                                size_t nBlocks, hipStream_t s);
hipError_t launch_exscan(u64* a, size_t n, u64* partials, hipStream_t s);
size_t exscan_partials(size_t n);

#define PLANES_TILE ((u64)32768)
hipError_t launch_planes_split(u8* planes, u64* planeOff, size_t* tensorRes, const u8* src, const u8* base, unsigned deltaOp, const u64* srcOff, size_t nTensors,
                               unsigned E, u64 capacity, hipStream_t s);
hipError_t launch_planes_merge(u8* dst, const u64* dstOff, size_t* results, const u8* planes, const u64* planeOff, const size_t* planeSizes, const u8* base,
                               unsigned deltaOp, size_t nTensors, unsigned E, u64 dstCapacity, hipStream_t s);
hipError_t launch_planes_offsets(u64* planeOff, size_t* tensorRes, const u64* srcOff, size_t nTensors, unsigned E, u64 capacity, hipStream_t s);
hipError_t launch_segments(u64* segOff, size_t* tensorRes, const u64* planeOff, const u64* srcOff, const u64* segFirst, size_t nTensors, unsigned E, size_t nSeg,
                           unsigned segLog, hipStream_t s);
struct PlWriter { size_t maxTotalBlocks; unsigned blockSizeId; int codec; uint8_t* d_codecs; int policy; unsigned tolerancePermille, slotAlignLog; void* d_workspace; size_t workspaceBytes; };
struct PlSparse { unsigned permille; void* d_contents; uint64_t* d_contentOffsets; };
size_t sparse_workspace(u64 capacity, size_t nUnits);
bool bad_sparse(u64 capacity, size_t nUnits, const void* d_workspace, size_t workspaceBytes);
hipError_t launch_sparse_pack(u8* contents, u64* contentOff, const u8* units, const u64* unitOff, size_t nUnits, u64 capacity, unsigned permille, u8* ws, hipStream_t s);
int planes_compress(void* d_dst, uint64_t dstCapacity, uint64_t* d_frameOffsets, size_t* d_frameResults, size_t* d_tensorResults, const void* d_src, const void* d_base,
                    unsigned deltaOp, const uint64_t* d_srcOffsets, size_t nTensors, unsigned E, uint64_t capacity, const uint64_t* d_segFirst, size_t nSegments,
                    unsigned segLog, void* d_planes, uint64_t* d_planeOffsets, uint64_t* d_segOffsets, const PlWriter& w, void* stream, const PlSparse* sparse = nullptr,
                    bool pred = false);
hipError_t launch_planes_split_pred(u8* planes, u64* planeOff, size_t* tensorRes, const u8* src, const u64* srcOff, size_t nTensors, unsigned E, u64 capacity,
                                    hipStream_t s);
hipError_t launch_planes_merge_pred(u8* dst, const u64* dstOff, size_t* results, const u8* planes, const u64* planeOff, const size_t* planeSizes, size_t nTensors,
                                    unsigned E, u64 dstCapacity, hipStream_t s);
hipError_t launch_planes_verdicts(size_t* results, const u64* dstOff, const size_t* planeSizes, size_t nTensors, unsigned E, u64 dstCapacity, hipStream_t s);
hipError_t launch_planes_split_each(u8* planes, u64* planeOff, size_t* tensorRes, const u8* src, const u8* base, const u8* transforms, const u64* srcOff, size_t nTensors,
                                    unsigned E, u64 capacity, hipStream_t s);
hipError_t launch_planes_merge_each(u8* dst, const u64* dstOff, size_t* results, const u8* planes, const u64* planeOff, const size_t* planeSizes, const u8* base,
                                    const u8* transforms, size_t nTensors, unsigned E, u64 dstCapacity, hipStream_t s);

enum { PK_HIST = 0, PK_FSE_CPREP, PK_FSE_ENCODE, PK_FSE_DPREP, PK_FSE_DECODE, PK_HUF_CPREP, PK_HUF_ENCODE, PK_HUF_DPREP, PK_HUF_DECODE, PK_FSE_ENCODE_WAVE, PK_COUNT };
void probe_before(int kernelId, hipStream_t s);
void probe_after(int kernelId, hipStream_t s);

struct HostCallBuf {
    void* p = nullptr;
    hipError_t alloc(size_t n);
    ~HostCallBuf();
    HostCallBuf() = default;
    HostCallBuf(const HostCallBuf&) = delete; HostCallBuf& operator=(const HostCallBuf&) = delete;
private:
    size_t carved = 0; bool owned = false;
};
#define FSEHIP_SCRATCH_MAX ((size_t)1 << 30)

struct DevProps { int cus; int ldsPerCU; bool ok; };
const DevProps& dev_props();
hipError_t ensure_dyn_lds(const void* kernel, int bytes);
int fse_compress_view(void* d_dst, size_t dstStride, size_t dstCapacity, size_t* d_results, const BlockView& src, unsigned maxSymbolValue, unsigned tableLog,
                      size_t nBlocks, void* d_workspace, size_t workspaceBytes, hipStream_t s);
int huf_compress_view(int streams, void* d_dst, size_t dstStride, size_t dstCapacity, size_t* d_results, const BlockView& src, unsigned maxSymbolValue,
                      unsigned tableLog, size_t nBlocks, void* d_workspace, size_t workspaceBytes, hipStream_t s);
int fse_decompress_view(void* d_dst, const u64* d_dstOffsets, const size_t* d_dstCaps, size_t* d_results, const BlockView& csrc, unsigned maxLog, size_t nBlocks,
                        void* d_workspace, size_t workspaceBytes, hipStream_t s);
int huf_decompress_view(void* d_dst, const u64* d_dstOffsets, const size_t* d_dstSizes, size_t* d_results, const BlockView& csrc, size_t nBlocks,
                        void* d_workspace, size_t workspaceBytes, hipStream_t s);
int huf_compress_batch_impl(int streams, void* d_dst, size_t dstStride, size_t dstCapacity, size_t* d_results,
                            const void* d_src, size_t srcStride, const size_t* d_sizes, size_t uniformSize,
                            unsigned maxSymbolValue, unsigned tableLog, size_t nBlocks, void* d_workspace, size_t workspaceBytes, void* stream);
int batch_arg_error(size_t* d_results, const size_t* d_sizes, size_t uniform, size_t dstCapacity, size_t nBlocks, size_t code, int mode, hipStream_t s);
hipError_t launch_xxh32(u32* hashes, const u8* data, const u64* starts, const u64* lens, size_t nItems, u32 seed, hipStream_t s);
int release_thread_scratch(void);
int frame_pool_release_scratch(void);
int frame_pool_shutdown(void);
// ... 1 lines not shown
```

Measured before the change: 211,200 MiB/s of uncompressed data through encode+decode (whole job).

## Use persistent grid-stride walk kernels for FSE encode, decode and table build

Lane-encode, decode and decode-table-build kernels are re-included into persistent grid-stride wrappers that loop over groups with a resident-sized grid instead of launching one workgroup per group. The encode list-building kernel is widened to 16 waves with LDS prefix sums, which cuts global atomics. The zeroing of the encode counters is folded into the histogram kernel, removing a separate launch. The intent is to cut launch and workgroup-scheduling overhead and atomic contention. The cost is more complex macro-based code and the risk of load imbalance or missing state resets between loop iterations.

```diff
diff --git a/finitestateentropy_amd/csrc/capi_batch.hip b/finitestateentropy_amd/csrc/capi_batch.hip
--- a/finitestateentropy_amd/csrc/capi_batch.hip
+++ b/finitestateentropy_amd/csrc/capi_batch.hip
@@ -99,7 +99,7 @@
     Carver c; CounterWs<FseMeta> cb; u32* ctables; u32* encLists; u32* encCounts;
     FseCompWs(void* ws, size_t chunk, const FseCWs& w)
         : c(ws), cb(c, chunk), ctables(c.take<u32>(chunk * 4 * w.ctU32)), encLists(c.take<u32>(chunk * FSE_EBINS * sizeof(u32))),
-          encCounts(c.last<u32>(FSE_EBINS * sizeof(u32))) {}
+          encCounts(c.last<u32>((FSE_EBINS + 1) * sizeof(u32))) {}
     size_t end() const { return c.used(); }
 };
 
@@ -137,7 +137,9 @@
     for (size_t b0 = 0; b0 < nBlocks; b0 += chunk) {
         const size_t nb = pass_blocks(nBlocks, b0, chunk);
         const BlockView src = subview(srcAll, b0);
-        CK(launch_hist(ws.cb.hist_args(msv, src, nb), s));
+        HistArgs h = ws.cb.hist_args(msv, src, nb);
+        h.zero = ws.encCounts; h.nZero = FSE_EBINS + 1;
+        CK(launch_hist(h, s));
         FseCPrepArgs c;
         c.counts = ws.cb.counts; c.maxSVs = ws.cb.maxSVs; c.histResults = ws.cb.hres; c.src = src;
         c.dst = (u8*)d_dst + b0 * dstStride; c.dstStride = dstStride; c.dstCapacity = dstCapacity;
@@ -169,7 +171,7 @@
         return d;
     }
 };
-static_assert(5 * 255 + FSE_DCLS_COUNT * sizeof(u32) <= WS_SLACK && 6 * 255 + FSE_EBINS * sizeof(u32) <= WS_SLACK, "WS_SLACK covers the padding of the FSE workspaces");
+static_assert(5 * 255 + FSE_DCLS_COUNT * sizeof(u32) <= WS_SLACK && 6 * 255 + (FSE_EBINS + 1) * sizeof(u32) <= WS_SLACK, "WS_SLACK covers the padding of the FSE workspaces");
 static unsigned clamp_maxlog(unsigned maxLog) { return (maxLog == 0 || maxLog > FSEHIP_FSE_MAX_TABLELOG) ? FSEHIP_FSE_MAX_TABLELOG : maxLog; }
 
 extern "C" size_t FSEHIP_FSE_decompress_batch_workspaceSize(size_t nBlocks, unsigned maxLog) { return ws_size(nBlocks, FseDecWs::bytes_per_block(clamp_maxlog(maxLog))); }
diff --git a/finitestateentropy_amd/csrc/fse_decode.hip b/finitestateentropy_amd/csrc/fse_decode.hip
--- a/finitestateentropy_amd/csrc/fse_decode.hip
+++ b/finitestateentropy_amd/csrc/fse_decode.hip
@@ -1,3 +1,4 @@
+#ifndef FSE_DEC_GROUP_PASS
 #include "internal.h"
 #include <atomic>
 
@@ -351,11 +352,14 @@
 __global__ __launch_bounds__(FSE_DEC_THREADS) void k_fse_decode(FseDecArgs a)
 {
     extern __shared__ __attribute__((aligned(16))) u32 lds[];
+#define FSE_DEC_GROUP blockIdx.x
+#define FSE_DEC_WAY_OUT return
+#endif
     const int tid = threadIdx.x, lane = tid & 63, wave = tid >> 6;
     unsigned long long tBorn = 0, wBorn = 0;
     (void)tBorn; (void)wBorn;
     TIMING(tBorn = __builtin_readcyclecounter(); wBorn = wall_clock64(););
-    const size_t first = (size_t)blockIdx.x * a.G;
+    const size_t first = (size_t)(FSE_DEC_GROUP) * a.G;
     static_assert(FSE_DBINS % 4 == 0, "the bin lengths are read as 16-byte vectors");
     size_t nTot = a.nBlocks, q0 = first;
     u32 bin0 = 0, cnt0 = 0xFFFFFFFFu;
@@ -376,7 +380,7 @@
         }
         nTot = (size_t)before;
     }
-    if (first >= nTot) return;
+    if (first >= nTot) FSE_DEC_WAY_OUT;
     auto slotBlock = [&](size_t g) -> size_t {
         if (!a.list) return first + g;
         size_t q = q0 + g; u32 i = bin0;
@@ -420,7 +424,7 @@
         __syncthreads();
         if (!flagsSh[1]) {
             if (tid == 0) __hip_atomic_fetch_and(a.slotBitmap + (slot >> 5), ~(1u << (slot & 31u)), __ATOMIC_RELEASE, __HIP_MEMORY_SCOPE_AGENT);
-            return;
+            FSE_DEC_WAY_OUT;
         }
     }
     else __syncthreads();
@@ -621,7 +625,7 @@
         ctl->inLo = (u32)ib; ctl->inHi = (u32)(ib >> 32); ctl->outLo = (u32)ob; ctl->outHi = (u32)(ob >> 32); ctl->symLo = (u32)tb; ctl->symHi = (u32)(tb >> 32);
     }
     __syncthreads();
-    if (!decWave) { fse_decode_service<TIMED, CALLER>(a, ldsb, ctlAll, slotBytes, ringOff, inOff, lane, (wave - FSE_DEC_WAVES) * FSE_SRV_G, FAST, flagsSh); return; }
+    if (!decWave) { fse_decode_service<TIMED, CALLER>(a, ldsb, ctlAll, slotBytes, ringOff, inOff, lane, (wave - FSE_DEC_WAVES) * FSE_SRV_G, FAST, flagsSh); FSE_DEC_WAY_OUT; }
 
     __builtin_amdgcn_s_setprio(3);
     uint2* const myRing = (uint2*)(ldsb + (size_t)(gsl < a.G ? gsl : 0) * slotBytes + ringOff) + half;
@@ -775,6 +779,40 @@
                             atomicAdd(&g_decTiming[14], tE - tBulk1); });
     }
     if (CALLER) fse_scratch_slot_done(a, flagsSh, lane);
+#ifndef FSE_DEC_GROUP_PASS
+#undef FSE_DEC_GROUP
+#undef FSE_DEC_WAY_OUT
+}
+template <bool FAST, bool VIEW>
+DEV void fse_decode_walk_class(const FseDecArgs& a)
+{
+    extern __shared__ __attribute__((aligned(16))) u32 lds[];
+    constexpr bool TIMED = false, CALLER = false;
+    size_t nGroups = 0;
+    for (u32 i = 0; i < FSE_DBINS; ++i) nGroups += a.count[i];
+    nGroups = (nGroups + (size_t)a.G - 1) / (size_t)a.G;
+    for (size_t group = blockIdx.x; group < nGroups; group += gridDim.x) {
+        {
+#define FSE_DEC_GROUP_PASS
+#define FSE_DEC_GROUP group
+#define FSE_DEC_WAY_OUT goto groupDone
+#include "fse_decode.hip"
+#undef FSE_DEC_GROUP_PASS
+#undef FSE_DEC_GROUP
+#undef FSE_DEC_WAY_OUT
+        }
+groupDone:
+        __builtin_amdgcn_s_setprio(0);
+        __syncthreads();
+    }
+}
+template <bool VIEW>
+__global__ __launch_bounds__(FSE_DEC_THREADS) void k_fse_decode_walk(FseDecArgs a)
+{
+    static_assert(FSE_DCLS_PLAIN == FSE_DCLS_REV12 + 1, "the plain-cell class's lists follow the tableLog-12 class's");
+    fse_decode_walk_class<true, VIEW>(a);
+    a.list += (size_t)FSE_DBINS * a.nBlocks; a.count += FSE_DBINS;
+    fse_decode_walk_class<false, VIEW>(a);
 }
 
 static void fse_decode_geometry(unsigned ldsLog, size_t ldsBytes, unsigned* slotU32, int* G)
@@ -827,7 +865,7 @@
     return hipSuccess;
 }
 
-static hipError_t fse_decode_launch(FseDecArgs a, bool rev, hipStream_t s)
+static hipError_t fse_decode_launch(FseDecArgs a, bool rev, hipStream_t s, bool walk = false)
 {
     const size_t ldsBytes = FSE_DEC_LDS;
     const bool caller = a.atab == nullptr;
@@ -843,11 +881,19 @@
     if (a.G < 1) return hipErrorInvalidValue;
     if (caller && ((size_t)a.G << a.ldsLog) > FSE_SYM_SLOT_BYTES) return hipErrorInvalidValue;
     const size_t groups = (a.nBlocks + a.G - 1) / a.G;
+    const size_t resident = (size_t)FSE_WGS_PER_CU * (size_t)(dev_props().ok ? dev_props().cus : 256);
+    const dim3 walkGrid((unsigned)(groups < resident ? groups : resident));
     if (a.dstOffsets) {
         if (caller || !a.dstCaps) return hipErrorInvalidValue;
         hipError_t e = ensure_dyn_lds((const void*)k_fse_decode<true, false, false, true>, FSE_DEC_LDS);
         if (e == hipSuccess) e = ensure_dyn_lds((const void*)k_fse_decode<false, false, false, true>, FSE_DEC_LDS);
         if (e != hipSuccess) return e;
+        if (walk) {
+            e = ensure_dyn_lds((const void*)k_fse_decode_walk<true>, FSE_DEC_LDS);
+            if (e != hipSuccess) return e;
+            hipLaunchKernelGGL((k_fse_decode_walk<true>), walkGrid, dim3(FSE_DEC_THREADS), ldsBytes, s, a);
+            return hipGetLastError();
+        }
         if (rev) hipLaunchKernelGGL((k_fse_decode<true, false, false, true>), dim3((unsigned)groups), dim3(FSE_DEC_THREADS), ldsBytes, s, a);
         else     hipLaunchKernelGGL((k_fse_decode<false, false, false, true>), dim3((unsigned)groups), dim3(FSE_DEC_THREADS), ldsBytes, s, a);
         return hipGetLastError();
@@ -860,6 +906,11 @@
         }
         else if (rev) hipLaunchKernelGGL((k_fse_decode<true, false, true>), dim3((unsigned)groups), dim3(FSE_DEC_THREADS), ldsBytes, s, a);
         else     hipLaunchKernelGGL((k_fse_decode<false, false, true>), dim3((unsigned)groups), dim3(FSE_DEC_THREADS), ldsBytes, s, a);
+    }
+    else if (walk) {
+        const hipError_t e = ensure_dyn_lds((const void*)k_fse_decode_walk<false>, FSE_DEC_LDS);
+        if (e != hipSuccess) return e;
+        hipLaunchKernelGGL((k_fse_decode_walk<false>), walkGrid, dim3(FSE_DEC_THREADS), ldsBytes, s, a);
     }
     else if (rev && g_decTimingOn.load(std::memory_order_relaxed)) hipLaunchKernelGGL((k_fse_decode<true, true, false>), dim3((unsigned)groups), dim3(FSE_DEC_THREADS), ldsBytes, s, a);
     else if (rev) hipLaunchKernelGGL((k_fse_decode<true, false, false>), dim3((unsigned)groups), dim3(FSE_DEC_THREADS), ldsBytes, s, a);
@@ -918,12 +969,15 @@
     if (a.nBlocks == 0) return hipSuccess;
     probe_before(PK_FSE_DECODE, s);
     hipError_t e = hipSuccess;
+    const bool walk = !g_decTimingOn.load(std::memory_order_relaxed);
     for (int c = 0; c < FSE_DCLS_KINDS && e == hipSuccess; ++c) {
         if (c != FSE_DCLS_REV11 && a.maxTableLog <= FSE_DEC_FAST_MAXLOG) break;
         a.list = lists + (size_t)c * FSE_DBINS * a.nBlocks; a.count = counts + c * FSE_DBINS;
         a.ldsLog = c == FSE_DCLS_REV11 ? (a.maxTableLog < FSE_DEC_FAST_MAXLOG ? a.maxTableLog : FSE_DEC_FAST_MAXLOG) : a.maxTableLog;
+        if (c == FSE_DCLS_REV12 && walk) { e = fse_decode_launch(a, true, s, true); break; }
         e = fse_decode_launch(a, c != FSE_DCLS_PLAIN, s);
     }
     probe_after(PK_FSE_DECODE, s);
     return e;
 }
+#endif
diff --git a/finitestateentropy_amd/csrc/fse_encode.hip b/finitestateentropy_amd/csrc/fse_encode.hip
--- a/finitestateentropy_amd/csrc/fse_encode.hip
+++ b/finitestateentropy_amd/csrc/fse_encode.hip
@@ -1,3 +1,4 @@
+#ifndef FSE_ENC_GROUP_PASS
 #include "internal.h"
 
 #define FSE_ENC_STEP(x, sym, bits, nb)                                                              \
@@ -10,14 +11,17 @@
 __global__ __launch_bounds__(64) void k_fse_encode(FseEncArgs a)
 {
     extern __shared__ __attribute__((aligned(16))) u32 lds[];
+#define FSE_ENC_GROUP blockIdx.x
+#define FSE_ENC_WAY_OUT return
+#endif
     const u8* const ldsb = (const u8*)lds;
     const u32 lane = threadIdx.x;
-    const size_t first = (size_t)blockIdx.x * a.G;
+    const size_t first = (size_t)(FSE_ENC_GROUP) * a.G;
 
     if (a.meta) {
         const size_t bb = first + lane;
         const bool mine = lane < (u32)a.G && bb < a.nBlocks && !fse_enc_skip(a.meta[bb].state, a.onlyState);
-        if (!__any(mine)) return;
+        if (!__any(mine)) FSE_ENC_WAY_OUT;
     }
 
     for (int g = 0; g < a.G; ++g) {
@@ -40,18 +44,18 @@
         }
     }
     __syncthreads();
-    if (lane >= (u32)a.G) return;
+    if (lane >= (u32)a.G) FSE_ENC_WAY_OUT;
     const size_t b = first + lane;
-    if (b >= a.nBlocks) return;
+    if (b >= a.nBlocks) FSE_ENC_WAY_OUT;
     u32 hdr = 0;
-    if (a.meta) { if (fse_enc_skip(a.meta[b].state, a.onlyState)) return; hdr = a.meta[b].hdrSize; }
-    if (a.sizeSplit && view_size(a.src, b) >= FSE_ENC_WAVE_MIN) return;
+    if (a.meta) { if (fse_enc_skip(a.meta[b].state, a.onlyState)) FSE_ENC_WAY_OUT; hdr = a.meta[b].hdrSize; }
+    if (a.sizeSplit && view_size(a.src, b) >= FSE_ENC_WAVE_MIN) FSE_ENC_WAY_OUT;
 
     const u32 h0 = a.ctables[b * a.ctStrideU32];
     const u32 tl = h0 & 0xFFFFu;
     if (tl > a.maxTableLog) {
         a.results[b] = FERR(tableLog_tooLarge);
-        return;
+        FSE_ENC_WAY_OUT;
     }
     const u32* const tt = lds + (size_t)lane * a.slotU32 + 1 + (tl ? (1u << (tl - 1)) : 1u);
 
@@ -63,7 +67,7 @@
     const size_t cap64 = a.dstCapacity - hdr;
 
     size_t csize = 0;
-    if (n64 >= ((size_t)1 << 31)) { a.results[b] = FERR(srcSize_wrong); return; }
+    if (n64 >= ((size_t)1 << 31)) { a.results[b] = FERR(srcSize_wrong); FSE_ENC_WAY_OUT; }
     const u32 n = (u32)n64;
     if (n > 2 && cap64 > 8) {
         const u32 lim = (u32)(cap64 - 8);
@@ -133,6 +137,28 @@
         if (csize != 0 && (size_t)hdr + csize < n64 - 1) r = (size_t)hdr + csize;
         a.results[b] = r;
     } else a.results[b] = csize;
+#ifndef FSE_ENC_GROUP_PASS
+#undef FSE_ENC_GROUP
+#undef FSE_ENC_WAY_OUT
+}
+__global__ __launch_bounds__(64) void k_fse_encode_walk(FseEncArgs a)
+{
+    extern __shared__ __attribute__((aligned(16))) u32 lds[];
+    if (a.count[FSE_EBINS] == 0) return;
+    const size_t groups = (a.nBlocks + (size_t)a.G - 1) / (size_t)a.G;
+    for (size_t group = blockIdx.x; group < groups; group += gridDim.x) {
+        {
+#define FSE_ENC_GROUP_PASS
+#define FSE_ENC_GROUP group
+#define FSE_ENC_WAY_OUT goto groupDone
+#include "fse_encode.hip"
+#undef FSE_ENC_GROUP_PASS
+#undef FSE_ENC_GROUP
+#undef FSE_ENC_WAY_OUT
+        }
+groupDone:
+        __syncthreads();
+    }
 }
 
 #define FSE_ENC_LDS (80 * 1024)
@@ -155,13 +181,19 @@
 {
     if (a.nBlocks == 0) return hipSuccess;
     const size_t ldsBytes = FSE_ENC_LDS;
-    {   const hipError_t e = ensure_dyn_lds((const void*)k_fse_encode, (int)ldsBytes); if (e != hipSuccess) return e; }
+    const bool walk = a.meta && a.onlyState == FSE_ENC_LANE && a.list && a.count;
+    {   const hipError_t e = ensure_dyn_lds(walk ? (const void*)k_fse_encode_walk : (const void*)k_fse_encode, (int)ldsBytes); if (e != hipSuccess) return e; }
     fse_encode_geometry(a.maxTableLog, &a.slotU32, &a.G);
     if (a.nBlocks > 1 && ((a.src.stride > 0x3FFFFFFu) || (a.dstStride > 0x3FFFFFFu))) a.G = 1;
     if (a.dstCapacity > 0x7FFFFFF0u) a.dstCapacity = 0x7FFFFFF0u;
     const size_t groups = (a.nBlocks + a.G - 1) / a.G;
     probe_before(PK_FSE_ENCODE, s);
-    hipLaunchKernelGGL(k_fse_encode, dim3((unsigned)groups), dim3(64), ldsBytes, s, a);
+    if (walk) {
+        const size_t resident = 2 * (size_t)(dev_props().ok ? dev_props().cus : 256);
+        hipLaunchKernelGGL(k_fse_encode_walk, dim3((unsigned)(groups < resident ? groups : resident)), dim3(64), ldsBytes, s, a);
+    }
+    else hipLaunchKernelGGL(k_fse_encode, dim3((unsigned)groups), dim3(64), ldsBytes, s, a);
     probe_after(PK_FSE_ENCODE, s);
     return hipGetLastError();
 }
+#endif
diff --git a/finitestateentropy_amd/csrc/fse_encode_wave.hip b/finitestateentropy_amd/csrc/fse_encode_wave.hip
--- a/finitestateentropy_amd/csrc/fse_encode_wave.hip
+++ b/finitestateentropy_amd/csrc/fse_encode_wave.hip
@@ -401,7 +401,7 @@
         const unsigned long long partMask = (WV_LANES == 64u ? ~0ull : ((1ull << (WV_LANES & 63u)) - 1ull)) << partBase;
         if (on && (thin & partMask)) {
             if (a.meta && a.onlyState == FSE_ENC_PAR) {
-                if (hl == 0) const_cast<FseMeta*>(a.meta)[b].state = FSE_ENC_LANE;
+                if (hl == 0) { const_cast<FseMeta*>(a.meta)[b].state = FSE_ENC_LANE; if (a.count) atomicAdd(&a.count[FSE_EBINS], 1u); }
             } else if (hl == 0) {
                 const size_t cs = wv_serial<TT4>(ttb, src, n, dst, cap, tl);
                 a.results[b] = a.meta ? ((cs != 0 && (size_t)hdr + cs < n64 - 1) ? (size_t)hdr + cs : 0) : cs;
@@ -440,29 +440,39 @@
     if (on && hl == 0) a.results[b] = result;
 }
 
-__global__ __launch_bounds__(64) void k_fse_enc_lists(FseEncArgs a)
-{
-    const size_t b = (size_t)blockIdx.x * 64 + threadIdx.x;
-    const u32 lane = threadIdx.x;
+#define FSE_ELIST_WAVES 16
+__global__ __launch_bounds__(64 * FSE_ELIST_WAVES) void k_fse_enc_lists(FseEncArgs a)
+{
+    __shared__ u32 at[FSE_EBINS + 1][FSE_ELIST_WAVES];
+    const size_t b = (size_t)blockIdx.x * (64 * FSE_ELIST_WAVES) + threadIdx.x;
+    const u32 lane = threadIdx.x & 63u, wave = threadIdx.x >> 6;
     int bin = -1;
-    if (b < a.nBlocks && a.meta[b].state == FSE_ENC_PAR) { const u32 p = a.meta[b].pace; bin = (int)(p < FSE_EBINS ? p : FSE_EBINS - 1); }
+    if (b < a.nBlocks) {
+        const u32 st = a.meta[b].state;
+        if (st == FSE_ENC_PAR) { const u32 p = a.meta[b].pace; bin = (int)(p < FSE_EBINS ? p : FSE_EBINS - 1); }
+        else if (st == FSE_ENC_LANE) bin = FSE_EBINS;
+    }
     const unsigned long long below = (1ull << lane) - 1ull;
-    for (int c = 0; c < FSE_EBINS; ++c) {
+    u32 place = 0;
+    for (int c = 0; c <= FSE_EBINS; ++c) {
         const unsigned long long mask = __ballot(bin == c);
-        if (!mask) continue;
-        const int leader = __builtin_ctzll(mask);
-        u32 base = 0;
-        if ((int)lane == leader) base = atomicAdd(&a.count[c], (u32)__builtin_popcountll(mask));
-        base = (u32)__shfl((int)base, leader, WAVE);
-        if (bin == c) a.list[(size_t)c * a.nBlocks + base + (u32)__builtin_popcountll(mask & below)] = (u32)b;
-    }
+        if (lane == 0) at[c][wave] = (u32)__builtin_popcountll(mask);
+        if (bin == c) place = (u32)__builtin_popcountll(mask & below);
+    }
+    __syncthreads();
+    if (threadIdx.x <= FSE_EBINS) {
+        u32 total = 0;
+        for (int w = 0; w < FSE_ELIST_WAVES; ++w) { const u32 n = at[threadIdx.x][w]; at[threadIdx.x][w] = total; total += n; }
+        const u32 base = total ? atomicAdd(&a.count[threadIdx.x], total) : 0u;
+        for (int w = 0; w < FSE_ELIST_WAVES; ++w) at[threadIdx.x][w] += base;
+    }
+    __syncthreads();
+    if (bin >= 0 && bin < FSE_EBINS) a.list[(size_t)bin * a.nBlocks + at[bin][wave] + place] = (u32)b;
 }
 hipError_t launch_fse_enc_lists(const FseEncArgs& a, hipStream_t s)
 {
     if (a.nBlocks == 0) return hipSuccess;
-    const hipError_t e = launch_zero_u32(a.count, FSE_EBINS, s);
-    if (e != hipSuccess) return e;
-    hipLaunchKernelGGL(k_fse_enc_lists, dim3((unsigned)((a.nBlocks + 63) / 64)), dim3(64), 0, s, a);
+    hipLaunchKernelGGL(k_fse_enc_lists, dim3((unsigned)((a.nBlocks + 64 * FSE_ELIST_WAVES - 1) / (64 * FSE_ELIST_WAVES))), dim3(64 * FSE_ELIST_WAVES), 0, s, a);
     return hipGetLastError();
 }
 
diff --git a/finitestateentropy_amd/csrc/fse_tables.hip b/finitestateentropy_amd/csrc/fse_tables.hip
--- a/finitestateentropy_amd/csrc/fse_tables.hip
+++ b/finitestateentropy_amd/csrc/fse_tables.hip
@@ -1,3 +1,4 @@
+#ifndef FSE_DBUILD_ENTRY_PASS
 #include "internal.h"
 
 #include "wave_glue.h"
@@ -166,12 +167,15 @@
         for (int k = firstList / (int)FSE_DBINS; k < (firstList + nLists) / (int)FSE_DBINS; ++k) total += a.counts[FSE_DCLS_COUNT + k];
         if (blockIdx.x >= total) return;
     }
+#define FSE_DBUILD_ENTRY blockIdx.x
+#define FSE_DBUILD_WAY_OUT return
+#endif
     constexpr int MAXL = 2 * FSE_DBINS;
     static_assert(FSE_DBINS % 4 == 0, "the list lengths are read as 16-byte vectors");
     uint4 cv[MAXL / 4];
 #pragma unroll
     for (int i = 0; i < MAXL / 4; ++i) cv[i] = 4 * i < nLists ? ((const uint4*)(a.counts + firstList))[i] : make_uint4(0, 0, 0, 0);
-    u32 idx = blockIdx.x;
+    u32 idx = FSE_DBUILD_ENTRY;
     int c = firstList + nLists;
     {   u32 before = 0; bool found = false;
 #pragma unroll
@@ -184,15 +188,15 @@
             before += n;
         }
     }
-    if (c == firstList + nLists) return;
+    if (c == firstList + nLists) FSE_DBUILD_WAY_OUT;
     const size_t b = a.lists[(size_t)c * a.nBlocks + idx];
     const u32 lane = threadIdx.x;
     const FseMeta m = a.meta[b];
-    if (m.state == 0) return;
+    if (m.state == 0) FSE_DBUILD_WAY_OUT;
     const u32 tl = m.tableLog, ts = 1u << tl;
     if (ts > ldsCapTs || ts > 64u * MAXC) {
         if (lane == 0) { a.meta[b].state = 0; a.results[b] = FERR(tableLog_tooLarge); }
-        return;
+        FSE_DBUILD_WAY_OUT;
     }
     const WaveBuildLds w = wave_build_carve(wbLds, ldsCapTs, false);
     *(uint2*)(w.nrm + 4 * lane) = *(const uint2*)(a.norms + b * 256 + 4 * lane);
@@ -210,6 +214,29 @@
         S[x] = (u8)s;
     });
     if (lane == 0) a.meta[b].state = m.state | (fast ? 2u : 0u);
+#ifndef FSE_DBUILD_ENTRY_PASS
+#undef FSE_DBUILD_ENTRY
+#undef FSE_DBUILD_WAY_OUT
+}
+template <u32 MAXC>
+__global__ __launch_bounds__(64) void k_fse_dbuild_walk(FseDPrepArgs a, u32 capTs, int firstList, int nLists, u32 ldsCapTs)
+{
+    extern __shared__ __attribute__((aligned(16))) u8 wbLds[];
+    u32 total = 0;
+    for (int k = firstList / (int)FSE_DBINS; k < (firstList + nLists) / (int)FSE_DBINS; ++k) total += a.counts[FSE_DCLS_COUNT + k];
+    for (u32 entry = blockIdx.x; entry < total; entry += gridDim.x) {
+        {
+#define FSE_DBUILD_ENTRY_PASS
+#define FSE_DBUILD_ENTRY entry
+#define FSE_DBUILD_WAY_OUT goto entryDone
+#include "fse_tables.hip"
+#undef FSE_DBUILD_ENTRY_PASS
+#undef FSE_DBUILD_ENTRY
+#undef FSE_DBUILD_WAY_OUT
+        }
+entryDone:
+        __syncthreads();
+    }
 }
 
 __global__ __launch_bounds__(256) void k_fse_export_dtable(FseDPrepArgs a, u32 capTs, u32* dtables, size_t dtStrideU32)
@@ -284,10 +311,16 @@
 
 static void launch_fse_dbuild_lists(const FseDPrepArgs& a, u32 capTs, int firstList, int nLists, u32 ldsCapTs, hipStream_t s)
 {
+    const size_t ldsBytes = wave_build_lds_bytes(ldsCapTs, false);
     if (wb_small(ldsCapTs))
-        hipLaunchKernelGGL(k_fse_dbuild<32>, dim3((unsigned)a.nBlocks), dim3(64), wave_build_lds_bytes(ldsCapTs, false), s, a, capTs, firstList, nLists, ldsCapTs);
-    else
-        hipLaunchKernelGGL(k_fse_dbuild<64>, dim3((unsigned)a.nBlocks), dim3(64), wave_build_lds_bytes(ldsCapTs, false), s, a, capTs, firstList, nLists, ldsCapTs);
+        hipLaunchKernelGGL(k_fse_dbuild<32>, dim3((unsigned)a.nBlocks), dim3(64), ldsBytes, s, a, capTs, firstList, nLists, ldsCapTs);
+    else {
+        const size_t cus = (size_t)(dev_props().ok ? dev_props().cus : 256), ldsPerCu = 160u * 1024u;
+        size_t perCu = ldsPerCu / (ldsBytes ? ldsBytes : 1);
+        perCu = perCu < 1 ? 1 : perCu > 16 ? 16 : perCu;
+        const size_t grid = a.nBlocks < cus * perCu ? a.nBlocks : cus * perCu;
+        hipLaunchKernelGGL(k_fse_dbuild_walk<64>, dim3((unsigned)grid), dim3(64), ldsBytes, s, a, capTs, firstList, nLists, ldsCapTs);
+    }
 }
 static void launch_fse_dbuilds(const FseDPrepArgs& a, hipStream_t s)
 {
@@ -436,3 +469,4 @@
     probe_after(PK_FSE_DPREP, s);
     return hipGetLastError();
 }
+#endif
diff --git a/finitestateentropy_amd/csrc/hist.hip b/finitestateentropy_amd/csrc/hist.hip
--- a/finitestateentropy_amd/csrc/hist.hip
+++ b/finitestateentropy_amd/csrc/hist.hip
@@ -36,6 +36,7 @@
     const unsigned limitIn = (a.maxSVs && !a.useUniformIn) ? a.maxSVs[b] : a.uniformMaxSV;
     const bool checked = limitIn < 255u && !a.trustInput;
     const unsigned nOut = limitIn < 255u ? limitIn + 1u : 256u;
+    if (a.zero && b == 0 && lane < a.nZero) a.zero[lane] = 0;
 
     u32 t0 = 0, t1 = 0, t2 = 0, t3 = 0;
 
diff --git a/finitestateentropy_amd/csrc/internal.h b/finitestateentropy_amd/csrc/internal.h
--- a/finitestateentropy_amd/csrc/internal.h
+++ b/finitestateentropy_amd/csrc/internal.h
@@ -25,6 +25,7 @@
     size_t* results;
     BlockView src;
     size_t nBlocks;
+    u32* zero = nullptr; u32 nZero = 0;
 };
 hipError_t launch_hist(const HistArgs& a, hipStream_t s);
 #define HIST_PIECE ((size_t)65536)
```

After: 212,500 MiB/s of uncompressed data through encode+decode (whole job), median of 6. No clear change (+0.6%).
